# advimman/lama

Hardware: AMD Instinct MI355X
Metric: inpainted images/sec at 512x512 big-lama (higher is better)
Workload: dtype f32 (3-term f16 split on the 16-bit MFMA, fp32 accumulate, fp32 activations); 1 GPU; big-lama FFCResNetGenerator 512x512 batch=8/GPU fp32 (BASELINE configs[1]), mask-compose + generator + blend + u8, random-init weights; global_batch=8, resolution=512, parallelism=dp1, hip_graph=True, precision=f16x3, split_batch=1, full=False

## Files before the change

### include/lama_hip.h

```cpp
#ifndef LAMA_HIP_H
#define LAMA_HIP_H
#include <stddef.h>
#include <stdint.h>

#ifdef __cplusplus
extern "C" {
#endif

#define LAMA_HIP_VERSION 112

#define LAMA_OK 0
#define LAMA_ERR_BAD_ARG (-1)
#define LAMA_ERR_UNSUPPORTED (-2)
#define LAMA_ERR_WORKSPACE (-3)

#define LAMA_ACT_NONE 0
#define LAMA_ACT_RELU 1
#define LAMA_ACT_SIGMOID 2
#define LAMA_ACT_TANH 3

#define LAMA_PAD_ZERO 0
#define LAMA_PAD_REFLECT 1

#define LAMA_PREC_F32 0
#define LAMA_PREC_BF16X3 1
#define LAMA_PREC_F16X3 2
#define LAMA_PREC_F16 3

#define LAMA_DT_F32 0
#define LAMA_DT_F16 1

typedef struct lama_tensor {
    void* ptr;
    int64_t batch_stride;
    int32_t C, H, W;
    int32_t dtype;
} lama_tensor;

typedef struct lama_conv2d_args {
    lama_tensor x;
    const void* w_packed;
    int32_t kh, kw, stride, pad, pad_mode, transposed;
    lama_tensor x2;
    const void* w2_packed;
    const float* bias;
    int32_t act;
    lama_tensor resid;
    lama_tensor y;
    int32_t batch;
    int32_t precision;
    uint32_t* range_flag;
    const void* fuse1_w;
    const float* fuse1_bias;
    lama_tensor fuse1_y;
    int32_t flags;
} lama_conv2d_args;
#define LAMA_CONV_COOPERATIVE 1
#define LAMA_CONV_SIBLINGS_SHIFT 8
#define LAMA_CONV_SIBLINGS_MASK (7 << LAMA_CONV_SIBLINGS_SHIFT)
#define LAMA_CONV_SIBLINGS_LOG2(flags) (((flags) & LAMA_CONV_SIBLINGS_MASK) >> LAMA_CONV_SIBLINGS_SHIFT)
#define LAMA_CONV_DEFER_OUT 2

void lama_fuse1_channel_order(int32_t* order);

int lama_version(void);
const char* lama_error_string(int code);

int64_t lama_conv2d_packed_weight_bytes(int32_t cout, int32_t cin, int32_t kh, int32_t kw, int32_t stride,
                                        int32_t transposed, int32_t precision);
int lama_conv2d_pack_weight(void* stream, const float* w, const float* scale, int32_t cout, int32_t cin, int32_t kh,
                            int32_t kw, int32_t stride, int32_t transposed, int32_t precision, void* dst);
int lama_conv2d_fwd(void* stream, const lama_conv2d_args* args);

int64_t lama_winograd_packed_weight_bytes(int32_t cout, int32_t cin, int32_t precision);
int32_t lama_winograd_supported(int32_t cout, int32_t cin, int32_t H, int32_t W, int32_t precision);
int32_t lama_winograd_preferred(int32_t batch, int32_t cout, int32_t cin, int32_t H, int32_t W, int32_t precision);
int lama_winograd_pack_weight(void* stream, const float* w, const float* scale, int32_t cout, int32_t cin, int32_t precision, void* dst);
size_t lama_winograd_workspace_bytes(int32_t batch, int32_t cout, int32_t H, int32_t W);
int lama_winograd_conv3x3_fwd(void* stream, const lama_conv2d_args* args, void* workspace, size_t workspace_bytes);
int lama_winograd_out_fwd(void* stream, const lama_conv2d_args* args, void* workspace, size_t workspace_bytes);
int lama_rfft2_winograd_out_fwd(void* stream, const lama_tensor* x, const lama_tensor* spec, int32_t batch, void* workspace, size_t workspace_bytes,
                                const lama_conv2d_args* wino_args, void* wino_workspace, size_t wino_workspace_bytes);
int lama_fourier_unit_winograd_out_fwd(void* stream, const lama_tensor* x, const void* w_packed, const float* bias, const lama_tensor* y,
                                       int32_t batch, int32_t add_input, int32_t precision, void* workspace, size_t workspace_bytes,
                                       uint32_t* range_flag, const lama_conv2d_args* wino_args, void* wino_workspace,
                                       size_t wino_workspace_bytes);

int lama_multidilated_conv3x3_fwd(void* stream, const lama_conv2d_args* args, int32_t groups, int32_t min_dilation);

int lama_rfft2_fwd(void* stream, const lama_tensor* x, const lama_tensor* spec, int32_t batch, void* workspace,
                   size_t workspace_bytes);
int lama_irfft2_fwd(void* stream, const lama_tensor* spec, const lama_tensor* resid, const lama_tensor* y,
                    int32_t batch, void* workspace, size_t workspace_bytes);
int lama_rfft2_masked_fwd(void* stream, const lama_tensor* x, const lama_tensor* spec, const lama_tensor* mask_y, int32_t batch,
                          void* workspace, size_t workspace_bytes);
int lama_irfft2_masked_fwd(void* stream, const lama_tensor* spec, const lama_tensor* resid, const lama_tensor* mask_y, const lama_tensor* y,
                           int32_t batch, void* workspace, size_t workspace_bytes);
size_t lama_fft_workspace_bytes(int32_t batch, int32_t C, int32_t h, int32_t w);
#define LAMA_FFT_KIND_WINO64 0
#define LAMA_FFT_KIND_IP64 1
#define LAMA_FFT_KIND_IP128 2
#define LAMA_FFT_KIND_TRACE64 3
#define LAMA_FFT_KIND_SEQ 4
#define LAMA_FFT_KIND_SIZED 5
#define LAMA_FFT_KIND_GENERIC 6
int lama_fft_route_query(const lama_tensor* real, const lama_tensor* resid, const lama_tensor* spec, const lama_tensor* mask, int32_t batch,
                         int32_t inverse, const void* workspace, size_t workspace_bytes, int32_t* family, int32_t* kind);

size_t lama_fourier_unit_workspace_bytes(int32_t batch, int32_t C, int32_t h, int32_t w);
int lama_fourier_unit_fwd(void* stream, const lama_tensor* x, const void* w_packed, const float* bias,
                          const lama_tensor* y, int32_t batch, int32_t add_input, int32_t precision, void* workspace,
                          size_t workspace_bytes, uint32_t* range_flag);
int lama_fourier_unit_ex_fwd(void* stream, const lama_tensor* x, const void* w_packed, const float* bias, const lama_tensor* y,
// ... 111 lines not shown
```

### lama_amd/_lib.py

```python
from __future__ import annotations

import ctypes as C
import os
from typing import Optional

import torch

ACT_NONE, ACT_RELU, ACT_SIGMOID, ACT_TANH = 0, 1, 2, 3
PAD_ZERO, PAD_REFLECT = 0, 1
PREC_F32, PREC_BF16X3, PREC_F16X3, PREC_F16 = 0, 1, 2, 3
CONV_COOPERATIVE = 1
CONV_DEFER_OUT = 2
CONV_SIBLINGS_SHIFT = 8
DT_F32, DT_F16 = 0, 1
POOL_MAX, POOL_AVG_EXCLUDE_PAD = 0, 1
ABI_VERSION = 112
PREC_NAMES = {'f32': PREC_F32, 'bf16x3': PREC_BF16X3, 'f16x3': PREC_F16X3, 'f16': PREC_F16}

_DEFAULT = os.path.join(os.path.dirname(os.path.abspath(__file__)), 'lib', 'liblama_hip.so')


class LamaError(RuntimeError):

    def __init__(self, msg: str = '', code=None):
        super().__init__(msg)
        self.code = code


class LamaRangeError(LamaError):
    """A weight or an activation left the range of the fp16 split (|x| <= 65504): re-run with PREC_BF16X3 / PREC_F32."""

F16_MAX = 65504.0
ERR_BAD_ARG, ERR_UNSUPPORTED, ERR_WORKSPACE = -1, -2, -3
FFT_KIND_WINO64, FFT_KIND_IP64, FFT_KIND_IP128, FFT_KIND_TRACE64, FFT_KIND_SEQ, FFT_KIND_SIZED, FFT_KIND_GENERIC = range(7)


class Tensor4(C.Structure):
    _fields_ = [('ptr', C.c_void_p), ('batch_stride', C.c_int64), ('C', C.c_int32), ('H', C.c_int32), ('W', C.c_int32),
                ('dtype', C.c_int32)]


class Conv2dArgs(C.Structure):
    _fields_ = [('x', Tensor4), ('w_packed', C.c_void_p),
                ('kh', C.c_int32), ('kw', C.c_int32), ('stride', C.c_int32), ('pad', C.c_int32),
                ('pad_mode', C.c_int32), ('transposed', C.c_int32),
                ('x2', Tensor4), ('w2_packed', C.c_void_p), ('bias', C.c_void_p), ('act', C.c_int32),
                ('resid', Tensor4), ('y', Tensor4), ('batch', C.c_int32), ('precision', C.c_int32),
                ('range_flag', C.c_void_p), ('fuse1_w', C.c_void_p), ('fuse1_bias', C.c_void_p), ('fuse1_y', Tensor4),
                ('flags', C.c_int32)]


class Conv2dRectArgs(C.Structure):
    _fields_ = [('x', Tensor4), ('w_packed', C.c_void_p), ('bias', C.c_void_p), ('act', C.c_int32), ('y', Tensor4), ('batch', C.c_int32),
                ('kh', C.c_int32), ('kw', C.c_int32), ('stride', C.c_int32), ('pad_h', C.c_int32), ('pad_w', C.c_int32),
                ('precision', C.c_int32), ('range_flag', C.c_void_p)]


class TailLists(C.Structure):
    _fields_ = [('n_up', C.c_int32), ('head_rs', C.c_int32), ('up_mg', C.c_int32 * 4), ('head_list', C.c_void_p), ('head_count', C.c_void_p),
                ('up_list', C.c_void_p * 4), ('up_count', C.c_void_p * 4)]


def view(t: Optional[torch.Tensor], c0: int = 0, c: Optional[int] = None) -> Tensor4:
    if t is None:
        return Tensor4(None, 0, 0, 0, 0, 0)
    if t.dtype not in (torch.float32, torch.float16) or t.dim() != 4 or not t.is_contiguous():
        raise LamaError(f'expected a contiguous fp32 / fp16 NCHW tensor, got {t.dtype} {tuple(t.shape)}')
    B, Ct, H, W = t.shape
    c = Ct - c0 if c is None else c
    if c0 < 0 or c <= 0 or c0 + c > Ct:
        raise LamaError('channel slice out of range')
    return Tensor4(t.data_ptr() + t.element_size() * c0 * H * W, Ct * H * W, c, H, W, DT_F16 if t.dtype == torch.float16 else DT_F32)


class LamaLib:
    def __init__(self, path: Optional[str] = None, host_emulated: bool = False):
        self.host_emulated = host_emulated
        path = path or _DEFAULT
        if not os.path.exists(path):
            raise LamaError(f'{path} not found: build it with `python -m lama_amd.build` '
                            f'(hipcc --offload-arch=gfx950); lama_amd has no fallback path')
        self.path = path
        L = self._l = C.CDLL(path)
        i32, i64, vp, sz = C.c_int32, C.c_int64, C.c_void_p, C.c_size_t
        T = C.POINTER(Tensor4)
        L.lama_version.restype = C.c_int
        L.lama_error_string.restype = C.c_char_p
        L.lama_error_string.argtypes = [C.c_int]
        L.lama_conv2d_packed_weight_bytes.restype = i64
        L.lama_conv2d_packed_weight_bytes.argtypes = [i32] * 7
        L.lama_conv2d_pack_weight.restype = C.c_int
        L.lama_conv2d_pack_weight.argtypes = [vp, vp, vp, i32, i32, i32, i32, i32, i32, i32, vp]
        L.lama_conv2d_fwd.restype = C.c_int
        L.lama_conv2d_fwd.argtypes = [vp, C.POINTER(Conv2dArgs)]
        L.lama_conv2d_list_fwd.restype, L.lama_conv2d_list_fwd.argtypes = C.c_int, [vp, C.POINTER(Conv2dArgs), vp, vp, i32]
        L.lama_conv2d_list_supported.restype, L.lama_conv2d_list_supported.argtypes = i32, [C.POINTER(Conv2dArgs), i32]
        L.lama_tail_lists_workspace_bytes.restype, L.lama_tail_lists_workspace_bytes.argtypes = sz, [i32, i32, i32, C.POINTER(TailLists)]
        L.lama_tail_lists_build.restype, L.lama_tail_lists_build.argtypes = C.c_int, [vp, T, i32, C.POINTER(TailLists), vp, sz]
        L.lama_rfft2_fwd.restype = C.c_int
        L.lama_rfft2_fwd.argtypes = [vp, T, T, i32, vp, sz]
        L.lama_irfft2_fwd.restype = C.c_int
        L.lama_irfft2_fwd.argtypes = [vp, T, T, T, i32, vp, sz]
        L.lama_winograd_out_fwd.restype = C.c_int
        L.lama_winograd_out_fwd.argtypes = [vp, C.POINTER(Conv2dArgs), vp, sz]
        L.lama_rfft2_winograd_out_fwd.restype = C.c_int
        L.lama_rfft2_winograd_out_fwd.argtypes = [vp, T, T, i32, vp, sz, C.POINTER(Conv2dArgs), vp, sz]
        L.lama_rfft2_masked_fwd.restype = C.c_int
        L.lama_rfft2_masked_fwd.argtypes = [vp, T, T, T, i32, vp, sz]
        L.lama_irfft2_masked_fwd.restype = C.c_int
        L.lama_irfft2_masked_fwd.argtypes = [vp, T, T, T, T, i32, vp, sz]
        L.lama_fft_workspace_bytes.restype = sz
        L.lama_fft_workspace_bytes.argtypes = [i32] * 4
        L.lama_fft_route_query.restype = C.c_int
        L.lama_fft_route_query.argtypes = [T, T, T, T, i32, i32, vp, sz, C.POINTER(C.c_int32), C.POINTER(C.c_int32)]
        L.lama_fourier_unit_workspace_bytes.restype = sz
        L.lama_fourier_unit_workspace_bytes.argtypes = [i32] * 4
        L.lama_fourier_unit_fwd.restype = C.c_int
        L.lama_fourier_unit_fwd.argtypes = [vp, T, vp, vp, T, i32, i32, i32, vp, sz, vp]
        L.lama_fourier_unit_winograd_out_fwd.restype = C.c_int
        L.lama_fourier_unit_winograd_out_fwd.argtypes = [vp, T, vp, vp, T, i32, i32, i32, vp, sz, vp, C.POINTER(Conv2dArgs), vp, sz]
        L.lama_fourier_unit_ex_fwd.restype = C.c_int
        L.lama_fourier_unit_ex_fwd.argtypes = [vp, T, vp, vp, T, i32, i32, i32, vp, sz, vp, i32, C.POINTER(Conv2dArgs), vp, sz]
        L.lama_mask_compose_fwd.restype = C.c_int
        L.lama_mask_compose_fwd.argtypes = [vp, T, T, T, i32]
        L.lama_blend_fwd.restype = C.c_int
        L.lama_blend_fwd.argtypes = [vp, T, T, T, T, i32]
        L.lama_quantize_u8_hwc_fwd.restype = C.c_int
        L.lama_quantize_u8_hwc_fwd.argtypes = [vp, T, vp, i32, i32, i32]
        L.lama_mask_compose_u8_fwd.restype = C.c_int
        L.lama_mask_compose_u8_fwd.argtypes = [vp, vp, vp, vp, T, i32, i32]
        L.lama_blend_quantize_u8_fwd.restype = C.c_int
        L.lama_blend_quantize_u8_fwd.argtypes = [vp, vp, vp, vp, T, vp, i32, i32]
        L.lama_resize_u8_fwd.restype = C.c_int
        L.lama_resize_u8_fwd.argtypes = [vp, vp, vp, vp, vp, i32, i32, C.c_double, T, T, i32, i32]
        L.lama_eval_ingest_u8_fwd.restype = C.c_int
        L.lama_eval_ingest_u8_fwd.argtypes = [vp, vp, vp, vp, C.POINTER(i32), i32, i32, i32, i32, C.c_float, C.c_float, T, T, vp, i32]
        L.lama_affine_act_fwd.restype = C.c_int
        L.lama_affine_act_fwd.argtypes = [vp, T, vp, vp, i32, T, i32]
        L.lama_reflect_pad_fwd.restype = C.c_int
        L.lama_reflect_pad_fwd.argtypes = [vp, T, i32, T, i32]
        f32, dp = C.c_float, C.POINTER(C.c_double)
        for name, args in (('lama_act_bwd', [vp, T, T, i32, T, i32]), ('lama_add_fwd', [vp, T, T, T, i32]),
                           ('lama_reflect_pad_bwd', [vp, T, T, i32, T, i32]), ('lama_reflect_pad_bwd_fused', [vp, T, T, T, i32, T, i32, T, T, i32, vp]),
                           ('lama_dgrad_ring_fwd', [vp, T, vp, i32, vp, i32]),
                           ('lama_gauss5_fwd', [vp, T, T, i32]),
                           ('lama_gauss5_bwd', [vp, T, T, i32]), ('lama_bilinear_fwd', [vp, T, T, i32]),
                           ('lama_bilinear_bwd', [vp, T, T, i32]), ('lama_threshold_fwd', [vp, T, f32, T, i32]),
                           ('lama_erode_fwd', [vp, T, vp, i32, i32, f32, T, i32]),
                           ('lama_l1_masked_fwd', [vp, T, T, T, f32, i32, vp, i32]),
                           ('lama_l1_masked_bwd', [vp, T, T, T, f32, i32, f32, i32, T, i32]),
                           ('lama_l1_masked_per_image_fwd', [vp, T, T, T, f32, i32, vp, i32]),
                           ('lama_l1_masked_per_image_bwd', [vp, T, T, T, f32, i32, vp, i32, T, i32]),
                           ('lama_adam_step', [vp, vp, vp, vp, vp, i64, f32, f32, f32, f32, i32])):
            fn = getattr(L, name)
            fn.restype, fn.argtypes = C.c_int, args
# ... 531 lines not shown
```

### lama_amd/csrc/conv_mfma.hip

```cpp
#include "common.h"

typedef float f32x16 __attribute__((ext_vector_type(16)));

#define CONV_BN 128
#define CONV_MAX_TAPS 49

struct ConvSeg {
    const float* x;
    long long bstride;
    int C, H, W;
    const float* w;
    int stride, pad_mode;
    int dy0, dx0;
    int PH, PW;
    int tapoff[CONV_MAX_TAPS];
};

struct ConvParams {
    ConvSeg s1, s2;
    const float* bias;
    const float* resid;
    long long resid_bstride;
    float* y;
    long long y_bstride;
// ... 491 lines not shown
    const int m0 = blockIdx.y * 16, b = blockIdx.z;
    if (pix >= HW) return;
    const int gy = pix / p.W, gx = pix - gy * p.W;
    const float* xb = p.x + (long long)b * p.x_bstride;
    float acc[16];
#pragma unroll
    for (int j = 0; j < 16; ++j) acc[j] = 0.0f;
    for (int c = 0; c < p.C; ++c) {
        const int d = p.dmin << (c / p.gch);
        const float* xc = xb + (long long)c * HW;
        const float* wc = p.w + ((long long)(c >> 3) * 72 + (c & 7)) * p.Mpad + m0;
        for (int ky = 0; ky < 3; ++ky) {
            const int iy = conv_src_coord(gy + (ky - 1) * d, p.H, LAMA_PAD_REFLECT);
            for (int kx = 0; kx < 3; ++kx) {
                const int ix = conv_src_coord(gx + (kx - 1) * d, p.W, LAMA_PAD_REFLECT);
                const float v = xc[iy * p.W + ix];
                const float* wt = wc + (long long)((ky * 3 + kx) * 8) * p.Mpad;
#pragma unroll
                for (int j = 0; j < 16; ++j) acc[j] = fmaf(wt[j], v, acc[j]);
            }
        }
    }
#pragma unroll
    for (int j = 0; j < 16; ++j) {
        const int m = m0 + j;
        float v = acc[j];
        if (p.bias) v += p.bias[m];
        if (p.act == LAMA_ACT_RELU) v = fmaxf(v, 0.0f);
        else if (p.act == LAMA_ACT_SIGMOID) v = 1.0f / (1.0f + expf(-v));
        else if (p.act == LAMA_ACT_TANH) v = tanhf(v);
        const long long o = (long long)m * HW + pix;
        if (p.resid) v += p.resid[(long long)b * p.resid_bstride + o];
        p.y[(long long)b * p.y_bstride + o] = v;
    }
}

extern "C" int lama_multidilated_conv3x3_fwd(void* stream, const lama_conv2d_args* a, int32_t groups, int32_t min_dilation) {
    if (!a || !tensor_ok(a->x) || !tensor_ok(a->y) || !a->w_packed || a->batch <= 0) return LAMA_ERR_BAD_ARG;
    if ((groups != 1 && groups != 2 && groups != 4) || min_dilation < 1 || min_dilation > 8) return LAMA_ERR_UNSUPPORTED;
    if (a->kh != 3 || a->kw != 3 || a->stride != 1 || a->pad_mode != LAMA_PAD_REFLECT || a->transposed) return LAMA_ERR_UNSUPPORTED;
    if (a->x2.ptr || a->fuse1_w) return LAMA_ERR_UNSUPPORTED;
    if (a->x.dtype != LAMA_DT_F32 || a->y.dtype != LAMA_DT_F32 || (a->resid.ptr && a->resid.dtype != LAMA_DT_F32)) return LAMA_ERR_UNSUPPORTED;
    if (a->x.H != a->y.H || a->x.W != a->y.W) return LAMA_ERR_BAD_ARG;
    if (a->resid.ptr && (a->resid.C != a->y.C || a->resid.H != a->y.H || a->resid.W != a->y.W)) return LAMA_ERR_BAD_ARG;
    const int cout = a->y.C, cin = a->x.C, H = a->x.H, W = a->x.W;
    if (cin % (16 * groups) != 0 || cout % 32 != 0) return LAMA_ERR_UNSUPPORTED;
    const int dmax = min_dilation << (groups - 1);
    if (H <= dmax || W <= dmax) return LAMA_ERR_UNSUPPORTED;
    if (a->precision == LAMA_PREC_BF16X3) return lama_cb_mdconv_fwd_bf16x3((hipStream_t)stream, a, groups, min_dilation);
    if (a->precision == LAMA_PREC_F16X3) return lama_cb_mdconv_fwd_f16x3((hipStream_t)stream, a, groups, min_dilation);
    if (a->precision != LAMA_PREC_F32) return LAMA_ERR_UNSUPPORTED;
    if ((long long)cin * H * W >= (1ll << 31) || cout / 16 > 65535 || a->batch > 65535) return LAMA_ERR_UNSUPPORTED;
    MdF32Params p;
    memset(&p, 0, sizeof(p));
    p.x = (const float*)a->x.ptr;
    p.x_bstride = a->x.batch_stride;
    p.C = cin; p.H = H; p.W = W;
    p.w = (const float*)a->w_packed;
    p.Mpad = lama_round_up(cout, pick_bm(cout));
    p.bias = a->bias;
    p.resid = (const float*)a->resid.ptr;
    p.resid_bstride = a->resid.batch_stride;
    p.y = (float*)a->y.ptr;
    p.y_bstride = a->y.batch_stride;
    p.M = cout;
    p.gch = cin / groups;
    p.dmin = min_dilation;
    p.act = a->act;
    hipLaunchKernelGGL(mdconv_f32_kernel, dim3(lama_ceil_div(H * W, LAMA_NTHREADS), cout / 16, a->batch), dim3(LAMA_NTHREADS), 0, (hipStream_t)stream, p);
    LAMA_CHECK_LAUNCH();
    return LAMA_OK;
}

extern "C" void lama_fuse1_channel_order(int32_t* order) {
    for (int kq = 0; kq < 24; ++kq)
        for (int kh = 0; kh < 2; ++kh)
            for (int i = 0; i < 8; ++i) order[16 * kq + 8 * kh + i] = 32 * (kq / 2) + 16 * (kq & 1) + 8 * (i / 4) + 4 * kh + (i % 4);
}

static int conv2d_impl(void* stream, const lama_conv2d_args* a, const LamaTileList* tl) {
    if (!a || !tensor_ok(a->x) || !tensor_ok(a->y) || !a->w_packed || a->batch <= 0) return LAMA_ERR_BAD_ARG;
    if (a->precision != LAMA_PREC_F32 && a->precision != LAMA_PREC_BF16X3 && a->precision != LAMA_PREC_F16X3 && a->precision != LAMA_PREC_F16)
        return LAMA_ERR_UNSUPPORTED;
    {
        const bool xh = a->x.dtype == LAMA_DT_F16, yh = a->y.dtype == LAMA_DT_F16;
        if ((a->x.dtype != LAMA_DT_F32 && !xh) || (a->y.dtype != LAMA_DT_F32 && !yh)) return LAMA_ERR_BAD_ARG;
        if (a->x2.ptr && a->x2.dtype != LAMA_DT_F32 && a->x2.dtype != LAMA_DT_F16) return LAMA_ERR_BAD_ARG;
        if (a->x2.ptr && a->x2.dtype == LAMA_DT_F16 && a->precision != LAMA_PREC_F16) return LAMA_ERR_UNSUPPORTED;
        if (a->resid.ptr && a->resid.dtype != a->y.dtype) return LAMA_ERR_BAD_ARG;
        if ((xh || yh) != (a->precision == LAMA_PREC_F16)) return LAMA_ERR_UNSUPPORTED;
    }
    const int cout = a->y.C, cin = a->x.C;
    ConvPlan pl;
    if (!make_plan(cout, cin, a->kh, a->kw, a->stride, a->pad, a->transposed, &pl)) return LAMA_ERR_UNSUPPORTED;
    int Ho, Wo;
    if (a->transposed) {
        Ho = a->x.H * 2; Wo = a->x.W * 2;
    } else {
        Ho = (a->x.H + 2 * a->pad - a->kh) / a->stride + 1;
        Wo = (a->x.W + 2 * a->pad - a->kw) / a->stride + 1;
    }
    if (Ho != a->y.H || Wo != a->y.W) return LAMA_ERR_BAD_ARG;
    if (a->pad_mode == LAMA_PAD_REFLECT && (a->pad >= a->x.H || a->pad >= a->x.W)) return LAMA_ERR_BAD_ARG;
    const bool has2 = a->x2.ptr != nullptr;
    if (has2 && (a->transposed || !a->w2_packed || a->x2.H != Ho || a->x2.W != Wo || !tensor_ok(a->x2))) return LAMA_ERR_BAD_ARG;
    if (a->resid.ptr && (a->resid.C != cout || a->resid.H != Ho || a->resid.W != Wo)) return LAMA_ERR_BAD_ARG;
    if (a->fuse1_w) {
        if (!tensor_ok(a->fuse1_y) || a->fuse1_y.dtype != LAMA_DT_F32 || a->fuse1_y.C != 192 || a->fuse1_y.H != Ho || a->fuse1_y.W != Wo) return LAMA_ERR_BAD_ARG;
        if (cout != 384 || !has2 || a->kh != 3 || a->stride != 1 || a->y.dtype != LAMA_DT_F32 ||
            (a->precision != LAMA_PREC_BF16X3 && a->precision != LAMA_PREC_F16X3))
            return LAMA_ERR_UNSUPPORTED;
    }
    if (a->precision == LAMA_PREC_BF16X3) return lama_cb_conv2d_fwd_bf16x3((hipStream_t)stream, a, Ho, Wo, tl);
    if (a->precision == LAMA_PREC_F16X3) return lama_cb_conv2d_fwd_f16x3((hipStream_t)stream, a, Ho, Wo, tl);
    if (a->precision == LAMA_PREC_F16) return lama_cb_conv2d_fwd_f16((hipStream_t)stream, a, Ho, Wo, tl);
    if (tl) return LAMA_ERR_UNSUPPORTED;

    ConvPlan pl2;
    if (has2 && !make_plan(cout, a->x2.C, 1, 1, 1, 0, 0, &pl2)) return LAMA_ERR_UNSUPPORTED;
    if (has2 && pl2.BM != pl.BM) return LAMA_ERR_UNSUPPORTED;

    for (int cls = 0; cls < pl.nseg; ++cls) {
        ConvParams p;
        memset(&p, 0, sizeof(p));
        const bool flat = (pl.T[cls] == 1 && !a->transposed && a->stride == 1 && a->pad == 0 && !has2);
        p.bias = a->bias;
        p.resid = (const float*)a->resid.ptr;
        p.resid_bstride = a->resid.batch_stride;
        p.y = (float*)a->y.ptr;
        p.y_bstride = a->y.batch_stride;
        p.M = cout;
        p.Mpad = pl.Mpad;
        p.MT = pl.MT;
        p.B = a->batch;
        p.act = a->act;
        if (flat) {
            p.Ho = 1; p.Wo = Ho * Wo; p.GH = 1; p.GW = Ho * Wo; p.ostep = 1;
        } else if (a->transposed) {
            p.Ho = Ho; p.Wo = Wo; p.GH = a->x.H; p.GW = a->x.W; p.ostep = 2;
            p.oy0 = pl.oy0[cls]; p.ox0 = pl.ox0[cls];
        } else {
            p.Ho = Ho; p.Wo = Wo; p.GH = Ho; p.GW = Wo; p.ostep = 1;
        }
        const int stride = a->transposed ? 1 : a->stride;
        const int pad_mode = a->transposed ? LAMA_PAD_ZERO : a->pad_mode;
        const int maxp1 = pl.T[cls] == 1 ? pl.BKC[cls] * CONV_BN / LAMA_NTHREADS : 10;
        int twlog = flat ? 7 : 5;
        while (twlog > 3 && (1 << (twlog - 1)) >= p.GW) --twlog;
        bool ok = false;
        for (; twlog >= 3; --twlog) {
            ok = fill_seg(&p.s1, a->x, (const float*)a->w_packed + pl.woff[cls], pl, cls, stride, pad_mode, twlog, maxp1, flat);
            if (ok) break;
        }
        if (!ok) return LAMA_ERR_UNSUPPORTED;
        p.TWlog = twlog;
        p.tiles_x = lama_ceil_div(p.GW, 1 << twlog);
        p.tiles_y = lama_ceil_div(p.GH, CONV_BN >> twlog);
        int T2 = 0, BKC2 = 0;
        if (has2) {
            T2 = 1; BKC2 = pl2.BKC[0];
            if (!fill_seg(&p.s2, a->x2, (const float*)a->w2_packed, pl2, 0, 1, LAMA_PAD_ZERO, twlog, BKC2 * CONV_BN / LAMA_NTHREADS, false))
                return LAMA_ERR_UNSUPPORTED;
        }
        int rc = launch_conv((hipStream_t)stream, p, pl.T[cls], pl.BKC[cls], T2, BKC2, pl.BM);
        if (rc != LAMA_OK) return rc;
    }
    return LAMA_OK;
// ... 14 lines not shown
```

### lama_amd/csrc/conv_split3.inc

```
#include "common.h"
#include <stdlib.h>

typedef float f32x16 __attribute__((ext_vector_type(16)));
typedef float f32x2 __attribute__((ext_vector_type(2)));
#ifndef CB_HALF
#define CB_HALF 0
#endif
#ifndef CB_HF_W2
#define CB_HF_W2 1
#endif
#if CB_F16
typedef _Float16 cb_half_t;
#define CB_MFMA __builtin_amdgcn_mfma_f32_32x32x16_f16
#if CB_HALF
#define CB_NAME(x) x##_f16
#else
#define CB_NAME(x) x##_f16x3
#endif
#else
typedef __bf16 cb_half_t;
#define CB_MFMA __builtin_amdgcn_mfma_f32_32x32x16_bf16
#define CB_NAME(x) x##_bf16x3
#endif
typedef cb_half_t bf16x2 __attribute__((ext_vector_type(2)));
typedef cb_half_t bf16x8 __attribute__((ext_vector_type(8)));
typedef unsigned u32x4 __attribute__((ext_vector_type(4)));

namespace CB_NAME(cbns) {

#define CB_THREADS 512
#define CB_MAX_TAPS 49

enum { CB_IO_F32 = 0, CB_IO_F16_F32 = 1, CB_IO_F32_F16 = 2, CB_IO_F16 = 3, CB_IO_X2H = 4 };

struct CbSeg {
    const float* x;
    long long bstride;
    int C, H, W;
    const char* w;
    int mft;
    int nchunk, NG;
    int stride, pad_mode;
    int dy0, dx0;
    int PH, PW;
    int PWs, PWh;
    int npix;
    int tapoff[CB_MAX_TAPS];
    int vpad;
};

struct CbParams {
    CbSeg s1, s2;
    const float* bias;
    const float* resid;
    long long resid_bstride;
    float* y;
    long long y_bstride;
    int M, MT;
    int Ho, Wo;
    int GH, GW, oy0, ox0, ostep;
    long long* trace;
    const char* f1_w;
    const float* f1_bias;
    float* f1_y;
    long long f1_y_bstride;
    int TWlog, tiles_x, tiles_y, B;
    int act;
    int wbytes, pbytes;
    int nwbuf;
    unsigned* range_flag;
};

template <int BM, int NACC = 1, int MODE = 0>
struct CbGeom {
    static constexpr int WAVES_M = (BM >= 128 || ((NACC == 4 || MODE == 1) && BM == 64)) ? 2 : 1;
    static constexpr int WAVES_N = 8 / WAVES_M;
    static constexpr int BN = WAVES_N * 32;
    static constexpr int TM = BM / WAVES_M / 32;
    static constexpr int MF = BM / 32;
};

__device__ __forceinline__ int cb_src_coord(int i, int n, int pad_mode) {
    if (pad_mode == LAMA_PAD_REFLECT) {
        if (i < 0) i = -i;
        if (i >= n) i = 2 * (n - 1) - i;
        if (i < 0) i = 0;
        if (i >= n) i = n - 1;
        return i;
    }
    return (i < 0 || i >= n) ? -1 : i;
}

__device__ __forceinline__ void cb_split2(float a, float b, unsigned& hi, unsigned& lo) {
    f32x2 v = {a, b};
    bf16x2 h = __builtin_convertvector(v, bf16x2);
    f32x2 r = v - __builtin_convertvector(h, f32x2);
    bf16x2 l = __builtin_convertvector(r, bf16x2);
    hi = __builtin_bit_cast(unsigned, h);
    lo = __builtin_bit_cast(unsigned, l);
}

__device__ __forceinline__ void cb_split2_mix(float a, float b, unsigned& hi, unsigned& lo) {
#if CB_F16
    f32x2 v = {a, b};
    hi = __builtin_bit_cast(unsigned, __builtin_convertvector(v, bf16x2));
    LAMA_F16_SPLIT_LO(lo, hi, a, b);
#else
    cb_split2(a, b, hi, lo);
#endif
}

typedef unsigned short cb_u16x2 __attribute__((ext_vector_type(2)));
__device__ __forceinline__ void cb_split2(float a, float b, unsigned& hi, unsigned& lo, unsigned& rw) {
    cb_split2(a, b, hi, lo);
#if CB_F16
    rw = __builtin_bit_cast(unsigned, __builtin_elementwise_max(__builtin_bit_cast(cb_u16x2, rw), __builtin_bit_cast(cb_u16x2, hi & 0x7fff7fffu)));
// ... 752 lines not shown
        return LAMA_ERR_UNSUPPORTED;
    }
#if defined(LAMA_PROFILING) && !CB_HALF
    if (!CB_F16 && T1 == 9 && T2 == 0 && BM == 128 && maxu <= 1) {
        static const int abl = lama_env_int("LAMA_CB_ABLATE", 0);
#define CB_ABL(v) \
    if (abl == v) { hipLaunchKernelGGL((CB_NAME(conv_kernel)<9, 3, 1, 0, 0, 0, 128, 1, v>), dim3(grid), dim3(CB_THREADS), shmem, st, p); LAMA_CHECK_LAUNCH(); return LAMA_OK; }
        CB_ABL(1) CB_ABL(2) CB_ABL(4) CB_ABL(6) CB_ABL(8) CB_ABL(14) CB_ABL(15) CB_ABL(16) CB_ABL(32)
#undef CB_ABL
    }
#endif
#define CB_CASE(t1, g1, k1, t2, g2, k2) \
    if (T1 == t1 && T2 == t2) return cb_launch_bm<t1, g1, k1, t2, g2, k2>(st, p, BM, maxu, grid, shmem, io);
    CB_CASE(9, 3, 1, 0, 0, 0)
    CB_CASE(9, 3, 1, 1, 1, 2)
    CB_CASE(1, 1, 2, 0, 0, 0)
    CB_CASE(49, 7, 1, 0, 0, 0)
    CB_CASE(2, 2, 1, 0, 0, 0)
    CB_CASE(4, 4, 1, 0, 0, 0)
#undef CB_CASE
    return LAMA_ERR_UNSUPPORTED;
}

#include "conv_wreg_host.inc"

}

}
using namespace CB_NAME(cbns);

int64_t CB_NAME(lama_cb_packed_weight_bytes)(int cout, int cin, int kh, int kw, int stride, int transposed) {
    CbPlan pl;
    if (!cb_make_plan(cout, cin, kh, kw, stride, transposed ? 1 : kh / 2, transposed, &pl)) return LAMA_ERR_UNSUPPORTED;
    return pl.total_bytes;
}

int CB_NAME(lama_cb_pack_weight)(hipStream_t stream, const float* w, const float* scale, int cout, int cin, int kh, int kw, int stride,
                        int transposed, void* dst) {
    CbPlan pl;
    if (!cb_make_plan(cout, cin, kh, kw, stride, transposed ? 1 : kh / 2, transposed, &pl)) return LAMA_ERR_UNSUPPORTED;
    for (int cls = 0; cls < pl.nseg; ++cls) {
        CbPackParams pp;
        memset(&pp, 0, sizeof(pp));
        pp.w = w;
        pp.scale = scale;
        pp.dst = (char*)dst + pl.woff[cls];
        pp.M = cout;
        pp.C = cin;
        pp.MFT = pl.mft;
        pp.mode = pl.mode;
        pp.TG = pl.TG[cls];
        pp.KS = pl.KS[cls];
        pp.NG = pl.T[cls] / pl.TG[cls];
        pp.nchunk = pl.nchunk[cls];
        pp.kh = kh;
        pp.kw = kw;
        pp.transposed = transposed;
        for (int t = 0; t < pl.T[cls]; ++t) { pp.tap_ky[t] = pl.ky[cls][t]; pp.tap_kx[t] = pl.kx[cls][t]; }
        long long total = pl.cls_bytes[cls] / 32;
        int grid = (int)((total + 255) / 256);
        if (grid > 4096) grid = 4096;
        hipLaunchKernelGGL(CB_NAME(conv_pack_kernel), dim3(grid), dim3(256), 0, stream, pp);
        LAMA_CHECK_LAUNCH();
    }
    return LAMA_OK;
}

int CB_NAME(lama_cb_conv2d_fwd)(hipStream_t stream, const lama_conv2d_args* a, int Ho, int Wo, const LamaTileList* tl) {
    const int cout = a->y.C, cin = a->x.C;
    CbPlan pl;
    if (!cb_make_plan(cout, cin, a->kh, a->kw, a->stride, a->pad, a->transposed, &pl)) return LAMA_ERR_UNSUPPORTED;
    const bool has2 = a->x2.ptr != nullptr;
    if (tl) {
        if (has2 || a->fuse1_w) return LAMA_ERR_UNSUPPORTED;
        const int io_l = (a->x.dtype == LAMA_DT_F16 ? 1 : 0) | (a->y.dtype == LAMA_DT_F16 ? 2 : 0);
        if ((io_l != CB_IO_F32) != (CB_HALF != 0)) return LAMA_ERR_UNSUPPORTED;
        return a->transposed ? ct_try_launch(stream, a, pl, Ho, Wo, io_l, tl) : head_try_launch(stream, a, pl, Ho, Wo, io_l, tl);
    }
    CbPlan pl2;
    if (has2 && !cb_make_plan(cout, a->x2.C, 1, 1, 1, 0, 0, &pl2)) return LAMA_ERR_UNSUPPORTED;
    if (has2 && pl.mode) return LAMA_ERR_UNSUPPORTED;
    const int io = (a->x.dtype == LAMA_DT_F16 ? 1 : 0) | (a->y.dtype == LAMA_DT_F16 ? 2 : 0) | ((has2 && a->x2.dtype == LAMA_DT_F16) ? CB_IO_X2H : 0);
    if ((io != CB_IO_F32) != (CB_HALF != 0)) return LAMA_ERR_UNSUPPORTED;
    {
        int rc = cw_try_launch(stream, a, pl, has2 ? &pl2 : nullptr, Ho, Wo, io);
        if (rc != LAMA_ERR_UNSUPPORTED) return rc;
        if (!has2) {
            rc = ct_try_launch(stream, a, pl, Ho, Wo, io);
            if (rc != LAMA_ERR_UNSUPPORTED) return rc;
        }
    }
    if (a->fuse1_w) return LAMA_ERR_UNSUPPORTED;

    if (!has2) {
        int rc = stem_try_launch(stream, a, pl, Ho, Wo, io);
        if (rc != LAMA_ERR_UNSUPPORTED) return rc;
        rc = head_try_launch(stream, a, pl, Ho, Wo, io);
        if (rc != LAMA_ERR_UNSUPPORTED) return rc;
    }
    int BM = cb_pick_bm(pl.rows, pl.mode ? 49 : pl.T[0], a->transposed ? 1 : a->stride, a->batch, a->transposed ? a->x.H : Ho,
                        a->transposed ? a->x.W : Wo);
    { static const int bm_env = lama_env_int("LAMA_CB_BM", 0); if (bm_env && a->transposed) BM = bm_env; }
    if (BM < 128 && !a->transposed && a->stride == 2) BM = 128;
    if (pl.mode == 1) BM = cout > 64 ? 128 : 64;
    const int BN = (BM >= 128 || ((a->transposed || pl.mode == 1) && BM == 64)) ? 128 : 256;
    if ((long long)a->x.C * a->x.H * a->x.W >= (1ll << 31) || (has2 && (long long)a->x2.C * a->x2.H * a->x2.W >= (1ll << 31)))
        return LAMA_ERR_UNSUPPORTED;

    for (int cls = 0; cls < (a->transposed ? 1 : pl.nseg); ++cls) {
        CbParams p;
        memset(&p, 0, sizeof(p));
        const bool flat = (pl.T[cls] == 1 && !a->transposed && a->stride == 1 && a->pad == 0 && !has2);
        p.bias = a->bias;
        p.resid = (const float*)a->resid.ptr;
        p.resid_bstride = a->resid.batch_stride;
        p.y = (float*)a->y.ptr;
        p.y_bstride = a->y.batch_stride;
        p.M = pl.rows;
        p.MT = lama_ceil_div(pl.rows, BM);
        p.B = a->batch;
        p.act = a->act;
        p.range_flag = a->range_flag;
        if (flat) {
            p.Ho = 1; p.Wo = Ho * Wo; p.GH = 1; p.GW = Ho * Wo; p.ostep = 1;
        } else if (a->transposed) {
            p.Ho = Ho; p.Wo = Wo; p.GH = a->x.H; p.GW = a->x.W; p.ostep = 2;
            p.oy0 = pl.oy0[cls]; p.ox0 = pl.ox0[cls];
        } else {
            p.Ho = Ho; p.Wo = Wo; p.GH = Ho; p.GW = Wo; p.ostep = 1;
        }
        const int stride = a->transposed ? 1 : a->stride;
        const int pad_mode = a->transposed ? LAMA_PAD_ZERO : a->pad_mode;
        int twlog = flat ? lama_ilog2(BN) : 5;
        while (pl.mode != 2 && twlog > 3 && (1 << (twlog - 1)) >= p.GW) --twlog;
        const int TW = 1 << twlog, TH = BN >> twlog;
        p.TWlog = twlog;
        p.tiles_x = pl.mode == 2 ? lama_ceil_div(p.GW, 26) : lama_ceil_div(p.GW, TW);
        p.tiles_y = lama_ceil_div(p.GH, TH);
        int units = cb_fill_seg(&p.s1, a->x, (const char*)a->w_packed + pl.woff[cls], pl, cls, stride, pad_mode, TH, TW, flat);
        p.s1.vpad = a->pad;
        long long wbytes = (long long)pl.TG[cls] * pl.KS[cls] * (BM / 32) * 2048;
        long long pbytes = (long long)2 * 2 * pl.KS[cls] * p.s1.npix * 16;
        int TG2 = 0, KS2 = 0;
        if (has2) {
            TG2 = pl2.TG[0]; KS2 = pl2.KS[0];
            int u2 = cb_fill_seg(&p.s2, a->x2, (const char*)a->w2_packed, pl2, 0, 1, LAMA_PAD_ZERO, TH, TW, false);
            units = u2 > units ? u2 : units;
            long long w2 = (long long)TG2 * KS2 * (BM / 32) * 2048, p2 = (long long)2 * 2 * KS2 * p.s2.npix * 16;
            wbytes = w2 > wbytes ? w2 : wbytes;
            pbytes = p2 > pbytes ? p2 : pbytes;
        }
        p.wbytes = (int)wbytes;
        p.pbytes = (int)pbytes;
        {
            int smax = p.s1.nchunk * p.s1.NG;
            if (has2 && p.s2.nchunk * p.s2.NG > smax) smax = p.s2.nchunk * p.s2.NG;
            p.nwbuf = smax < 3 ? smax : 3;
        }
        int rc = cb_launch(stream, p, pl.T[cls], has2 ? 1 : 0, BM, lama_ceil_div(units, CB_THREADS), a->transposed != 0, pl.mode, io);
        if (rc != LAMA_OK) return rc;
    }
    return LAMA_OK;
}

#if !CB_HALF
int CB_NAME(lama_cb_mdconv_fwd)(hipStream_t stream, const lama_conv2d_args* a, int groups, int min_dilation) {
// ... 238 lines not shown
```

### lama_amd/csrc/conv_stem_dev.inc

```

struct StemParams {
    const float* x;
    long long x_bstride;
    int C, H, W;
    const char* w;
    int mft;
    const float* bias;
    float* y;
    long long y_bstride;
    int M, B, act;
    int tx;
    int ns, rs;
    int nseg;
    unsigned* range_flag;
};

#define STEM_WIN 40
#define STEM_SLOT (4 * STEM_WIN)
#define STEM_WAVE_LDS (8 * STEM_SLOT + 64)
#define STEM_LDS_BYTES (4 * STEM_WAVE_LDS * 4)

__device__ __forceinline__ void stem_pack2(float a, float b, unsigned& pa, unsigned& pb, unsigned& rw) {
    unsigned hi, lo;
    cb_split2(a, b, hi, lo, rw);
    pa = __builtin_amdgcn_perm(lo, hi, 0x05040100u);
    pb = __builtin_amdgcn_perm(lo, hi, 0x07060302u);
}

template <bool HO = false>
__global__ __launch_bounds__(256, 2) void CB_NAME(stem7_ws_kernel)(StemParams p) {
    constexpr int ESO = HO ? 2 : 4;
    const int tid = threadIdx.x, lane = tid & 63, wave = LAMA_WAVE_UNIFORM(tid >> 6);
    const int F = wave & 1, half = wave >> 1;
    const int khalf = lane >> 5, l31 = lane & 31;
    const int H = p.H, W = p.W, HW = H * W;
    const int strip = blockIdx.x * 2 + half, nstrips = gridDim.x * 2;
    unsigned* const win = reinterpret_cast<unsigned*>(lama_smem) + wave * STEM_WAVE_LDS;
    unsigned rw = 0;

    for (int i = lane; i < STEM_WAVE_LDS; i += 64) win[i] = 0u;

    constexpr bool ALO = !HO || CB_HF_W2;
    u32x4 ah[14], al[ALO ? 14 : 1];
    {
        const lama_buf_t wres = LAMA_BUF_RSRC(p.w, (long long)14 * p.mft * 2048);
        const int Fc = F < p.mft ? F : p.mft - 1;
#pragma unroll
        for (int s = 0; s < 14; ++s) {
            ah[s] = __builtin_bit_cast(u32x4, LAMA_BUF_LOAD_B128(wres, lane * 16, (s * p.mft + Fc) * 2048));
            if constexpr (ALO) al[s] = __builtin_bit_cast(u32x4, LAMA_BUF_LOAD_B128(wres, lane * 16 + 1024, (s * p.mft + Fc) * 2048));
        }
    }
    float bv[16];
    {
        const lama_buf_t bres = LAMA_BUF_RSRC(p.bias, p.bias ? (long long)p.M * 4 : 0ll);
#pragma unroll
        for (int r = 0; r < 16; ++r) bv[r] = __builtin_bit_cast(float, LAMA_BUF_LOAD_B32(bres, (F * 32 + (r & 3) + 8 * (r >> 2) + 4 * khalf) * 4, 0));
    }
    int widx[2][8];
#pragma unroll
    for (int ks = 0; ks < 2; ++ks)
#pragma unroll
        for (int e = 0; e < 8; ++e) {
            const int c = 16 * ks + 8 * khalf + e;
            const int cc = c / 7, kx = c - cc * 7;
            widx[ks][e] = c < 28 ? cc * STEM_WIN + l31 + kx : l31;
        }
    int lcc[3], lj[3], lw[3];
#pragma unroll
    for (int i = 0; i < 3; ++i) {
        const int id = lane + 64 * i;
        lcc[i] = id / 38;
        lj[i] = id - lcc[i] * 38;
        lw[i] = id < 152 ? lcc[i] * STEM_WIN + lj[i] : -1;
    }
    LAMA_WAVE_SYNC();

#pragma unroll 1
    for (int g = strip; g < p.nseg; g += nstrips) {
        const int col = g / p.ns, part = g - col * p.ns;
        const int b = col / p.tx, px0 = (col - b * p.tx) * 32;
        const int y0 = part * p.rs, y1 = (y0 + p.rs < H) ? y0 + p.rs : H;
        const lama_buf_t xres = LAMA_BUF_RSRC(p.x + (long long)b * p.x_bstride, (long long)p.C * HW * 4);
        const lama_buf_t yres = LAMA_BUF_RSRC(reinterpret_cast<char*>(p.y) + (long long)b * p.y_bstride * ESO, (long long)p.M * HW * ESO);
        int coloff[3];
#pragma unroll
        for (int i = 0; i < 3; ++i) {
            int ix = px0 - 3 + lj[i];
            ix = ix < 0 ? -ix : ix;
            ix = ix >= W ? 2 * (W - 1) - ix : ix;
            ix = ix < 0 ? 0 : (ix >= W ? W - 1 : ix);
            coloff[i] = (lw[i] >= 0 && lcc[i] < p.C) ? (lcc[i] * HW + ix) * 4 : 0x7ffffff0;
        }
        auto row_off = [&](int u) {
            int iy = u < 0 ? -u : u;
            iy = iy >= H ? 2 * (H - 1) - iy : iy;
            iy = iy < 0 ? 0 : (iy >= H ? H - 1 : iy);
            return iy * W * 4;
        };
        float nr[3];
        auto request_row = [&](int u) {
            const int ro = row_off(u);
#pragma unroll
            for (int i = 0; i < 3; ++i) nr[i] = __builtin_bit_cast(float, LAMA_BUF_LOAD_B32(xres, coloff[i], ro));
        };
        auto deposit_row = [&](int u) {
            unsigned pk[4];
            stem_pack2(nr[0], nr[1], pk[0], pk[1], rw);
            stem_pack2(nr[2], 0.0f, pk[2], pk[3], rw);
            unsigned* slot = win + ((u + 8) & 7) * STEM_SLOT;
#pragma unroll
            for (int i = 0; i < 3; ++i) {
                if (lw[i] >= 0) slot[lw[i]] = pk[i];
                else win[8 * STEM_SLOT + lane] = pk[i];
            }
        };
        for (int u = y0 - 3; u <= y0 + 3; ++u) {
            request_row(u);
            deposit_row(u);
        }
        LAMA_WAVE_SYNC();

#pragma unroll 1
        for (int y = y0; y < y1; ++y) {
            request_row(y + 4);
            f32x16 acc;
#pragma unroll
            for (int r = 0; r < 16; ++r) acc[r] = 0.0f;
            unsigned d[2][8];
            auto read_k = [&](auto s_tag) {
                constexpr int s = decltype(s_tag)::value;
                const unsigned* slot = win + ((y + (s >> 1) + 5) & 7) * STEM_SLOT;
#pragma unroll
                for (int e = 0; e < 8; ++e) d[s & 1][e] = slot[widx[s & 1][e]];
            };
            auto mma_k = [&](auto s_tag) {
                constexpr int s = decltype(s_tag)::value;
                if constexpr (s + 1 < 14) read_k(CbTag<(s + 1 < 14 ? s + 1 : 0)>{});
                unsigned hh[4], ll[4];
#pragma unroll
                for (int e = 0; e < 4; ++e) {
                    hh[e] = __builtin_amdgcn_perm(d[s & 1][2 * e + 1], d[s & 1][2 * e], 0x05040100u);
                    ll[e] = __builtin_amdgcn_perm(d[s & 1][2 * e + 1], d[s & 1][2 * e], 0x07060302u);
                }
                const bf16x8 bh = __builtin_bit_cast(bf16x8, u32x4{hh[0], hh[1], hh[2], hh[3]});
                const bf16x8 bl = __builtin_bit_cast(bf16x8, u32x4{ll[0], ll[1], ll[2], ll[3]});
                __builtin_amdgcn_sched_barrier(0);
                acc = CB_MFMA(__builtin_bit_cast(bf16x8, ah[s]), bh, acc, 0, 0, 0);
                if constexpr (!HO) acc = CB_MFMA(__builtin_bit_cast(bf16x8, ah[s]), bl, acc, 0, 0, 0);
                if constexpr (ALO) acc = CB_MFMA(__builtin_bit_cast(bf16x8, al[s]), bh, acc, 0, 0, 0);
            };
            read_k(CbTag<0>{});
            mma_k(CbTag<0>{}); mma_k(CbTag<1>{}); mma_k(CbTag<2>{}); mma_k(CbTag<3>{}); mma_k(CbTag<4>{}); mma_k(CbTag<5>{}); mma_k(CbTag<6>{});
            mma_k(CbTag<7>{}); mma_k(CbTag<8>{}); mma_k(CbTag<9>{}); mma_k(CbTag<10>{}); mma_k(CbTag<11>{}); mma_k(CbTag<12>{}); mma_k(CbTag<13>{});
            LAMA_WAVE_SYNC();
            deposit_row(y + 4);
            LAMA_WAVE_SYNC();
            const int px = px0 + l31;
            const int eoff = (px < W && F < p.mft) ? ((F * 32 + 4 * khalf) * HW + y * W + px) * ESO : 0x7ffffff0;
            float ov[16];
#pragma unroll
            for (int r = 0; r < 16; ++r) ov[r] = acc[r] + bv[r];
            if (p.act == LAMA_ACT_RELU) {
#pragma unroll
                for (int r = 0; r < 16; ++r) ov[r] = fmaxf(ov[r], 0.0f);
            } else if (p.act == LAMA_ACT_SIGMOID) {
#pragma unroll
                for (int r = 0; r < 16; ++r) ov[r] = 1.0f / (1.0f + expf(-ov[r]));
            } else if (p.act == LAMA_ACT_TANH) {
#pragma unroll
                for (int r = 0; r < 16; ++r) ov[r] = tanhf(ov[r]);
            }
#pragma unroll
            for (int r = 0; r < 16; ++r) {
                if constexpr (HO) LAMA_BUF_STORE_B16(yres, __builtin_bit_cast(unsigned short, (_Float16)ov[r]), eoff, ((r & 3) + 8 * (r >> 2)) * HW * ESO);
                else LAMA_BUF_STORE_B32(yres, __builtin_bit_cast(unsigned, ov[r]), eoff, ((r & 3) + 8 * (r >> 2)) * HW * ESO);
            }
        }
        LAMA_WAVE_SYNC();
    }
    cb_range_report(rw, p.range_flag);
}
```

### lama_amd/csrc/conv_wreg_dev.inc

```

template <int T, int KSC, int WMV, int KG>
struct CwShape {
    static_assert((T == 9 && (KSC == 2 || (KSC == 1 && KG == 1))) || (T == 1 && KSC == 4),
                  "3x3 over 32-channel chunks (16-channel chunks in the 4 x 1 geometry) or 1x1 over 64-channel chunks");
    static_assert(KG == 1 || KG == 2, "K-groups");
    static constexpr int THREADS = 64 * WMV * KG;
    static constexpr int NKG = T * KSC / KG;
    static constexpr int WPS = WMV * KG / 4;
    static constexpr int PFD = (T == 1 && KG == 2) ? 2 : 1;
#ifndef LAMA_CW_RING9
#define LAMA_CW_RING9 0
#endif
    static constexpr int RING = (T == 9) ? ((LAMA_CW_RING9 && KG == 2 && WPS <= 2) ? 9 : ((KSC == 2 && WMV == 4 && KG == 1) ? 6 : 3)) : ((WPS >= 3) ? 2 : 4);
    static constexpr bool BDB = WPS <= 2;
    static constexpr int NOCT = 2 * KSC;
    static_assert((PFD * NKG) % RING == 0, "ring slot must be a compile-time function of the unrolled position");
};

struct CwFrag {
    bf16x8 bh[4], bl[4];
};

template <int T, int KSC, int WMV, int KG, int ABL = 0, int SCH = 2, bool HF = false, bool HI = HF, bool ROLL = false, int NU = 2>
__device__ __forceinline__ void cw_segment(const CbSeg& s, int F, int b, int gy0, int gx0, int TWlog, char* pbuf0, int pbytes,
                                           f32x16 (&acc)[4], unsigned& rw, long long* trace = nullptr) {
    using S = CwShape<T, KSC, WMV, KG>;
    constexpr int NKG = S::NKG, PFD = S::PFD, RING = S::RING, NOCT = S::NOCT, D = RING - 1, THREADS = S::THREADS;
    constexpr bool BDB = S::BDB;
    constexpr int BKC = 16 * KSC;
    constexpr int ES = HI ? 2 : 4;
    const int tid = threadIdx.x, lane = tid & 63, wave = LAMA_WAVE_UNIFORM(tid >> 6);
    const int kg = KG == 1 ? 0 : wave / WMV;
    const int khalf = lane >> 5, l31 = lane & 31;
    const int TW = 1 << TWlog;
    const int HW = s.H * s.W;
    const int NPR = s.PH * s.PW;
    const int nunits = NPR * NOCT;
    const int pdump = NOCT * s.npix * 16;
    const int plo = pdump + 16;
    const int nchunk = s.C / BKC;

    int ubase[NU], lds_off[NU], uvalid[NU];
#pragma unroll
    for (int i = 0; i < NU; ++i) {
        const int u = i * THREADS + tid;
        int so = 0, lo = pdump, ok = 0, q = 0;
        if (u < nunits) {
            q = u / NPR;
            const int pp = u - q * NPR;
            const int py = pp / s.PW, px = pp - py * s.PW;
            const int iy = cb_src_coord(gy0 * s.stride + s.dy0 + py, s.H, s.pad_mode);
            const int ix = cb_src_coord(gx0 * s.stride + s.dx0 + px, s.W, s.pad_mode);
            if (iy >= 0 && ix >= 0) { so = iy * s.W + ix; ok = 1; }
            lo = (q * s.npix + py * s.PWs + (s.PWh ? (px & 1) * s.PWh + (px >> 1) : px)) * 16;
        }
        ubase[i] = (q * 8 * HW + so) * ES;
        lds_off[i] = lo;
        uvalid[i] = ok;
    }
    const lama_buf_t xres = LAMA_BUF_RSRC(reinterpret_cast<const char*>(s.x) + (long long)b * s.bstride * ES, (long long)s.C * HW * ES);
    float preg[PFD][NU][8];
    auto load_units = [&](int ch, auto slot_tag) {
        constexpr int SL = decltype(slot_tag)::value;
#pragma unroll
        for (int e = 0; e < 8; ++e) {
            const int so = (ch * BKC + e) * HW * ES;
#pragma unroll
            for (int i = 0; i < NU; ++i) {
                if constexpr (HI) preg[SL][i][e] = __builtin_bit_cast(float, (unsigned)LAMA_BUF_LOAD_B16(xres, ubase[i], so));
                else preg[SL][i][e] = __builtin_bit_cast(float, LAMA_BUF_LOAD_B32(xres, ubase[i], so));
            }
        }
    };
    auto write_units = [&](char* pb, auto slot_tag) {
        constexpr int SL = decltype(slot_tag)::value;
#pragma unroll
        for (int i = 0; i < NU; ++i) {
            unsigned hh[4], ll[4];
#pragma unroll
            for (int e = 0; e < 4; ++e) {
                if constexpr (HI) {
                    hh[e] = __builtin_bit_cast(unsigned, preg[SL][i][2 * e]) | (__builtin_bit_cast(unsigned, preg[SL][i][2 * e + 1]) << 16);
                    cb_range_watch(hh[e], rw);
                    ll[e] = 0u;
                } else if constexpr (HF) {
                    f32x2 v2 = {preg[SL][i][2 * e], preg[SL][i][2 * e + 1]};
                    hh[e] = __builtin_bit_cast(unsigned, __builtin_convertvector(v2, bf16x2));
                    cb_range_watch(hh[e], rw);
                    ll[e] = 0u;
                } else cb_split2(preg[SL][i][2 * e], preg[SL][i][2 * e + 1], hh[e], ll[e], rw);
            }
            u32x4 h = {hh[0], hh[1], hh[2], hh[3]}, l = {ll[0], ll[1], ll[2], ll[3]};
            if (!uvalid[i]) { h = u32x4{0, 0, 0, 0}; l = h; }
            *reinterpret_cast<u32x4*>(pb + lds_off[i]) = h;
            if constexpr (!HF) *reinterpret_cast<u32x4*>(pb + plo + lds_off[i]) = l;
        }
    };

    auto c16_of = [&](int kk) { return T == 9 ? (KG == 2 ? kg : kk / 9) : (KG == 2 ? 2 * kg + kk : kk); };
    int boff[4];
#pragma unroll
    for (int j = 0; j < 4; ++j) {
        const int n = j * 32 + l31;
        const int ty = n >> TWlog, tx = n & (TW - 1);
        boff[j] = (((KG == 2 ? (T == 9 ? 2 * kg : 4 * kg) : 0) + khalf) * s.npix + ty * s.stride * s.PWs + tx) * 16;
    }
    int tgoff[T];
#pragma unroll
    for (int t = 0; t < T; ++t) tgoff[t] = s.tapoff[t] * 16;
    auto read_bj = [&](CwFrag& f, const char* pb, int kk, int j, bool hi, bool lo) {
        const int koct = T == 9 ? (KG == 2 ? 0 : kk / 9) : kk;
        const char* bp = pb + tgoff[T == 1 ? 0 : kk % T] + koct * 2 * s.npix * 16 + boff[j];
        if (hi) f.bh[j] = *reinterpret_cast<const bf16x8*>(bp);
        if constexpr (!HF) { if (lo) f.bl[j] = *reinterpret_cast<const bf16x8*>(bp + plo); }
    };
    auto read_b = [&](CwFrag& f, const char* pb, int kk) {
#pragma unroll
        for (int j = 0; j < 4; ++j) read_bj(f, pb, kk, j, true, true);
    };

    const int kbytes = s.mft * 2048;
    const lama_buf_t wres = LAMA_BUF_RSRC(s.w, (long long)(s.C / 16) * T * kbytes);
    const int aoff = F * 2048 + lane * 16;
    constexpr bool ALO = !HF || CB_HF_W2;
    u32x4 ah[RING], al[ALO ? RING : 1];
    auto tap_of = [&](int sx) { return ROLL ? (sx % 3) * 3 + sx / 3 : sx; };
    auto kstep_q = [&](int c, int kk) { return (T == 9) ? (KSC * c + c16_of(kk)) * 9 + tap_of(kk % 9) : 4 * c + c16_of(kk); };
    auto load_a = [&](int R, int q) {
        ah[R] = __builtin_bit_cast(u32x4, LAMA_BUF_LOAD_B128(wres, aoff, q * kbytes));
        if constexpr (ALO) al[R] = __builtin_bit_cast(u32x4, LAMA_BUF_LOAD_B128(wres, aoff + 1024, q * kbytes));
    };

    load_units(0, CbTag<0>{});
#pragma unroll
    for (int i = 0; i < D; ++i) load_a(i, kstep_q(i / NKG, i % NKG));
    write_units(pbuf0, CbTag<0>{});
    if constexpr (PFD == 2) load_units(1, CbTag<1>{});
    __syncthreads();
    if constexpr (ABL & 64) { if (threadIdx.x == 0) trace[1] = LAMA_CLOCK(); }

    auto chunk = [&](int c, auto slot_tag) {
        constexpr int SLOT = decltype(slot_tag)::value;
        const char* pb = pbuf0 + (c & 1) * pbytes;
        char* pbn = pbuf0 + ((c + 1) & 1) * pbytes;
        CwFrag fr[BDB ? 2 : 1];
        read_b(fr[0], pb, 0);
        auto kstep = [&](auto kk_tag) {
            constexpr int kk = decltype(kk_tag)::value;
            constexpr int RS = (SLOT * NKG + kk) % RING;
            constexpr int CUR = BDB ? (kk & 1) : 0, NXT = BDB ? ((kk + 1) & 1) : 0;
            if constexpr (SCH == 2) __builtin_amdgcn_sched_barrier(0);
            constexpr bool LDU = !(ABL & 4) && !(ABL & 32) && kk == 0;
            constexpr bool WRU = !(ABL & 4) && !(ABL & 16) && kk == NKG - 1;
            constexpr bool RDB = (kk + 1 < NKG) && !(ABL & 2);
            if constexpr (LDU) load_units(c + PFD, CbTag<SLOT>{});
            if constexpr (!(ABL & 1)) {
                constexpr int n2 = kk + D;
                load_a((RS + D) % RING, kstep_q(c + n2 / NKG, n2 % NKG));
            }
            if constexpr (BDB && kk + 1 < NKG) {
                if constexpr (ABL & 2) fr[NXT] = fr[CUR];
                else read_b(fr[NXT], pb, kk + 1);
            }
            if constexpr ((ABL & 16) && kk == NKG - 1) {
#pragma unroll
                for (int e = 0; e < 8; ++e)
#pragma unroll
                    for (int i = 0; i < NU; ++i) LAMA_KEEP_LIVE(preg[0][i][e]);
            }
            if constexpr (WRU) write_units(pbn, CbTag<(SLOT + 1) % PFD>{});
            if constexpr (SCH == 1) __builtin_amdgcn_sched_barrier(0);
            const bf16x8 a_hi = __builtin_bit_cast(bf16x8, ah[RS]), a_lo = __builtin_bit_cast(bf16x8, al[ALO ? RS : 0]);
            CwFrag& f = fr[CUR];
            if constexpr (HF) {
                if constexpr (CB_HF_W2) {
#pragma unroll
                    for (int j = 0; j < 4; ++j) acc[j] = CB_MFMA(a_hi, f.bh[j], acc[j], 0, 0, 0);
                }
#pragma unroll
                for (int j = 0; j < 4; ++j) {
                    acc[j] = CB_MFMA(CB_HF_W2 ? a_lo : a_hi, f.bh[j], acc[j], 0, 0, 0);
                    if constexpr (!BDB && RDB) read_bj(f, pb, kk + 1, j, true, false);
                }
            } else if constexpr (ABL & 8) {
                LAMA_KEEP_LIVE(a_hi); LAMA_KEEP_LIVE(a_lo);
#pragma unroll
                for (int j = 0; j < 4; ++j) { LAMA_KEEP_LIVE(f.bh[j]); LAMA_KEEP_LIVE(f.bl[j]); }
            } else if constexpr (BDB) {
#pragma unroll
                for (int j = 0; j < 4; ++j) acc[j] = CB_MFMA(a_hi, f.bh[j], acc[j], 0, 0, 0);
#pragma unroll
                for (int j = 0; j < 4; ++j) acc[j] = CB_MFMA(a_hi, f.bl[j], acc[j], 0, 0, 0);
#pragma unroll
                for (int j = 0; j < 4; ++j) acc[j] = CB_MFMA(a_lo, f.bh[j], acc[j], 0, 0, 0);
            } else {
#pragma unroll
                for (int j = 0; j < 4; ++j) acc[j] = CB_MFMA(a_hi, f.bh[j], acc[j], 0, 0, 0);
#pragma unroll
                for (int j = 0; j < 4; ++j) {
                    acc[j] = CB_MFMA(a_hi, f.bl[j], acc[j], 0, 0, 0);
                    if constexpr (RDB) read_bj(f, pb, kk + 1, j, false, true);
                }
#pragma unroll
                for (int j = 0; j < 4; ++j) {
                    acc[j] = CB_MFMA(a_lo, f.bh[j], acc[j], 0, 0, 0);
                    if constexpr (RDB) read_bj(f, pb, kk + 1, j, true, false);
                }
            }
            if constexpr (SCH == 1) __builtin_amdgcn_sched_barrier(0);
            if constexpr (SCH == 2 && !(ABL & 8) && !HF) {
                constexpr int NVM = ((ABL & 1) ? 0 : 2) + (LDU ? 8 * NU : 0);
                auto grp = [&](auto i_tag) {
                    constexpr int i = decltype(i_tag)::value;
                    __builtin_amdgcn_sched_group_barrier(0x008, 1, 0);
                    if constexpr (BDB) {
                        if constexpr (RDB && i < 8) __builtin_amdgcn_sched_group_barrier(0x100, 1, 0);
                        constexpr int nv = (i >= 8) ? (NVM + 11 - i) / 4 : 0;
                        if constexpr (nv > 0) __builtin_amdgcn_sched_group_barrier(0x020, nv, 0);
                        if constexpr (WRU && i >= 8) __builtin_amdgcn_sched_group_barrier(0x200, (2 * NU + 11 - i) / 4, 0);
                    } else {
                        constexpr int nv = (i < 4) ? (NVM + 3 - i) / 4 : 0;
                        if constexpr (nv > 0) __builtin_amdgcn_sched_group_barrier(0x020, nv, 0);
                        if constexpr (WRU && i < 4) __builtin_amdgcn_sched_group_barrier(0x200, (2 * NU + 3 - i) / 4, 0);
                        if constexpr (RDB && i >= 4) __builtin_amdgcn_sched_group_barrier(0x100, 1, 0);
                    }
                };
                grp(CbTag<0>{}); grp(CbTag<1>{}); grp(CbTag<2>{}); grp(CbTag<3>{}); grp(CbTag<4>{}); grp(CbTag<5>{});
                grp(CbTag<6>{}); grp(CbTag<7>{}); grp(CbTag<8>{}); grp(CbTag<9>{}); grp(CbTag<10>{}); grp(CbTag<11>{});
                __builtin_amdgcn_sched_barrier(0);
            }
        };
        static_assert(NKG == 2 || NKG == 4 || NKG == 9 || NKG == 18, "k-steps per chunk");
        kstep(CbTag<0>{});
        kstep(CbTag<1>{});
        if constexpr (NKG > 2) { kstep(CbTag<2>{}); kstep(CbTag<3>{}); }
        if constexpr (NKG > 4) {
            kstep(CbTag<4>{}); kstep(CbTag<5>{}); kstep(CbTag<6>{}); kstep(CbTag<7>{}); kstep(CbTag<8>{});
        }
        if constexpr (NKG > 9) {
            kstep(CbTag<9>{}); kstep(CbTag<10>{}); kstep(CbTag<11>{}); kstep(CbTag<12>{}); kstep(CbTag<13>{}); kstep(CbTag<14>{});
            kstep(CbTag<15>{}); kstep(CbTag<16>{}); kstep(CbTag<17>{});
        }
        __syncthreads();
        if constexpr (ABL & 64) { if (threadIdx.x == 0 && c < 28) trace[2 + c] = LAMA_CLOCK(); }
    };
    struct CwRow { bf16x8 h, l; };
    [[maybe_unused]] int rowoff[6];
    if constexpr (ROLL) {
#pragma unroll
        for (int r = 0; r < 6; ++r) rowoff[r] = (((KG == 2 ? 2 * kg : 0) + khalf) * s.npix + r * s.PWs + l31) * 16;
    }
    [[maybe_unused]] auto read_row = [&](CwRow& d, const char* pb, int g, int kx, int r) {
        const char* bp = pb + (g * 2 * s.npix + kx) * 16 + rowoff[r];
        d.h = *reinterpret_cast<const bf16x8*>(bp);
        if constexpr (!HF) d.l = *reinterpret_cast<const bf16x8*>(bp + plo);
    };
    [[maybe_unused]] auto chunk_roll = [&](int c, auto) {
        static_assert(!ROLL || (T == 9 && PFD == 1 && NKG % 9 == 0), "ROLL: 3x3 only");
        const char* pb = pbuf0 + (c & 1) * pbytes;
        char* pbn = pbuf0 + ((c + 1) & 1) * pbytes;
        constexpr int NSET = NKG / 3;
        CwRow rows[8];
        [[maybe_unused]] long long tks[NKG + 1];
#pragma unroll
        for (int r = 0; r < 4; ++r) read_row(rows[r], pb, 0, 0, r);
        auto kstep = [&](auto kk_tag) {
            constexpr int kk = decltype(kk_tag)::value;
            constexpr int g = kk / 9, kx = (kk % 9) / 3, ky = kk % 3, si = kk / 3, par = si & 1;
            constexpr int RS = kk % RING;
            constexpr bool more = si + 1 < NSET;
            constexpr int gn = (3 * (si + 1)) / 9, kxn = ((3 * (si + 1)) % 9) / 3;
            constexpr int S2 = par ? 6 : 2, S3 = par ? 7 : 3, S2n = par ? 2 : 6, S3n = par ? 3 : 7;
            __builtin_amdgcn_sched_barrier(0);
            if constexpr (ABL & 64) { if (c == 8 && wave == 0) tks[kk] = LAMA_CYCLES(); }
            constexpr bool LDU = !(ABL & 4) && !(ABL & 32) && kk == 0;
            constexpr bool WRU = !(ABL & 4) && !(ABL & 16) && kk == NKG - 1;
            constexpr int NDS = (ABL & 2) ? 0 : ((ky == 0 || more) ? (HF ? 2 : 4) : 0);
            if constexpr (LDU) load_units(c + PFD, CbTag<0>{});
            if constexpr (!(ABL & 1)) {
                constexpr int n2 = kk + D;
                load_a((RS + D) % RING, kstep_q(c + n2 / NKG, n2 % NKG));
            }
            if constexpr (NDS > 0) {
                if constexpr (ky == 0) { read_row(rows[4], pb, g, kx, 4); read_row(rows[5], pb, g, kx, 5); }
                else if constexpr (ky == 1) { read_row(rows[0], pb, gn, kxn, 0); read_row(rows[S2n], pb, gn, kxn, 2); }
                else { read_row(rows[1], pb, gn, kxn, 1); read_row(rows[S3n], pb, gn, kxn, 3); }
            }
            if constexpr ((ABL & 16) && kk == NKG - 1) {
#pragma unroll
                for (int e = 0; e < 8; ++e)
#pragma unroll
                    for (int i = 0; i < NU; ++i) LAMA_KEEP_LIVE(preg[0][i][e]);
            }
            if constexpr (WRU) write_units(pbn, CbTag<0>{});
            const bf16x8 a_hi = __builtin_bit_cast(bf16x8, ah[RS]), a_lo = __builtin_bit_cast(bf16x8, al[ALO ? RS : 0]);
            auto slot = [&](int r) { return r == 2 ? S2 : (r == 3 ? S3 : r); };
            if constexpr (ABL & 8) {
                LAMA_KEEP_LIVE(a_hi); LAMA_KEEP_LIVE(a_lo);
#pragma unroll
                for (int j = 0; j < 4; ++j) { LAMA_KEEP_LIVE(rows[slot(ky + j)].h); LAMA_KEEP_LIVE(rows[slot(ky + j)].l); }
            } else {
#pragma unroll
            for (int j = 0; j < 4; ++j) acc[j] = CB_MFMA(a_hi, rows[slot(ky + j)].h, acc[j], 0, 0, 0);
            }
            if constexpr (!HF && !(ABL & 8)) {
#pragma unroll
                for (int j = 0; j < 4; ++j) acc[j] = CB_MFMA(a_hi, rows[slot(ky + j)].l, acc[j], 0, 0, 0);
#pragma unroll
                for (int j = 0; j < 4; ++j) acc[j] = CB_MFMA(a_lo, rows[slot(ky + j)].h, acc[j], 0, 0, 0);
            } else if constexpr (HF && CB_HF_W2 && !(ABL & 8)) {
#pragma unroll
                for (int j = 0; j < 4; ++j) acc[j] = CB_MFMA(a_lo, rows[slot(ky + j)].h, acc[j], 0, 0, 0);
            }
            if constexpr (SCH == 2 && !HF && !(ABL & 8)) {
                constexpr int NVM = ((ABL & 1) ? 0 : 2) + (LDU ? 8 * NU : 0);
                auto grp = [&](auto i_tag) {
                    constexpr int i = decltype(i_tag)::value;
                    __builtin_amdgcn_sched_group_barrier(0x008, 1, 0);
                    if constexpr (i < NDS) __builtin_amdgcn_sched_group_barrier(0x100, 1, 0);
                    constexpr int nv = (i >= 8) ? (NVM + 11 - i) / 4 : 0;
                    if constexpr (nv > 0) __builtin_amdgcn_sched_group_barrier(0x020, nv, 0);
                    if constexpr (WRU && i >= 8) __builtin_amdgcn_sched_group_barrier(0x200, (2 * NU + 11 - i) / 4, 0);
                };
                grp(CbTag<0>{}); grp(CbTag<1>{}); grp(CbTag<2>{}); grp(CbTag<3>{}); grp(CbTag<4>{}); grp(CbTag<5>{});
                grp(CbTag<6>{}); grp(CbTag<7>{}); grp(CbTag<8>{}); grp(CbTag<9>{}); grp(CbTag<10>{}); grp(CbTag<11>{});
                __builtin_amdgcn_sched_barrier(0);
            }
        };
        kstep(CbTag<0>{}); kstep(CbTag<1>{}); kstep(CbTag<2>{}); kstep(CbTag<3>{}); kstep(CbTag<4>{});
        kstep(CbTag<5>{}); kstep(CbTag<6>{}); kstep(CbTag<7>{}); kstep(CbTag<8>{});
        if constexpr (NKG > 9) {
            kstep(CbTag<9>{}); kstep(CbTag<10>{}); kstep(CbTag<11>{}); kstep(CbTag<12>{}); kstep(CbTag<13>{}); kstep(CbTag<14>{});
            kstep(CbTag<15>{}); kstep(CbTag<16>{}); kstep(CbTag<17>{});
        }
        if constexpr (ABL & 64) { if (c == 8 && wave == 0) tks[NKG] = LAMA_CYCLES(); }
        if constexpr (!(ABL & 128)) __syncthreads();
        if constexpr (ABL & 64) {
            if (threadIdx.x == 0 && c < 16) trace[2 + c] = LAMA_CLOCK();
            if (threadIdx.x == 0 && c == 8 && NKG == 9) {
#pragma unroll
                for (int i = 0; i <= NKG; ++i) trace[18 + i] = tks[i];
                trace[28] = LAMA_CYCLES();
            }
        }
    };
    if constexpr (ROLL) {
        for (int c = 0; c < nchunk; ++c) chunk_roll(c, CbTag<0>{});
    } else if constexpr (PFD == 1) {
        for (int c = 0; c < nchunk; ++c) chunk(c, CbTag<0>{});
    } else {
        for (int c = 0; c < nchunk; c += 2) {
            chunk(c, CbTag<0>{});
            if (c + 1 < nchunk) chunk(c + 1, CbTag<1>{});
        }
    }
}

template <int T1, int KSC1, int T2, int KSC2, int WMV = 4, int KG = 2, int ABL = 0, int SCH = 2, bool HF = false, bool HI1 = HF, bool HI2 = HF,
          bool HO = HF, bool ROLL = false, int NU = 2, bool FUSE1 = false>
__global__ __launch_bounds__(64 * WMV * KG, (WMV * KG == 4) ? 2 : 1) void CB_NAME(conv_wr_kernel)(CbParams p) {
    using AT = typename LamaAct<HO>::T;
    const int L = lama_xcd_remap(blockIdx.x, gridDim.x);
    const int mt = L % p.MT;
    int tile = L / p.MT;
    const int tix = tile % p.tiles_x;
    tile /= p.tiles_x;
    const int tiy = tile % p.tiles_y;
    const int b = tile / p.tiles_y;
    const int TW = 1 << p.TWlog, TH = 128 >> p.TWlog;
    const int gy0 = tiy * TH, gx0 = tix * TW;
    const int tid = threadIdx.x, lane = tid & 63, wave = LAMA_WAVE_UNIFORM(tid >> 6);
    const int kg = wave / WMV, wm = wave % WMV;
    const int F = mt * WMV + wm;
    const int Fc = F < p.s1.mft ? F : p.s1.mft - 1;

    long long* trace = nullptr;
    if constexpr (ABL & 64) {
        trace = p.trace + (long long)blockIdx.x * 32;
        if (threadIdx.x == 0) trace[0] = LAMA_CLOCK();
    }
    f32x16 acc[4];
#pragma unroll
    for (int j = 0; j < 4; ++j)
#pragma unroll
        for (int r = 0; r < 16; ++r) acc[j][r] = 0.0f;

    unsigned rw = 0;
    const int Fw = (ABL & 256) ? Fc % 6 : Fc;
    cw_segment<T1, KSC1, WMV, KG, (ABL & 255), SCH, HF, HI1, ROLL && T1 == 9, NU>(p.s1, Fw, b, gy0, gx0, p.TWlog, lama_smem, p.pbytes, acc, rw, trace);
    if constexpr (T2 > 0) cw_segment<T2, KSC2, WMV, KG, (ABL & 65), SCH, HF, HI2>(p.s2, Fw, b, gy0, gx0, p.TWlog, lama_smem, p.pbytes, acc, rw, (ABL & 64) ? trace + 7 : nullptr);
    cb_range_report(rw, p.range_flag);

    const long long plane = (long long)p.Ho * p.Wo;
    const int khalf4 = 4 * (lane >> 5);
    const int kplane = khalf4 * (int)plane;
    auto row_u = [&](int r) { return F * 32 + (r & 3) + 8 * (r >> 2); };
    float bv[16];
#pragma unroll
    for (int r = 0; r < 16; ++r) bv[r] = p.bias ? p.bias[row_u(r) + khalf4 < p.M ? row_u(r) + khalf4 : p.M - 1] : 0.0f;
    constexpr int NRV = (WMV * KG / 4 >= 3) ? 1 : 2;
    float rv[NRV][16];
    auto frag_off = [&](int j, bool& pv) {
        const int n = j * 32 + (lane & 31);
        const int gy = gy0 + (n >> p.TWlog), gx = gx0 + (n & (TW - 1));
        pv = gy < p.GH && gx < p.GW;
        return (gy < p.GH ? gy : p.GH - 1) * p.Wo + (gx < p.GW ? gx : p.GW - 1);
    };
    auto load_resid = [&](int j, int slot) {
        bool pv;
        const int po = frag_off(j, pv);
#pragma unroll
        for (int r = 0; r < 16; ++r) {
            const int mu = row_u(r), muc = mu < p.M ? mu : p.M - 1;
            rv[slot][r] = p.resid ? (float)(reinterpret_cast<const AT*>(p.resid) + (long long)b * p.resid_bstride + (long long)muc * plane)[(unsigned)(po + (mu + khalf4 < p.M ? kplane : 0))] : 0.0f;
        }
    };
    auto store_frag = [&](int j, const f32x16& v16, int slot) {
        bool pv;
        const unsigned lo = (unsigned)(frag_off(j, pv) + kplane);
#pragma unroll
        for (int r = 0; r < 16; ++r) {
            const int mu = row_u(r);
            float v = v16[r] + bv[r];
            if (p.act == LAMA_ACT_RELU) v = fmaxf(v, 0.0f);
            else if (p.act == LAMA_ACT_SIGMOID) v = 1.0f / (1.0f + expf(-v));
            else if (p.act == LAMA_ACT_TANH) v = tanhf(v);
            v += rv[slot][r];
            if (pv && mu + khalf4 < p.M) (reinterpret_cast<AT*>(p.y) + (long long)b * p.y_bstride + (long long)mu * plane)[lo] = (AT)v;
        }
    };
    if constexpr (FUSE1) {
        static_assert(WMV == 12 && KG == 1 && !HF, "fused conv1: the 12 x 1 geometry of the 3-term split only");
        const int F1 = wave % 6, g1 = wave / 6;
        const lama_buf_t w1res = LAMA_BUF_RSRC(p.f1_w, (long long)24 * 6 * 2048);
        char* const lb = lama_smem;
        constexpr int R1 = 6;
        u32x4 wh[R1], wl[R1];
        auto load_w1 = [&](int slot, int kk) {
            const int so = ((12 * g1 + kk) * 6 + F1) * 2048;
            wh[slot] = __builtin_bit_cast(u32x4, LAMA_BUF_LOAD_B128(w1res, lane * 16, so));
            wl[slot] = __builtin_bit_cast(u32x4, LAMA_BUF_LOAD_B128(w1res, lane * 16 + 1024, so));
        };
        u32x4 bq[4][2][2];
#pragma unroll
        for (int j = 0; j < 4; ++j) {
            load_resid(j, 0);
            bool pv;
            const unsigned lo = (unsigned)(frag_off(j, pv) + kplane);
            float vv[16];
#pragma unroll
            for (int r = 0; r < 16; ++r) {
                const int mu = row_u(r);
                float v = acc[j][r] + bv[r];
                if (p.act == LAMA_ACT_RELU) v = fmaxf(v, 0.0f);
                else if (p.act == LAMA_ACT_SIGMOID) v = 1.0f / (1.0f + expf(-v));
                else if (p.act == LAMA_ACT_TANH) v = tanhf(v);
                v += rv[0][r];
                vv[r] = v;
                if (pv && mu + khalf4 < p.M) (reinterpret_cast<AT*>(p.y) + (long long)b * p.y_bstride + (long long)mu * plane)[lo] = (AT)v;
            }
#pragma unroll
            for (int ks = 0; ks < 2; ++ks) {
                unsigned hh[4], ll[4];
#pragma unroll
                for (int e = 0; e < 4; ++e) cb_split2(vv[8 * ks + 2 * e], vv[8 * ks + 2 * e + 1], hh[e], ll[e], rw);
                bq[j][ks][0] = u32x4{hh[0], hh[1], hh[2], hh[3]};
                bq[j][ks][1] = u32x4{ll[0], ll[1], ll[2], ll[3]};
            }
        }
#pragma unroll
        for (int pass = 0; pass < 2; ++pass) {
#pragma unroll
            for (int i = 0; i < R1; ++i) load_w1(i, i);
#pragma unroll
            for (int jj = 0; jj < 2; ++jj)
#pragma unroll
                for (int ks = 0; ks < 2; ++ks) {
                    char* dst = lb + ((((2 * F + ks) * 2 + jj) * 2) * 64 + lane) * 16;
                    *reinterpret_cast<u32x4*>(dst) = bq[2 * pass + jj][ks][0];
                    *reinterpret_cast<u32x4*>(dst + 1024) = bq[2 * pass + jj][ks][1];
                }
            __syncthreads();
            f32x16 a2[2];
#pragma unroll
            for (int jj = 0; jj < 2; ++jj)
#pragma unroll
                for (int r = 0; r < 16; ++r) a2[jj][r] = 0.0f;
            bf16x8 xh[2][2], xl[2][2];
            auto read_x = [&](int buf, int kk) {
#pragma unroll
                for (int jj = 0; jj < 2; ++jj) {
                    const char* src = lb + ((((12 * g1 + kk) * 2 + jj) * 2) * 64 + lane) * 16;
                    xh[buf][jj] = *reinterpret_cast<const bf16x8*>(src);
                    xl[buf][jj] = *reinterpret_cast<const bf16x8*>(src + 1024);
                }
            };
            read_x(0, 0);
#pragma unroll
            for (int kk = 0; kk < 12; ++kk) {
                const bf16x8 w_hi = __builtin_bit_cast(bf16x8, wh[kk % R1]), w_lo = __builtin_bit_cast(bf16x8, wl[kk % R1]);
                if (kk + 1 < 12) read_x((kk + 1) & 1, kk + 1);
#pragma unroll
                for (int jj = 0; jj < 2; ++jj) {
                    a2[jj] = CB_MFMA(w_hi, xh[kk & 1][jj], a2[jj], 0, 0, 0);
                    a2[jj] = CB_MFMA(w_hi, xl[kk & 1][jj], a2[jj], 0, 0, 0);
                    a2[jj] = CB_MFMA(w_lo, xh[kk & 1][jj], a2[jj], 0, 0, 0);
                }
                if (kk + R1 < 12) load_w1(kk % R1, kk + R1);
            }
            {
                typedef float f32x4 __attribute__((ext_vector_type(4)));
                f32x4* xw = reinterpret_cast<f32x4*>(lama_smem + 96 * 1024) + wave * 256;
#pragma unroll
                for (int r4 = 0; r4 < 4; ++r4) {
                    const f32x16& o = g1 == 0 ? a2[1] : a2[0];
                    xw[r4 * 64 + lane] = f32x4{o[4 * r4], o[4 * r4 + 1], o[4 * r4 + 2], o[4 * r4 + 3]};
                }
                __syncthreads();
                const f32x4* xr = reinterpret_cast<const f32x4*>(lama_smem + 96 * 1024) + (F1 + 6 * (1 - g1)) * 256;
                f32x16 sum = g1 == 0 ? a2[0] : a2[1];
#pragma unroll
                for (int r4 = 0; r4 < 4; ++r4) {
                    const f32x4 o = xr[r4 * 64 + lane];
#pragma unroll
                    for (int e = 0; e < 4; ++e) sum[4 * r4 + e] += o[e];
                }
                bool pv;
                const unsigned lo1 = (unsigned)(frag_off(2 * pass + g1, pv) + kplane);
#pragma unroll
                for (int r = 0; r < 16; ++r) {
                    const int mu1 = F1 * 32 + (r & 3) + 8 * (r >> 2);
                    const float v = fmaxf(sum[r] + (p.f1_bias ? p.f1_bias[mu1 + khalf4] : 0.0f), 0.0f);
                    if (pv) (p.f1_y + (long long)b * p.f1_y_bstride + (long long)mu1 * plane)[lo1] = v;
                }
            }
        }
        cb_range_report(rw, p.range_flag);
    } else if constexpr (KG == 1) {
        if (NRV == 2) load_resid(0, 0);
#pragma unroll
        for (int j = 0; j < 4; ++j) {
            if (NRV == 1) load_resid(j, 0);
            else if (j + 1 < 4) load_resid(j + 1, (j + 1) & 1);
            store_frag(j, acc[j], NRV == 1 ? 0 : (j & 1));
        }
    } else {
        if (kg == 1) {
#pragma unroll
            for (int r = 0; r < 16; ++r) {
                float t0 = acc[0][r], t1 = acc[1][r];
                acc[0][r] = acc[2][r]; acc[1][r] = acc[3][r];
                acc[2][r] = t0; acc[3][r] = t1;
            }
        }
        typedef float f32x4 __attribute__((ext_vector_type(4)));
        f32x4* xw = reinterpret_cast<f32x4*>(lama_smem) + wave * 512;
#pragma unroll
        for (int jj = 0; jj < 2; ++jj)
#pragma unroll
            for (int r4 = 0; r4 < 4; ++r4)
                xw[(jj * 4 + r4) * 64 + lane] = f32x4{acc[2 + jj][4 * r4], acc[2 + jj][4 * r4 + 1], acc[2 + jj][4 * r4 + 2], acc[2 + jj][4 * r4 + 3]};
        __syncthreads();
        const f32x4* xr = reinterpret_cast<const f32x4*>(lama_smem) + ((1 - kg) * WMV + wm) * 512;
        if constexpr (NRV == 2) {
            load_resid(2 * kg, 0);
            load_resid(2 * kg + 1, 1);
        }
#pragma unroll
        for (int jj = 0; jj < 2; ++jj) {
            if constexpr (NRV == 1) load_resid(2 * kg + jj, 0);
            f32x16 sum = acc[jj];
#pragma unroll
            for (int r4 = 0; r4 < 4; ++r4) {
                const f32x4 o = xr[(jj * 4 + r4) * 64 + lane];
#pragma unroll
                for (int e = 0; e < 4; ++e) sum[4 * r4 + e] += o[e];
            }
            store_frag(2 * kg + jj, sum, NRV == 1 ? 0 : jj);
        }
    }
    if constexpr (ABL & 64) { if (threadIdx.x == 0) { trace[30] = LAMA_CLOCK(); trace[31] = L; } }
}
```

### lama_amd/csrc/conv_wreg_host.inc

```

template <int T1, int KSC1, int T2, int KSC2, int WMV, int KG>
int cw_launch_t(hipStream_t st, const CbParams& p, int grid, size_t shmem, int io = CB_IO_F32) {
#if CB_HALF
    constexpr bool CAN_ROLL = (T1 == 9 && WMV * KG <= 8);
    const bool roll = CAN_ROLL && p.TWlog == 5;
#define CW_H(hi1, hi2, ho)                                                                                                                       \
    do {                                                                                                                                         \
        if (roll) hipLaunchKernelGGL((CB_NAME(conv_wr_kernel)<T1, KSC1, T2, KSC2, WMV, KG, 0, 0, true, hi1, hi2, ho, CAN_ROLL>), dim3(grid),    \
                                     dim3(64 * WMV * KG), shmem, st, p);                                                                        \
        else hipLaunchKernelGGL((CB_NAME(conv_wr_kernel)<T1, KSC1, T2, KSC2, WMV, KG, 0, 0, true, hi1, hi2, ho>), dim3(grid),                   \
                                dim3(64 * WMV * KG), shmem, st, p);                                                                             \
    } while (0)
    const int io3 = io & 3;
    const bool x2h = (io & CB_IO_X2H) != 0;
    if (io != CB_IO_F32) {
        if (T2 > 0 && !x2h) return LAMA_ERR_UNSUPPORTED;
        if (io3 == CB_IO_F16) CW_H(true, true, true);
        else if constexpr ((T1 == 9 && T2 == 0 && WMV == 4 && KG == 2) || (T1 == 9 && T2 == 1 && WMV == 12 && KG == 1)) {
            if (io3 == CB_IO_F32_F16) CW_H(false, true, true);
            else if (io3 == CB_IO_F16_F32) CW_H(true, true, false);
            else return LAMA_ERR_UNSUPPORTED;
        } else return LAMA_ERR_UNSUPPORTED;
        LAMA_CHECK_LAUNCH();
        return LAMA_OK;
// ... 163 lines not shown
    memset(&p, 0, sizeof(p));
    p.x = (const float*)a->x.ptr;
    p.x_bstride = a->x.batch_stride;
    p.HW = (int)HW;
    p.C = C;
    p.w = (const char*)a->w_packed + pl.woff[0];
    p.mft = pl.mft;
    p.bias = a->bias;
    p.resid = (const float*)a->resid.ptr;
    p.resid_bstride = a->resid.batch_stride;
    p.y = (float*)a->y.ptr;
    p.y_bstride = a->y.batch_stride;
    p.M = pl.rows;
    p.B = a->batch;
    p.act = a->act;
    p.range_flag = a->range_flag;
    static const int NH_env = lama_env_int("LAMA_GEMM_WS_NH", 1) == 2 ? 2 : 1;
    const int NH = io != CB_IO_F32 ? 1 : NH_env;
    p.tiles_per_img = (int)lama_ceil_div64(HW, GW_TILE(NH));
    p.ntiles = p.B * p.tiles_per_img;
    p.ntypes = pl.mft / 3;
    const int wgs = 256 * (3 - NH);
    if (p.ntypes > wgs) return LAMA_ERR_UNSUPPORTED;
    if (mode != 2 && (long long)p.ntiles * p.ntypes < 64) return LAMA_ERR_UNSUPPORTED;
    p.nslots = wgs / p.ntypes;
    if (p.nslots > p.ntiles) p.nslots = p.ntiles;
    const int grid = p.nslots * p.ntypes;
    if (grid <= 0) return LAMA_OK;
    { static const int abl = lama_env_int("LAMA_GW_ABLATE", 0); p.abl = abl; }
    { static const int prio = lama_env_int("LAMA_SIDE_PRIO", 1); p.prio = prio; }
    const dim3 blk(GW_THREADS(NH));
    const size_t lds = GW_LDS_BYTES(NH);
#if defined(LAMA_PROFILING) && !CB_HALF
    if (CB_F16 && C == 384) {
        static const unsigned long long tr = lama_env_u64("LAMA_GW_TRACE");
        if (tr) {
            p.trace = reinterpret_cast<long long*>(tr);
            if (NH == 2) hipLaunchKernelGGL((CB_NAME(gemm1x1_ws_kernel)<6, true, 2, true>), dim3(grid), blk, lds, stream, p);
            else hipLaunchKernelGGL((CB_NAME(gemm1x1_ws_kernel)<6, true, 1, true>), dim3(grid), blk, lds, stream, p);
            LAMA_CHECK_LAUNCH();
            return LAMA_OK;
        }
    }
#endif
    const bool rs = p.resid != nullptr;
#if CB_HALF
    if (io == CB_IO_F16) {
#define GW_CASE_H(nch, rs_) hipLaunchKernelGGL((CB_NAME(gemm1x1_ws_kernel)<nch, rs_, 1, false, true>), dim3(grid), blk, lds, stream, p)
        if (C == 384) { if (rs) GW_CASE_H(6, true); else GW_CASE_H(6, false); }
        else { if (rs) GW_CASE_H(3, true); else GW_CASE_H(3, false); }
#undef GW_CASE_H
        LAMA_CHECK_LAUNCH();
        return LAMA_OK;
    }
    if (io == CB_IO_F32_F16) {
        if (C != 384 || rs) return LAMA_ERR_UNSUPPORTED;
        hipLaunchKernelGGL((CB_NAME(gemm1x1_ws_kernel)<6, false, 1, false, true, false, true>), dim3(grid), blk, lds, stream, p);
        LAMA_CHECK_LAUNCH();
        return LAMA_OK;
    }
    return LAMA_ERR_UNSUPPORTED;
#else
    if (io != CB_IO_F32) return LAMA_ERR_UNSUPPORTED;
#define GW_CASE(nch, rs, nh) hipLaunchKernelGGL((CB_NAME(gemm1x1_ws_kernel)<nch, rs, nh>), dim3(grid), blk, lds, stream, p)
    if (NH == 2) {
        if (C == 384) { if (rs) GW_CASE(6, true, 2); else GW_CASE(6, false, 2); }
        else { if (rs) GW_CASE(3, true, 2); else GW_CASE(3, false, 2); }
    } else {
        if (C == 384) { if (rs) GW_CASE(6, true, 1); else GW_CASE(6, false, 1); }
        else { if (rs) GW_CASE(3, true, 1); else GW_CASE(3, false, 1); }
    }
#undef GW_CASE
    LAMA_CHECK_LAUNCH();
    return LAMA_OK;
#endif
}

int cw_launch_s2(hipStream_t st, const CbParams& p, int grid, size_t shmem, int io) {
#if CB_HALF
    if (io != CB_IO_F16 && io != CB_IO_F16_F32) return LAMA_ERR_UNSUPPORTED;
    if (io == CB_IO_F16) hipLaunchKernelGGL((CB_NAME(conv_wr_kernel)<9, 1, 0, 0, 4, 1, 0, 0, true, true, true, true, false, 5>), dim3(grid), dim3(256), shmem, st, p);
    else hipLaunchKernelGGL((CB_NAME(conv_wr_kernel)<9, 1, 0, 0, 4, 1, 0, 0, true, true, true, false, false, 5>), dim3(grid), dim3(256), shmem, st, p);
#else
    if (io != CB_IO_F32) return LAMA_ERR_UNSUPPORTED;
    static const int geo = lama_env_int("LAMA_CW_S2", 1);
    if (geo == 2) hipLaunchKernelGGL((CB_NAME(conv_wr_kernel)<9, 2, 0, 0, 4, 2, 0, 2, false, false, false, false, false, 5>), dim3(grid), dim3(512), shmem, st, p);
    else hipLaunchKernelGGL((CB_NAME(conv_wr_kernel)<9, 1, 0, 0, 4, 1, 0, 2, false, false, false, false, false, 5>), dim3(grid), dim3(256), shmem, st, p);
#endif
    LAMA_CHECK_LAUNCH();
    return LAMA_OK;
}

static long long cw_pick_tile(int GW, int GH, int batch, unsigned flags, int* twlog_out) {
    int twlog = 5;
    while (twlog > 3 && (1 << (twlog - 1)) >= GW) --twlog;
    if (twlog == 5) {
        long long best_rounds = 0;
        for (int tl = 5; tl >= 3; --tl) {
            const long long nt = ((long long)batch * lama_ceil_div(GW, 1 << tl) * lama_ceil_div(GH, 128 >> tl)) << LAMA_CONV_SIBLINGS_LOG2(flags);
            const long long rounds = (nt + 255) / 256;
            if (tl == 5 || rounds < best_rounds) { best_rounds = rounds; twlog = tl; }
        }
        static const int force = lama_env_int("LAMA_CW_TWLOG", 0);
        if (force >= 3 && force <= 5) twlog = force;
    }
    *twlog_out = twlog;
    return (long long)lama_ceil_div(GW, 1 << twlog) * lama_ceil_div(GH, 128 >> twlog);
}

int cw_try_launch(hipStream_t stream, const lama_conv2d_args* a, const CbPlan& pl, const CbPlan* pl2, int Ho, int Wo, int io) {
    if (!pl2) {
        int rc = gk_try_launch(stream, a, pl, Ho, Wo, io);
        if (rc != LAMA_ERR_UNSUPPORTED) return rc;
        rc = g4_try_launch(stream, a, pl, Ho, Wo, io);
        if (rc != LAMA_ERR_UNSUPPORTED) return rc;
        rc = gw_try_launch(stream, a, pl, Ho, Wo, io);
        if (rc != LAMA_ERR_UNSUPPORTED) return rc;
    }
    if (!cw_enabled() || a->transposed || (a->stride != 1 && a->stride != 2) || pl.mode != 0 || pl.nseg != 1) return LAMA_ERR_UNSUPPORTED;
    const bool s2 = a->stride == 2;
    if (s2 && (pl.T[0] != 9 || pl2 || a->pad != 1)) return LAMA_ERR_UNSUPPORTED;
    const int T1 = pl.T[0];
    int twlog3 = 5;
    const long long tiles_img = (T1 == 9 && !s2) ? cw_pick_tile(Wo, Ho, a->batch, a->flags, &twlog3) : lama_ceil_div64((long long)Ho * Wo, 128);
    if (!((T1 == 9 && a->x.C % 32 == 0) || (T1 == 1 && a->x.C % 64 == 0))) return LAMA_ERR_UNSUPPORTED;
    if (pl2 && a->x2.C % 64 != 0) return LAMA_ERR_UNSUPPORTED;
    if (pl.rows < 96) return LAMA_ERR_UNSUPPORTED;
    int WMV = 4, KG = 2;
#if CB_HALF
    const int s2geo = 1;
#else
    static const int s2geo = lama_env_int("LAMA_CW_S2", 1);
#endif
    if (s2 && s2geo != 2) KG = 1;
    const int g41 = lama_env_int("LAMA_CW_41", 0);
    bool geo41 = false, coop41 = false;
    if (pl.T[0] == 9 && !pl2 && !s2 && pl.mft % 4 == 0) {
        const long long wgs = (long long)a->batch * tiles_img * (pl.mft / 4);
        const bool f32io = (io == CB_IO_F32) && !CB_HALF;
        if (g41 == 2 || ((g41 == 0 || g41 == 1) && wgs >= 512 && f32io)) { geo41 = true; KG = 1; }
        const bool flagged = (a->flags & LAMA_CONV_COOPERATIVE) && g41 != -1 && wgs >= 224;
        if ((flagged || g41 == 3) && f32io && wgs <= 320) { geo41 = true; coop41 = true; KG = 1; }
    }
    static const int g12 = lama_env_int("LAMA_CW_G12", 1);
    static const int g12_min = lama_env_int("LAMA_CW_G12_MIN", 160);
    const long long tiles_g = ((long long)a->batch * tiles_img) << LAMA_CONV_SIBLINGS_LOG2(a->flags);
    if (T1 == 9 && pl2 && pl.mft == 12 && (g12 == 2 || (g12 == 1 && tiles_g >= g12_min))) { WMV = 12; KG = 1; }
    if (T1 == 1 && !pl2) {
        static const int full_m = lama_env_int("LAMA_CW_1X1", 1);
        const long long tiles128 = (long long)a->batch * lama_ceil_div64((long long)Ho * Wo, 128);
        const bool want = full_m >= 2 || (full_m == 1 && tiles128 >= 96);
        if (full_m == 3 && pl.mft == 12) { WMV = 6; KG = 2; }
        else if (want && pl.mft == 12) { WMV = 12; KG = 1; }
        else if (want && pl.mft == 6) { WMV = 6; KG = 2; }
        else if (pl.mft % 4 != 0) return LAMA_ERR_UNSUPPORTED;
    }
    const int threads = 64 * WMV * KG;
    if ((long long)a->x.C * a->x.H * a->x.W >= (1ll << 31) || (pl2 && (long long)a->x2.C * a->x2.H * a->x2.W >= (1ll << 31)))
        return LAMA_ERR_UNSUPPORTED;
    CbParams p;
    memset(&p, 0, sizeof(p));
    const bool flat = (T1 == 1 && a->pad == 0 && !pl2);
    p.bias = a->bias;
    p.resid = (const float*)a->resid.ptr;
    p.resid_bstride = a->resid.batch_stride;
    p.y = (float*)a->y.ptr;
    p.y_bstride = a->y.batch_stride;
    p.M = pl.rows;
    p.MT = lama_ceil_div(pl.mft, WMV);
    p.B = a->batch;
    p.act = a->act;
    p.range_flag = a->range_flag;
    p.ostep = 1;
    if (flat) { p.Ho = 1; p.Wo = Ho * Wo; p.GH = 1; p.GW = Ho * Wo; }
    else { p.Ho = Ho; p.Wo = Wo; p.GH = Ho; p.GW = Wo; }
    int twlog = flat ? 7 : 5;
    while (twlog > 3 && (1 << (twlog - 1)) >= p.GW) --twlog;
    if (T1 == 9 && !s2) twlog = twlog3;
    const int TW = 1 << twlog, TH = 128 >> twlog;
    p.TWlog = twlog;
    p.tiles_x = lama_ceil_div(p.GW, TW);
    p.tiles_y = lama_ceil_div(p.GH, TH);
    const int KSC1 = T1 == 9 ? (KG == 1 && WMV == 4 && !coop41 ? 1 : 2) : 4;
    cb_fill_seg(&p.s1, a->x, (const char*)a->w_packed + pl.woff[0], pl, 0, a->stride, a->pad_mode, TH, TW, flat);
    p.s1.vpad = a->pad;
    int units = p.s1.PH * p.s1.PW * 2 * KSC1;
    long long pbytes = (long long)2 * (2 * KSC1 * p.s1.npix * 16 + 16);
    if (pl2) {
        cb_fill_seg(&p.s2, a->x2, (const char*)a->w2_packed, *pl2, 0, 1, LAMA_PAD_ZERO, TH, TW, false);
        const int u2 = p.s2.PH * p.s2.PW * 8;
        const long long p2 = (long long)2 * (8 * p.s2.npix * 16 + 16);
        units = u2 > units ? u2 : units;
        pbytes = p2 > pbytes ? p2 : pbytes;
    }
    if (units > (s2 ? 5 : (coop41 ? 4 : 2)) * threads) return LAMA_ERR_UNSUPPORTED;
    p.pbytes = (int)pbytes;
    size_t shmem = 2 * (size_t)pbytes;
    if (KG == 2 && shmem < (size_t)(threads / 64) * 8192) shmem = (size_t)(threads / 64) * 8192;
    if (shmem > 160 * 1024) return LAMA_ERR_UNSUPPORTED;
    const int grid = p.B * p.tiles_x * p.tiles_y * p.MT;
    if (grid <= 0) return LAMA_OK;
#if defined(LAMA_PROFILING) && !CB_HALF
    if (CB_F16 && T1 == 9 && !pl2 && WMV == 4 && !s2) {
        static const int abl = lama_env_int("LAMA_CW_ABLATE", 0);
#define CW_ABL(v) \
    if (abl == v && p.TWlog == 5) { hipLaunchKernelGGL((CB_NAME(conv_wr_kernel)<9, 2, 0, 0, 4, 2, v, 2, false, false, false, false, true>), dim3(grid), dim3(512), shmem, stream, p); LAMA_CHECK_LAUNCH(); return LAMA_OK; }
        CW_ABL(1) CW_ABL(2) CW_ABL(4) CW_ABL(3) CW_ABL(7) CW_ABL(8) CW_ABL(16) CW_ABL(32) CW_ABL(128) CW_ABL(132) CW_ABL(135)
#undef CW_ABL
        static const int sch = lama_env_int("LAMA_CW_SCHED", 2);
        if (sch == 0) { hipLaunchKernelGGL((CB_NAME(conv_wr_kernel)<9, 2, 0, 0, 4, 2, 0, 0>), dim3(grid), dim3(512), shmem, stream, p); LAMA_CHECK_LAUNCH(); return LAMA_OK; }
        if (sch == 1) { hipLaunchKernelGGL((CB_NAME(conv_wr_kernel)<9, 2, 0, 0, 4, 2, 0, 1>), dim3(grid), dim3(512), shmem, stream, p); LAMA_CHECK_LAUNCH(); return LAMA_OK; }
    }
    if (CB_F16 && pl2 && WMV == 12 && T1 == 9 && io == CB_IO_F32) {
        static const int ablg = lama_env_int("LAMA_CW_ABLATE", 0);
        if (ablg == 1 || ablg == 256) {
            if (a->fuse1_w && pl.rows == 384) {
                p.f1_w = (const char*)a->fuse1_w; p.f1_bias = a->fuse1_bias; p.f1_y = (float*)a->fuse1_y.ptr; p.f1_y_bstride = a->fuse1_y.batch_stride;
// ... 35 lines not shown
        if (p.TWlog == 5) hipLaunchKernelGGL((CB_NAME(conv_wr_kernel)<9, 2, 0, 0, 4, 1, 0, 2, false, false, false, false, true, 4>), dim3(grid), dim3(256), shmem, stream, p);
        else hipLaunchKernelGGL((CB_NAME(conv_wr_kernel)<9, 2, 0, 0, 4, 1, 0, 2, false, false, false, false, false, 4>), dim3(grid), dim3(256), shmem, stream, p);
        LAMA_CHECK_LAUNCH();
        return LAMA_OK;
    }
#endif
    if (geo41) return cw_launch_t<9, 1, 0, 0, 4, 1>(stream, p, grid, shmem, io);
    if (T1 == 9 && !pl2) return cw_launch_t<9, 2, 0, 0, 4, 2>(stream, p, grid, shmem, io);
    if (a->fuse1_w && !(T1 == 9 && pl2 && WMV == 12 && io == CB_IO_F32 && pl.rows == 384)) return LAMA_ERR_UNSUPPORTED;
#if !CB_HALF
    if (a->fuse1_w) {
        p.f1_w = (const char*)a->fuse1_w;
        p.f1_bias = a->fuse1_bias;
        p.f1_y = (float*)a->fuse1_y.ptr;
        p.f1_y_bstride = a->fuse1_y.batch_stride;
        if (shmem < 144 * 1024) shmem = 144 * 1024;
        hipLaunchKernelGGL((CB_NAME(conv_wr_kernel)<9, 2, 1, 4, 12, 1, 0, 2, false, false, false, false, false, 2, true>), dim3(grid), dim3(768), shmem, stream, p);
        LAMA_CHECK_LAUNCH();
        return LAMA_OK;
    }
#endif
    if (T1 == 9 && pl2 && WMV == 12) return cw_launch_t<9, 2, 1, 4, 12, 1>(stream, p, grid, shmem, io);
    if (T1 == 9 && pl2) return cw_launch_t<9, 2, 1, 4, 4, 2>(stream, p, grid, shmem, io);
    if (T1 == 1 && !pl2 && WMV == 12) return cw_launch_t<1, 4, 0, 0, 12, 1>(stream, p, grid, shmem, io);
    if (T1 == 1 && !pl2 && WMV == 6) return cw_launch_t<1, 4, 0, 0, 6, 2>(stream, p, grid, shmem, io);
    if (T1 == 1 && !pl2) return cw_launch_t<1, 4, 0, 0, 4, 2>(stream, p, grid, shmem, io);
    return LAMA_ERR_UNSUPPORTED;
}

int ct_try_launch(hipStream_t stream, const lama_conv2d_args* a, const CbPlan& pl, int Ho, int Wo, int io, const LamaTileList* tl = nullptr) {
#if CB_HALF
    (void)stream; (void)a; (void)pl; (void)Ho; (void)Wo; (void)io; (void)tl;
    return LAMA_ERR_UNSUPPORTED;
#else
    const int mode = lama_env_int("LAMA_CT", 1);
    if (mode == 0 || !a->transposed || pl.nseg != 5 || pl.mode != 0 || io != CB_IO_F32 || a->resid.ptr || a->fuse1_w) return LAMA_ERR_UNSUPPORTED;
    const int C = a->x.C, H = a->x.H, W = a->x.W, M = pl.rows;
    if (C % 32 != 0 || M % 64 != 0 || H < 1 || W < 1 || Ho != 2 * H || Wo != 2 * W) return LAMA_ERR_UNSUPPORTED;
    if ((long long)C * H * W * 4 >= (1ll << 31)) return LAMA_ERR_UNSUPPORTED;
    CtParams p;
    memset(&p, 0, sizeof(p));
    p.x = (const float*)a->x.ptr;
    p.x_bstride = a->x.batch_stride;
    p.C = C; p.H = H; p.W = W;
    for (int c = 0; c < 4; ++c) {
        const int cls = c + 1;
        p.w[c] = (const char*)a->w_packed + pl.woff[cls];
        p.T[c] = pl.T[cls];
        p.py[c] = pl.oy0[cls]; p.px[c] = pl.ox0[cls];
        if (pl.T[cls] != (1 + p.py[c]) * (1 + p.px[c])) return LAMA_ERR_UNSUPPORTED;
        for (int t = 0; t < pl.T[cls]; ++t) p.off[c][t] = pl.dy[cls][t] * CT_PWS + pl.dx[cls][t];
    }
    if (p.T[0] != 4 || p.T[3] != 1 || p.T[1] != 2 || p.T[2] != 2) return LAMA_ERR_UNSUPPORTED;
    bool table_ok = true;
    for (int q = 0; q < 9; ++q) table_ok = table_ok && p.off[c2_cls(q)][c2_tap(q)] == c2_dy(q) * CT_PWS + c2_dx(q);
    for (int c = 0; c < 4; ++c) table_ok = table_ok && p.py[c] == (c < 2 ? 1 : 0) && p.px[c] == ((c == 0 || c == 2) ? 1 : 0);
    if (!table_ok || (a->act != LAMA_ACT_NONE && a->act != LAMA_ACT_RELU)) return LAMA_ERR_UNSUPPORTED;
    p.mft = pl.mft;
    p.bias = a->bias;
    p.y = (float*)a->y.ptr;
    p.y_bstride = a->y.batch_stride;
    p.M = M; p.B = a->batch; p.act = a->act;
    p.tiles_x = lama_ceil_div(W, 32); p.tiles_y = lama_ceil_div(H, 4); p.MG = M / 64;
    p.range_flag = a->range_flag;
    if ((a->y.batch_stride % 4) != 0 || ((uintptr_t)a->y.ptr & 15) != 0) return LAMA_ERR_UNSUPPORTED;
    const long long tiles = (long long)a->batch * p.tiles_x * p.tiles_y * p.MG;
    if (tiles <= 0) return LAMA_OK;
    if (tiles >= (1ll << 30)) return LAMA_ERR_UNSUPPORTED;
    if (tl && tl->dry) return LAMA_OK;
    { static const int abl = lama_env_int("LAMA_CT_ABLATE", 0); p.abl = abl; }
    long long grid = tiles < 512 ? tiles : 512;
    { const int cap = lama_env_int("LAMA_CT_GRID", 0); if (cap > 0 && grid > cap) grid = cap; }
    if (tl) {
        p.list = tl->list; p.count = tl->count;
        hipLaunchKernelGGL(CB_NAME(convt2_kernel)<true>, dim3((int)grid), dim3(C2_THREADS), C2_LDS_BYTES, stream, p);
    } else
        hipLaunchKernelGGL(CB_NAME(convt2_kernel)<false>, dim3((int)grid), dim3(C2_THREADS), C2_LDS_BYTES, stream, p);
    LAMA_CHECK_LAUNCH();
    return LAMA_OK;
#endif
}

int stem_try_launch(hipStream_t stream, const lama_conv2d_args* a, const CbPlan& pl, int Ho, int Wo, int io) {
    if (io != CB_IO_F32 && io != CB_IO_F32_F16) return LAMA_ERR_UNSUPPORTED;
    static const int mode = lama_env_int("LAMA_STEM_WS", 1);
    if (mode == 0 || pl.mode != 1 || pl.mft != 2 || a->transposed || a->stride != 1 || a->pad != 3 || a->pad_mode != LAMA_PAD_REFLECT ||
        a->resid.ptr || a->x.H < 4 || a->x.W < 4)
        return LAMA_ERR_UNSUPPORTED;
    const long long HW = (long long)Ho * Wo;
    if ((long long)a->x.C * HW >= (1ll << 29) || 64 * HW >= (1ll << 29)) return LAMA_ERR_UNSUPPORTED;
    StemParams p;
    memset(&p, 0, sizeof(p));
    p.x = (const float*)a->x.ptr;
    p.x_bstride = a->x.batch_stride;
    p.C = a->x.C; p.H = Ho; p.W = Wo;
    p.w = (const char*)a->w_packed + pl.woff[0];
    p.mft = pl.mft;
    p.bias = a->bias;
    p.y = (float*)a->y.ptr;
    p.y_bstride = a->y.batch_stride;
    p.M = pl.rows;
    p.B = a->batch;
    p.act = a->act;
    p.range_flag = a->range_flag;
    p.tx = lama_ceil_div(Wo, 32);
    const long long ntiles = (long long)a->batch * Ho * p.tx;
    if (mode != 2 && ntiles < 4096) return LAMA_ERR_UNSUPPORTED;
    const long long cols = (long long)a->batch * p.tx;
    long long ns = cols >= 1024 ? 1 : lama_ceil_div64(1024, cols);
    if (ns > Ho) ns = Ho;
    p.rs = (int)lama_ceil_div64(Ho, ns);
    p.ns = lama_ceil_div(Ho, p.rs);
    if (cols * p.ns >= (1ll << 31)) return LAMA_ERR_UNSUPPORTED;
    p.nseg = (int)(cols * p.ns);
    int grid = 512;
    if ((long long)grid * 2 > p.nseg) grid = (p.nseg + 1) / 2;
#if CB_HALF
    if (io != CB_IO_F32_F16) return LAMA_ERR_UNSUPPORTED;
    hipLaunchKernelGGL(CB_NAME(stem7_ws_kernel)<true>, dim3(grid), dim3(256), STEM_LDS_BYTES, stream, p);
#else
    if (io != CB_IO_F32) return LAMA_ERR_UNSUPPORTED;
    hipLaunchKernelGGL(CB_NAME(stem7_ws_kernel)<false>, dim3(grid), dim3(256), STEM_LDS_BYTES, stream, p);
#endif
    LAMA_CHECK_LAUNCH();
    return LAMA_OK;
}

int head_try_launch(hipStream_t stream, const lama_conv2d_args* a, const CbPlan& pl, int Ho, int Wo, int io, const LamaTileList* tl = nullptr) {
    if (io != CB_IO_F32 && io != CB_IO_F16_F32) return LAMA_ERR_UNSUPPORTED;
    if (tl && (io != CB_IO_F32 || tl->head_rs < HEAD_R || tl->head_rs % HEAD_R != 0)) return LAMA_ERR_UNSUPPORTED;
    static const int mode = lama_env_int("LAMA_HEAD_WS", 1);
    if (mode == 0 || pl.mode != 2 || pl.mft != 1 || a->x.C != 64 || a->y.C > 4 || a->transposed || a->stride != 1 || a->pad != 3 ||
        a->pad_mode != LAMA_PAD_REFLECT || a->resid.ptr || a->x.H < 4 || a->x.W < 4)
        return LAMA_ERR_UNSUPPORTED;
    const long long HW = (long long)Ho * Wo;
    if (64 * HW >= (1ll << 29)) return LAMA_ERR_UNSUPPORTED;
    HeadParams p;
    memset(&p, 0, sizeof(p));
    p.x = (const float*)a->x.ptr;
    p.x_bstride = a->x.batch_stride;
    p.C = 64; p.H = Ho; p.W = Wo;
    p.w = (const char*)a->w_packed + pl.woff[0];
    p.bias = a->bias;
    p.y = (float*)a->y.ptr;
    p.y_bstride = a->y.batch_stride;
    p.M = a->y.C;
    p.B = a->batch;
    p.act = a->act;
    p.range_flag = a->range_flag;
    p.tx = lama_ceil_div(Wo, 26);
    const long long cols = (long long)a->batch * p.tx;
    if (mode != 2 && cols * Ho < 8192) return LAMA_ERR_UNSUPPORTED;
    const int wgs = 768;
    int best_rs = HEAD_R;
    double best = -1.0;
    for (int rs = HEAD_R; rs <= HEAD_R * lama_ceil_div(Ho, HEAD_R); rs += HEAD_R) {
        const long long nseg = cols * lama_ceil_div(Ho, rs);
        const double per = (double)nseg / wgs;
        const double rounds = per <= 1.0 ? 1.0 : (double)lama_ceil_div64(nseg, wgs);
        const double eff = (per <= 1.0 ? per : per / rounds) * rs / (rs + 6.0 + HEAD_D);
        if (eff > best) { best = eff; best_rs = rs; }
    }
    p.rs = tl ? tl->head_rs : best_rs;
    p.ns = lama_ceil_div(Ho, p.rs);
    if (cols * p.ns >= (1ll << 31)) return LAMA_ERR_UNSUPPORTED;
    p.nseg = (int)(cols * p.ns);
    const int grid = p.nseg < wgs ? p.nseg : wgs;
    if (tl && tl->dry) return LAMA_OK;
#if !CB_HALF
    if (tl) {
        p.list = tl->list; p.count = tl->count;
        hipLaunchKernelGGL((CB_NAME(head7_ws_kernel)<false, true>), dim3(grid), dim3(256), HEAD_LDS_BYTES, stream, p);
        LAMA_CHECK_LAUNCH();
        return LAMA_OK;
    }
#endif
#if CB_HALF
    if (io != CB_IO_F16_F32) return LAMA_ERR_UNSUPPORTED;
    hipLaunchKernelGGL(CB_NAME(head7_ws_kernel)<true>, dim3(grid), dim3(256), HEAD_LDS_BYTES, stream, p);
#else
    if (io != CB_IO_F32) return LAMA_ERR_UNSUPPORTED;
    hipLaunchKernelGGL(CB_NAME(head7_ws_kernel)<false>, dim3(grid), dim3(256), HEAD_LDS_BYTES, stream, p);
#endif
    LAMA_CHECK_LAUNCH();
    return LAMA_OK;
}
```

### lama_amd/ffc.py

```python
from __future__ import annotations

from typing import List, Optional, Tuple

import collections
import contextlib
import warnings

import torch
import torch.nn as nn

from . import _lib as L
from ._lib import LamaError, LamaRangeError

_ACT = {'relu': L.ACT_RELU, 'sigmoid': L.ACT_SIGMOID, 'tanh': L.ACT_TANH, None: L.ACT_NONE}



def _bn_fold(bn: nn.BatchNorm2d) -> Tuple[torch.Tensor, torch.Tensor]:
    scale = bn.weight.detach().float() / torch.sqrt(bn.running_var.detach().float() + bn.eps)
    shift = bn.bias.detach().float() - bn.running_mean.detach().float() * scale
    return scale, shift


def _act_code(layer) -> int:
    if layer is None or isinstance(layer, nn.Identity) or layer is nn.Identity:
        return L.ACT_NONE
    if isinstance(layer, nn.ReLU) or layer is nn.ReLU:
        return L.ACT_RELU
    if isinstance(layer, nn.Sigmoid) or layer is nn.Sigmoid:
        return L.ACT_SIGMOID
    if isinstance(layer, nn.Tanh) or layer is nn.Tanh:
        return L.ACT_TANH
    raise NotImplementedError(f'activation {layer} is not supported by the HIP epilogues')


def _adjacent(a: torch.Tensor, b: torch.Tensor) -> Optional[torch.Tensor]:
    if a.dim() != 4 or b.dim() != 4 or a.shape[0] != b.shape[0] or a.shape[2:] != b.shape[2:]:
        return None
    B, ca, H, W = a.shape
    cb = b.shape[1]
    bs = (ca + cb) * H * W
    want = (bs, H * W, W, 1)
    if tuple(a.stride()) != want or tuple(b.stride()) != want:
        return None
    if a.untyped_storage().data_ptr() != b.untyped_storage().data_ptr():
        return None
    if b.storage_offset() != a.storage_offset() + ca * H * W:
        return None
    return torch.as_strided(a, (B, ca + cb, H, W), want, a.storage_offset())


def _pair_buffer(x_l: torch.Tensor, x_g) -> Tuple[torch.Tensor, int, int]:
    if not torch.is_tensor(x_g):
        return x_l.contiguous(), x_l.shape[1], 0
    buf = _adjacent(x_l, x_g)
    if buf is None:
        buf = torch.cat([x_l, x_g], dim=1)
    return buf, x_l.shape[1], x_g.shape[1]


def _check_input(x: torch.Tensor):
    if not x.is_cuda:
        raise LamaError('lama_amd runs on an MI355X only: input tensor is on ' + str(x.device) +
                        ' (there is no CPU fallback; the CPU oracle lives in oracle/ for tests)')
    if x.dtype not in (torch.float32, torch.float16):
        raise LamaError(f'fp32 (or, with precision f16, fp16) activations expected, got {x.dtype}')


class SidePipe:

    def __init__(self, stream: 'torch.cuda.Stream'):
        self.stream = stream
        self.prev_local = None

    def join(self):
        if self.prev_local is not None:
            torch.cuda.current_stream(self.stream.device).wait_stream(self.stream)
            self.prev_local = None


class _Exec:

    def __init__(self, lib: Optional[L.LamaLib] = None):
        self._lib = lib
        self.injected = lib is not None
        self._flags = {}
        self._deferred_since_read = {}
        self._sticky = {}
        self._depth = 0
        self.no_fuse1 = set()
        self._cur_flag = None
        self.fuse1_min_tiles = 192
        self.siblings_log2 = 0
        self.winograd = True
        self.local_first = True
        self.cooperative_serial = False

    @property
    def lib(self) -> L.LamaLib:
        if self._lib is None:
            self._lib = L.get_lib()
        return self._lib

    def stream(self, t: torch.Tensor) -> int:
        return torch.cuda.current_stream(t.device).cuda_stream if t.is_cuda else 0

    def check(self, x: torch.Tensor):
        if not self.injected:
            _check_input(x)

    @contextlib.contextmanager
    def range_scope(self, t: torch.Tensor, precision: int, deferred: bool = False):
        outer = self._depth == 0
        if outer and precision in (L.PREC_F16X3, L.PREC_F16):
            key = self._dev_key(t.device)
            if key not in self._flags:
                self._flags[key] = torch.zeros(1, dtype=torch.int32, device=t.device)
            elif not deferred and self._deferred_since_read.get(key):
                if int(self._flags[key].item()) != 0:
                    self._sticky[key] = True
                self._flags[key].zero_()
            self._deferred_since_read[key] = bool(deferred)
            self._cur_flag = self._flags[key]
        self._depth += 1
        try:
            yield
        except BaseException:
            self._depth -= 1
            if outer:
                self._cur_flag = None
            raise
        self._depth -= 1
        if outer:
            flag, self._cur_flag = self._cur_flag, None
            if flag is not None and not deferred and int(flag.item()) != 0:
                flag.zero_()
                raise LamaRangeError(_RANGE_MSG)

    def range_flag_raised(self, device=None) -> bool:
        bad = False
        want = None if device is None else self._dev_key(device)
        for key, flag in self._flags.items():
            if want is not None and key != want:
                continue
            self._deferred_since_read[key] = False
            if int(flag.item()) != 0:
                flag.zero_()
                bad = True
            if self._sticky.pop(key, False):
                bad = True
        return bad

    @contextlib.contextmanager
    def scratch_range_scope(self, t: torch.Tensor, precision: int):
        key = self._dev_key(t.device)
        flag = self._flags.get(key)
        pending = bool(self._deferred_since_read.get(key))
        was = flag is not None and pending and int(flag.item()) != 0
        try:
            with self.range_scope(t, precision, deferred=True):
                yield
        finally:
            flag = self._flags.get(key)
            if flag is not None:
                flag.fill_(1 if was else 0)
            self._deferred_since_read[key] = pending

    @staticmethod
    def _dev_key(device) -> str:
        d = torch.device(device)
        if d.type == 'cuda' and d.index is None:
            d = torch.device('cuda', torch.cuda.current_device())
        return str(d)

    def conv2d(self, *a, **kw):
        flag = self._cur_flag if kw.get('precision') in (L.PREC_F16X3, L.PREC_F16) else None
        if self.siblings_log2:
            kw['siblings_log2'] = self.siblings_log2
        return self.lib.conv2d(*a, range_flag=flag, **kw)
# ... 45 lines not shown
        return super().load_state_dict(*a, **kw)

    def set_exec(self, ex: _Exec):
        for m in self.modules():
            if isinstance(m, _HipModule):
                m._exec = ex
                m._packed = None
        return self

    def set_precision(self, precision: int):
        for m in self.modules():
            if isinstance(m, _HipModule):
                m.precision = precision
        self._precision_hook(precision)
        self._invalidate()
        return self

    def _precision_hook(self, precision: int):
        """Per-layer exceptions to a uniform precision (FFCResNetGenerator: the fp32 tail of LAMA_PREC_F16)."""

    def train(self, mode: bool = True):
        if mode:
            raise NotImplementedError('lama_amd modules are inference-only (eval-mode BatchNorm is folded into the kernels)')
        return super().train(False)


class _PlanGenerator(_HipModule):

    def __init__(self):
        super().__init__()
        self.use_graph = False
        self.auto_fallback = True
        self.defer_range_check = False
        self.clone_output = True
        self.max_plans = 4
        self.sparse_tail = False
        self._assume_graph = False
        self.split_decisions = {}
        self._plans = collections.OrderedDict()

    def _invalidate(self):
        super()._invalidate()
        self._plans = collections.OrderedDict()

    @staticmethod
    def _plan_key(shape, device):
        return (tuple(int(v) for v in shape), _Exec._dev_key(device))

    has_sparse_tail = False

    def _sparse(self) -> bool:
        return bool(self.sparse_tail and self.has_sparse_tail)

    def _cache_key(self, shape, device):
        key = self._plan_key(shape, device)
        return key + ('sparse_tail',) if self._sparse() else key

    def _split_parts(self, shape, device) -> int:
        return 1

    def _new_plan(self, shape, device, n: int) -> dict:
        return self._build_plan(shape, device)

    def _make_room(self):
        while len(self._plans) >= max(1, self.max_plans):
            self._plans.popitem(last=False)

    def _plan_for(self, shape, device) -> dict:
        key = self._cache_key(shape, device)
        n = self._split_parts(shape, device)
        plan = self._plans.get(key)
        if plan is not None and plan.get('nsplit', 1) != n:
            plan = None
            del self._plans[key]
        if plan is None:
            self._make_room()
            plan = self._plans[key] = self._new_plan(shape, device, n)
        else:
            self._plans.move_to_end(key)
        return plan

    def drop_plan(self, shape, device) -> None:
        key = self._plan_key(shape, device)
        self._plans.pop(key, None)
        self._plans.pop(key + ('sparse_tail',), None)

    def input_buffer(self, shape, device) -> torch.Tensor:
        device = torch.device(device)
        plan = self._plan_for(shape, device)
        if plan['static_in'] is None:
            plan['static_in'] = torch.empty(tuple(shape), device=device, dtype=torch.float32)
        return plan['static_in']

    def _capture(self, plan, device):
        side = torch.cuda.Stream(device=device)
        side.wait_stream(torch.cuda.current_stream(device))
        with torch.cuda.stream(side):
            self._run_plan(plan, plan['static_in'])
        torch.cuda.current_stream(device).wait_stream(side)
        g = torch.cuda.CUDAGraph()
        with torch.cuda.graph(g):
            plan['static_out'] = self._run_plan(plan, plan['static_in'])
        plan['graph'] = g

    def _forward(self, x: torch.Tensor) -> torch.Tensor:
        plan = self._plan_for(x.shape, x.device)
        fin = (lambda t: t.clone()) if self.clone_output else (lambda t: t)
        if not (self.use_graph and x.is_cuda):
            return fin(self._run_plan(plan, x))
        own = plan['static_in'] is not None and x.data_ptr() == plan['static_in'].data_ptr()
        if plan['graph'] is None:
            if not own:
                plan['static_in'] = torch.empty_like(x)
                plan['static_in'].copy_(x)
            self._capture(plan, x.device)
        if not own:
            plan['static_in'].copy_(x)
        plan['graph'].replay()
        return fin(plan['static_out'])

    def _can_fall_back(self) -> bool:
        return self.auto_fallback and self.precision in (L.PREC_F16X3, L.PREC_F16)

    def _check_input(self, x: torch.Tensor):
        self._exec.check(x)

    def forward(self, input: torch.Tensor) -> torch.Tensor:
        self._check_input(input)
        x = input.contiguous()
        try:
            with self._exec.range_scope(x, self.precision, deferred=self.defer_range_check):
                return self._forward(x)
        except LamaRangeError as e:
            if not self._can_fall_back():
                raise
            warnings.warn(f'lama_amd: {e}; switching this generator to the 3-term bf16 split (PREC_BF16X3)')
            self.set_precision(L.PREC_BF16X3)
            return self.forward(input)

    def check_range(self, device=None, reduce=None) -> bool:
        bad = self._exec.range_flag_raised(device)
        if reduce is not None:
            bad = bool(reduce(bad))
        if not bad:
            return True
        if not self._can_fall_back():
            raise LamaRangeError(_RANGE_MSG)
        warnings.warn(f'lama_amd: {_RANGE_MSG}; switching this generator to the 3-term bf16 split (PREC_BF16X3): re-run the inputs since the last check')
        self.set_precision(L.PREC_BF16X3)
        return False


def _plan_up(layers, i, src, dst, src_shape, bufs, steps, device):
    lay, n = layers[i], len(layers)
    bn = layers[i + 1] if i + 1 < n and isinstance(layers[i + 1], BatchNorm2dEval) else None
    act = layers[i + 2] if bn is not None and i + 2 < n and isinstance(layers[i + 2], Activation) else None
    B, _, H, W = src_shape
    shp = (B, lay.out_channels, 2 * H, 2 * W)
    bufs[dst] = torch.empty(shp, device=device, dtype=_act_dtype(lay.precision))
    steps.append(('up', lay, src, dst, bn, _ACT[act.kind] if act else L.ACT_NONE))
    return shp, 1 + (bn is not None) + (act is not None)


def _plan_out(layers, i, src, dst, src_shape, pad, bufs, steps, device):
    lay = layers[i]
    act = layers[i + 1] if i + 1 < len(layers) and isinstance(layers[i + 1], Activation) else None
    B, _, H, W = src_shape
    kk, p = lay.kernel_size[0], lay.padding[0] + pad
# ... 106 lines not shown
                self._pack(None)
            x1 = torch.empty(b, half, h, w, device=x.device, dtype=x.dtype)
            t = torch.empty_like(x1)
            st = self._exec.stream(x)
            self.run_front(L.view(x), x1, t, self.fu.workspace(x1), b, st)
            y = torch.empty(b, self.conv2.out_channels, h, w, device=x.device, dtype=x.dtype)
            self._exec.conv2d(L.view(t), self._packed['w2'], L.view(y), b, 1, precision=self.precision, stream=st)
        return y



class FFC(_HipModule):

    def __init__(self, in_channels, out_channels, kernel_size, ratio_gin, ratio_gout, stride=1, padding=0, dilation=1,
                 groups=1, bias=False, enable_lfu=True, padding_type='reflect', gated=False, **spectral_kwargs):
        super().__init__()
        assert stride == 1 or stride == 2, "Stride should be 1 or 2."
        if dilation != 1 or groups != 1 or bias or gated:
            raise NotImplementedError('FFC: dilation/groups/bias/gated variants are not used by the shipped LaMa configs')
        if padding_type != 'reflect' and padding != 0:
            raise NotImplementedError('FFC: only reflect padding is implemented')
        self.stride, self.kernel_size, self.padding = stride, kernel_size, padding
        in_cg = int(in_channels * ratio_gin)
        in_cl = in_channels - in_cg
        out_cg = int(out_channels * ratio_gout)
        out_cl = out_channels - out_cg
        self.in_cl, self.in_cg, self.out_cl, self.out_cg = in_cl, in_cg, out_cl, out_cg
        self.ratio_gin, self.ratio_gout = ratio_gin, ratio_gout
        self.global_in_num = in_cg

        def conv(ci, co):
            return nn.Conv2d(ci, co, kernel_size, stride, padding, dilation, groups, bias, padding_mode=padding_type)

        self.convl2l = nn.Identity() if in_cl == 0 or out_cl == 0 else conv(in_cl, out_cl)
        self.convl2g = nn.Identity() if in_cl == 0 or out_cg == 0 else conv(in_cl, out_cg)
        self.convg2l = nn.Identity() if in_cg == 0 or out_cl == 0 else conv(in_cg, out_cl)
        self.convg2g = nn.Identity() if in_cg == 0 or out_cg == 0 else SpectralTransform(in_cg, out_cg, stride, 1, enable_lfu,
                                                                                         **spectral_kwargs)
        self.gated = gated
        self.gate = nn.Identity()
        if in_cl == 0:
            raise NotImplementedError('FFC with ratio_gin == 1 (no local input) is not implemented')
        if in_cg > 0 and (out_cl == 0 or out_cg == 0):
            raise NotImplementedError('FFC with a global input needs both local and global outputs (ratio_gout in (0,1))')
        if in_cg > 0 and (stride != 1 or kernel_size != 3):
            raise NotImplementedError('FFC with a global input is implemented for 3x3 stride-1 layers (the resnet blocks)')

    def pack(self, sl=None, bl=None, sg=None, bg=None):
        f, lib, prec = self, self._exec.lib, self.precision
        pk = {}

        def cat_opt(ts, n):
            return None if any(t is None for t in ts) else torch.cat(ts, 0).contiguous()

        if f.in_cg == 0:
            ws, ss, bs = [], [], []
            if f.out_cl:
                ws.append(f.convl2l.weight.detach()); ss.append(sl); bs.append(bl)
            if f.out_cg:
                ws.append(f.convl2g.weight.detach()); ss.append(sg); bs.append(bg)
            pk['w_all'] = lib.pack_conv_weight(torch.cat(ws, 0), cat_opt(ss, 0), stride=f.stride, precision=prec)
            pk['b_all'] = cat_opt(bs, 0)
        else:
            w_lout = torch.cat([f.convl2l.weight.detach(), f.convg2l.weight.detach()], dim=1)
            pk['w_lout'] = lib.pack_conv_weight(w_lout, sl, precision=prec)
            if (f.kernel_size == 3 and f.stride == 1 and f.padding == 1 and prec in (L.PREC_F16X3, L.PREC_BF16X3)
                    and w_lout.shape[0] % 128 == 0 and w_lout.shape[1] % 32 == 0):
                try:
                    pk['w_lout_wino'] = lib.pack_winograd_weight(w_lout, sl, prec)
                except LamaRangeError:
                    pass
            pk['b_l'] = None if bl is None else bl.contiguous()
            pk['w_l2g'] = lib.pack_conv_weight(f.convl2g.weight.detach(), sg, precision=prec)
            pk['b_g'] = None if bg is None else bg.contiguous()
            st = f.convg2g
            st._packed = None
            st._pack(sg)
            st._packed['fused_scale'] = id(sg) if sg is not None else 'none'
            st.fu._pack()
        return pk

    def launch(self, pk: dict, act: int, src: torch.Tensor, dst: torch.Tensor, scratch: Optional[dict],
               resid: Optional[torch.Tensor] = None, extra_pad: int = 0, side: Optional['torch.cuda.Stream'] = None,
               x1_ready: bool = False, fuse_next: Optional['SpectralTransform'] = None) -> bool:
        f, ex, prec = self, self._exec, self.precision
        B = src.shape[0]
        st = ex.stream(src)
        pad = f.padding + extra_pad
        if f.in_cg == 0:
            ex.conv2d(L.view(src), pk['w_all'], L.view(dst), B, f.kernel_size, f.stride, pad, L.PAD_REFLECT, False, pk['b_all'],
                      act, None if resid is None else L.view(resid), precision=prec, stream=st)
            return False
        cl, cg, ocl, ocg = f.in_cl, f.in_cg, f.out_cl, f.out_cg
        spec = f.convg2g
        wino = (ex.winograd and pad == 1 and 'w_lout_wino' in pk and scratch is not None and scratch.get('wino') is not None
                and src.dtype == torch.float32 and dst.dtype == torch.float32 and not isinstance(side, SidePipe))

        def local_conv(stream, cooperative):
            rl = None if resid is None else L.view(resid, 0, ocl)
            if wino:
                try:
                    defer = bool(scratch.get('defer_out')) and side is None
                    pend = ex.winograd_conv3x3(L.view(src), pk['w_lout_wino'], L.view(dst, 0, ocl), B, scratch['wino'], pk['b_l'], act, rl,
                                               precision=prec, stream=stream, defer_out=defer)
                    if defer:
                        scratch['pending_out'] = (pend, scratch['wino'])
                    return
                except LamaError as e:
                    if e.code != L.ERR_UNSUPPORTED:
                        raise
                    scratch['wino'] = None
            ex.conv2d(L.view(src), pk['w_lout'], L.view(dst, 0, ocl), B, 3, 1, pad, L.PAD_REFLECT, False, pk['b_l'], act, rl, precision=prec,
                      stream=stream, cooperative=cooperative)

        if isinstance(side, SidePipe) and src.is_cuda:
            main = torch.cuda.current_stream(src.device)
            side.stream.wait_stream(main)
            local_conv(side.stream.cuda_stream, True)
            done = torch.cuda.Event()
            done.record(side.stream)
            spec.run_front(L.view(src, cl, cg), scratch['x1'], scratch['t'], scratch['ws'], B, st, x1_ready)
            if side.prev_local is not None:
                main.wait_event(side.prev_local)
            side.prev_local = done
        elif side is not None and src.is_cuda:
            main = torch.cuda.current_stream(src.device)
            side.wait_stream(main)
            if not ex.local_first:
                spec.run_front(L.view(src, cl, cg), scratch['x1'], scratch['t'], scratch['ws'], B, side.cuda_stream, x1_ready)
            local_conv(st, True)
            if ex.local_first:
                spec.run_front(L.view(src, cl, cg), scratch['x1'], scratch['t'], scratch['ws'], B, side.cuda_stream, x1_ready)
            main.wait_stream(side)
        else:
            spec.run_front(L.view(src, cl, cg), scratch['x1'], scratch['t'], scratch['ws'], B, st, x1_ready, wino_out=scratch.pop('pending_out', None))
            local_conv(st, ex.cooperative_serial)
        fuse1 = None
        shape_key = (tuple(src.shape), prec)
        tiles = (B * ((dst.shape[2] * dst.shape[3] + 127) // 128)) << ex.siblings_log2
        if (fuse_next is not None and f.kernel_size == 3 and f.stride == 1 and ocg == 384 and shape_key not in ex.no_fuse1
                and (tiles >= ex.fuse1_min_tiles or ex.injected)):
            fuse1 = fuse_next.fuse1_operands(scratch['x1'])
        gargs = (L.view(src, 0, cl), pk['w_l2g'], L.view(dst, ocl, ocg), B, 3, 1, pad, L.PAD_REFLECT, False, pk['b_g'], act,
                 None if resid is None else L.view(resid, ocl, ocg))
        gkw = dict(x2=L.view(scratch['t']), w2_packed=spec._packed['w2'], precision=prec, stream=st)
        if fuse1 is not None:
            try:
                ex.conv2d(*gargs, fuse1=fuse1, **gkw)
                return True
            except LamaError as e:
                if e.code != L.ERR_UNSUPPORTED:
                    raise
                ex.no_fuse1.add(shape_key)
        ex.conv2d(*gargs, **gkw)
        return False

    def out_shape(self, src_shape, extra_pad: int = 0):
        B, _, H, W = src_shape
        pad = self.padding + extra_pad
        Ho = (H + 2 * pad - self.kernel_size) // self.stride + 1
        Wo = (W + 2 * pad - self.kernel_size) // self.stride + 1
        return (B, self.out_cl + self.out_cg, Ho, Wo)

    def make_scratch(self, src_shape, device, alias_t: bool = False) -> Optional[dict]:
        if self.in_cg == 0:
            return None
        B, _, H, W = src_shape
        half = self.convg2g.conv2.in_channels
        x1 = torch.empty(B, half, H, W, device=device, dtype=_act_dtype(self.precision))
        sc = dict(x1=x1, t=x1 if alias_t else torch.empty_like(x1), ws=self.convg2g.fu.workspace(x1))
        lib = self._exec.lib
        if (self._exec.winograd and self.kernel_size == 3 and self.stride == 1 and self.padding == 1 and self.out_cl
                and lib.winograd_preferred(B, self.out_cl, self.in_cl + self.in_cg, H, W, self.precision)):
            sc['wino'] = torch.empty(lib.winograd_workspace_bytes(B, self.out_cl, H, W) // 4, device=device, dtype=torch.float32)
        return sc

    def forward(self, x):
        x_l, x_g = x if type(x) is tuple else (x, 0)
        self._exec.check(x_l)
        src, cl, cg = _pair_buffer(x_l, x_g)
        if cl != self.in_cl or cg != self.in_cg:
            raise LamaError(f'FFC expected ({self.in_cl},{self.in_cg}) local/global channels, got ({cl},{cg})')
        with self._exec.range_scope(src, self.precision):
            if self._packed is None or (self.in_cg and (self.convg2g._packed or {}).get('fused_scale') != 'none'):
                self._packed = self.pack()
            dst = torch.empty(self.out_shape(src.shape), device=src.device, dtype=_act_dtype(self.precision))
            self.launch(self._packed, L.ACT_NONE, src, dst, self.make_scratch(src.shape, src.device))
        return (dst[:, :self.out_cl] if self.out_cl else 0), (dst[:, self.out_cl:] if self.out_cg else 0)


class FFC_BN_ACT(_HipModule):

    def __init__(self, in_channels, out_channels, kernel_size, ratio_gin, ratio_gout, stride=1, padding=0, dilation=1,
                 groups=1, bias=False, norm_layer=nn.BatchNorm2d, activation_layer=nn.Identity, padding_type='reflect',
                 enable_lfu=True, **kwargs):
        super().__init__()
        if norm_layer is not nn.BatchNorm2d:
            raise NotImplementedError('only BatchNorm2d (eval) is folded into the kernels')
        self.ffc = FFC(in_channels, out_channels, kernel_size, ratio_gin, ratio_gout, stride, padding, dilation, groups, bias,
                       enable_lfu, padding_type=padding_type, **kwargs)
        global_channels = int(out_channels * ratio_gout)
        self.bn_l = nn.Identity() if ratio_gout == 1 else nn.BatchNorm2d(out_channels - global_channels)
        self.bn_g = nn.Identity() if ratio_gout == 0 else nn.BatchNorm2d(global_channels)
        self.act_l = nn.Identity() if ratio_gout == 1 else activation_layer(inplace=True)
        self.act_g = nn.Identity() if ratio_gout == 0 else activation_layer(inplace=True)
        self._act = _act_code(activation_layer)

    def _pack(self):
        if self._packed is not None:
            return self._packed
        f = self.ffc
        sl, bl = _bn_fold(self.bn_l) if f.out_cl else (None, None)
        sg, bg = _bn_fold(self.bn_g) if f.out_cg else (None, None)
        self._packed = f.pack(sl, bl, sg, bg)
        self._packed['_sg'] = sg
        f._packed = None
        return self._packed

    def run(self, src: torch.Tensor, dst: torch.Tensor, scratch: Optional[dict], resid: Optional[torch.Tensor] = None,
            extra_pad: int = 0, side: Optional['torch.cuda.Stream'] = None, x1_ready: bool = False,
            fuse_next: Optional['FFC_BN_ACT'] = None) -> bool:
        f = self.ffc
        if f.in_cg and self._packed is not None and (f.convg2g._packed or {}).get('fused_scale') != id(self._packed.get('_sg')):
            self._packed = None
        nxt = None
        if fuse_next is not None and fuse_next.ffc.in_cg:
            fuse_next._pack()
            nxt = fuse_next.ffc.convg2g
        return f.launch(self._pack(), self._act, src, dst, scratch, resid, extra_pad, side, x1_ready, nxt)

    def out_shape(self, src_shape, extra_pad: int = 0):
        return self.ffc.out_shape(src_shape, extra_pad)

    def make_scratch(self, src_shape, device, alias_t: bool = False) -> Optional[dict]:
        return self.ffc.make_scratch(src_shape, device, alias_t)

    def forward(self, x, extra_pad: int = 0):
        x_l, x_g = x if type(x) is tuple else (x, 0)
        self._exec.check(x_l)
        src, cl, cg = _pair_buffer(x_l, x_g)
        if cl != self.ffc.in_cl or cg != self.ffc.in_cg:
            raise LamaError(f'FFC_BN_ACT expected ({self.ffc.in_cl},{self.ffc.in_cg}) local/global channels, got ({cl},{cg})')
        dst = torch.empty(self.out_shape(src.shape, extra_pad), device=src.device,
                          dtype=torch.float32 if self.ffc.out_cg else _act_dtype(self.precision))
        with self._exec.range_scope(src, self.precision):
            self.run(src, dst, self.make_scratch(src.shape, src.device), None, extra_pad)
        ocl, ocg = self.ffc.out_cl, self.ffc.out_cg
        return (dst[:, :ocl] if ocl else 0), (dst[:, ocl:] if ocg else 0)


class FFCResnetBlock(_HipModule):

    def __init__(self, dim, padding_type, norm_layer, activation_layer=nn.ReLU, dilation=1, spatial_transform_kwargs=None,
                 inline=False, **conv_kwargs):
        super().__init__()
        if spatial_transform_kwargs is not None or inline or dilation != 1:
            raise NotImplementedError('FFCResnetBlock: spatial transforms / inline / dilation are not used by big-lama')
        self.conv1 = FFC_BN_ACT(dim, dim, kernel_size=3, padding=dilation, dilation=dilation, norm_layer=norm_layer,
                                activation_layer=activation_layer, padding_type=padding_type, **conv_kwargs)
        self.conv2 = FFC_BN_ACT(dim, dim, kernel_size=3, padding=dilation, dilation=dilation, norm_layer=norm_layer,
                                activation_layer=activation_layer, padding_type=padding_type, **conv_kwargs)
        self.inline = inline

    def run(self, src: torch.Tensor, tmp: torch.Tensor, dst: torch.Tensor, scratch: Optional[dict], side=None, x1_ready: bool = False,
            next_block: Optional['FFCResnetBlock'] = None, fuse: bool = False) -> bool:
        mid_ready = self.conv1.run(src, tmp, scratch, side=side, x1_ready=x1_ready, fuse_next=self.conv2 if fuse else None)
        return self.conv2.run(tmp, dst, scratch, resid=src, side=side, x1_ready=mid_ready,
                              fuse_next=None if next_block is None else next_block.conv1)

    def forward(self, x):
        x_l, x_g = x if type(x) is tuple else (x, 0)
        self._exec.check(x_l)
        src, cl, cg = _pair_buffer(x_l, x_g)
        tmp, dst = torch.empty_like(src, dtype=_act_dtype(self.precision)), torch.empty_like(src)
        with self._exec.range_scope(src, self.precision):
            self.run(src, tmp, dst, self.conv1.make_scratch(src.shape, src.device))
        return (dst[:, :cl], dst[:, cl:]) if cg else (dst, 0)


class ConcatTupleLayer(nn.Module):

    def forward(self, x):
        assert isinstance(x, tuple)
        x_l, x_g = x
        assert torch.is_tensor(x_l) or torch.is_tensor(x_g)
        if not torch.is_tensor(x_g):
            return x_l
        buf = _adjacent(x_l, x_g)
        return buf if buf is not None else torch.cat(x, dim=1)



class ReflectionPad2d(_HipModule):
    def __init__(self, padding: int):
        super().__init__()
        self.padding = int(padding)

    def forward(self, x):
        self._exec.check(x)
        x = x.contiguous()
        B, Cn, H, W = x.shape
        y = torch.empty(B, Cn, H + 2 * self.padding, W + 2 * self.padding, device=x.device, dtype=torch.float32)
        self._exec.lib.reflect_pad(L.view(x), self.padding, L.view(y), B, self._exec.stream(x))
        return y


class _Affine(_HipModule):
    def _launch(self, x, scale, shift, act):
        self._exec.check(x)
        x = x.contiguous()
        y = torch.empty_like(x)
        self._exec.lib.affine_act(L.view(x), scale, shift, act, L.view(y), x.shape[0], self._exec.stream(x))
# ... 93 lines not shown
        layers = list(self)
        i, n = 0, len(layers)
        while i < n:
            cur = layers[i]
            nxt = layers[i + 1] if i + 1 < n else None
            if isinstance(cur, ReflectionPad2d) and isinstance(nxt, FFC_BN_ACT) and torch.is_tensor(x):
                x = nxt(x, extra_pad=cur.padding); i += 2
            elif isinstance(cur, ReflectionPad2d) and isinstance(nxt, Conv2dOut):
                act = layers[i + 2] if i + 2 < n and isinstance(layers[i + 2], Activation) else None
                x = nxt(x, extra_pad=cur.padding, act=_ACT[act.kind] if act else L.ACT_NONE)
                i += 3 if act else 2
            elif isinstance(cur, ConvTranspose2dUp) and isinstance(nxt, BatchNorm2dEval) and i + 2 < n and \
                    isinstance(layers[i + 2], Activation):
                x = cur(x, bn=nxt, act=_ACT[layers[i + 2].kind]); i += 3
            else:
                x = cur(x); i += 1
        return x



class FFCResNetGenerator(_PlanGenerator):

    def __init__(self, input_nc, output_nc, ngf=64, n_downsampling=3, n_blocks=9, norm_layer=nn.BatchNorm2d,
                 padding_type='reflect', activation_layer=nn.ReLU, up_norm_layer=nn.BatchNorm2d, up_activation=nn.ReLU(True),
                 init_conv_kwargs={}, downsample_conv_kwargs={}, resnet_conv_kwargs={}, spatial_transform_layers=None,
                 spatial_transform_kwargs={}, add_out_act=True, max_features=1024, out_ffc=False, out_ffc_kwargs={}):
        assert (n_blocks >= 0)
        super().__init__()
        if spatial_transform_layers is not None or out_ffc:
            raise NotImplementedError('spatial_transform_layers / out_ffc are not used by big-lama and not implemented')
        if norm_layer is not nn.BatchNorm2d or up_norm_layer is not nn.BatchNorm2d or padding_type != 'reflect':
            raise NotImplementedError('only BatchNorm2d + reflect padding (the big-lama configuration) are implemented')
        up_act = 'relu' if isinstance(up_activation, nn.ReLU) else None
        if up_act is None:
            raise NotImplementedError('up_activation must be ReLU')

        model: List[nn.Module] = [ReflectionPad2d(3),
                                  FFC_BN_ACT(input_nc, ngf, kernel_size=7, padding=0, norm_layer=norm_layer,
                                             activation_layer=activation_layer, **init_conv_kwargs)]
        for i in range(n_downsampling):
            mult = 2 ** i
            if i == n_downsampling - 1:
                cur_conv_kwargs = dict(downsample_conv_kwargs)
                cur_conv_kwargs['ratio_gout'] = resnet_conv_kwargs.get('ratio_gin', 0)
            else:
                cur_conv_kwargs = downsample_conv_kwargs
            model += [FFC_BN_ACT(min(max_features, ngf * mult), min(max_features, ngf * mult * 2), kernel_size=3, stride=2,
                                 padding=1, norm_layer=norm_layer, activation_layer=activation_layer, **cur_conv_kwargs)]
        mult = 2 ** n_downsampling
        feats_num_bottleneck = min(max_features, ngf * mult)
        for i in range(n_blocks):
            model += [FFCResnetBlock(feats_num_bottleneck, padding_type=padding_type, activation_layer=activation_layer,
                                     norm_layer=norm_layer, **resnet_conv_kwargs)]
        model += [ConcatTupleLayer()]
        for i in range(n_downsampling):
            mult = 2 ** (n_downsampling - i)
            model += [ConvTranspose2dUp(min(max_features, ngf * mult), min(max_features, int(ngf * mult / 2))),
                      BatchNorm2dEval(min(max_features, int(ngf * mult / 2))), Activation(up_act)]
        model += [ReflectionPad2d(3), Conv2dOut(ngf, output_nc, kernel_size=7, padding=0)]
        if add_out_act:
            kind = 'tanh' if add_out_act is True else add_out_act
            if kind not in ('tanh', 'sigmoid'):
                raise ValueError(f'Unknown activation kind {kind}')
            model.append(Activation(kind))
        self.model = LayerSequence(*model)
        self.overlap_streams = True
        self.fuse_conv1 = None
        self.serial_with_winograd = True
        self.serial_when_full = True
        self.fuse_conv1_serial = True
        self.pipeline_local = False
        self.f16_fp32_tail = True
        self.inplace_residual = True
        self.alias_t = True
        self.alias_wino = True
        self.defer_wino_out = True
        self.split_batch = None
        self.n_downsampling = n_downsampling
        self.verify_split = True
        self._split_ok = {}
        self.split_margin = 0.02
        self.split_replays = 9
        self.tail_head_rs = 16
        super().train(False)

    def _precision_hook(self, precision: int):
        if precision != L.PREC_F16 or not getattr(self, 'f16_fp32_tail', False):
            return
        tail = False
        for lay in self.model:
            tail = tail or isinstance(lay, ConcatTupleLayer)
            if tail and isinstance(lay, _HipModule):
                lay.precision = L.PREC_F16X3

    def _invalidate(self):
        super()._invalidate()
        self._split_ok = {}

    def _build_plan(self, shape, device, one_stream: bool = False):
        layers = list(self.model)
        steps = []
        bufs = {}
        cur_shape = tuple(shape)
        cur = 'in'
        i, n = 0, len(layers)
        pad_pending = 0

        adt = _act_dtype(self.precision)

        def new(name, shp, dtype=None):
            bufs[name] = torch.empty(shp, device=device, dtype=dtype or adt)
            return name

        scratch = None
        k = 0
        while i < n:
            lay = layers[i]
            if isinstance(lay, ReflectionPad2d):
                pad_pending = lay.padding; i += 1; continue
            if isinstance(lay, FFC_BN_ACT):
                shp = lay.out_shape(cur_shape, pad_pending)
                feeds_blocks = lay.ffc.out_cg > 0
                dst = new(f'a{k}', shp, torch.float32 if feeds_blocks else None); k += 1
                steps.append(('ffc', lay, cur, dst, pad_pending))
                cur, cur_shape, pad_pending = dst, shp, 0
            elif isinstance(lay, FFCResnetBlock):
                if 'rt' not in bufs:
                    scratch = lay.conv1.make_scratch(cur_shape, device, alias_t=self.alias_t)
                    new('rt', cur_shape)
                if self.inplace_residual and cur != 'in' and bufs[cur].dtype == torch.float32:
                    dst = cur
                else:
                    dst = 'rA' if cur != 'rA' else 'rB'
                    if dst not in bufs:
                        new(dst, cur_shape, torch.float32)
                steps.append(('res', lay, cur, 'rt', dst))
                cur = dst
            elif isinstance(lay, ConcatTupleLayer):
                pass
            elif isinstance(lay, ConvTranspose2dUp):
                dst = f'a{k}'; k += 1
                cur_shape, took = _plan_up(layers, i, cur, dst, cur_shape, bufs, steps, device)
                cur = dst; i += took - 1
            elif isinstance(lay, Conv2dOut):
                cur_shape, took = _plan_out(layers, i, cur, 'out', cur_shape, pad_pending, bufs, steps, device)
                cur, pad_pending = 'out', 0; i += took - 1
            else:
                raise LamaError(f'no fused plan for layer {type(lay).__name__}; run generator.model layer by layer')
            i += 1
        res_layers = [l for st_ in steps if st_[0] == 'res' for l in (st_[1].conv1, st_[1].conv2)]
        wino = bool(scratch and scratch.get('wino') is not None and self._exec.winograd and res_layers
                    and all('w_lout_wino' in l._pack() for l in res_layers))
        if scratch and scratch.get('wino') is not None and not wino:
            scratch['wino'] = None
        serial = wino and self.serial_with_winograd
        if not wino and not serial and self.serial_when_full and res_layers and scratch and scratch.get('x1') is not None:
            B_, _, H_, W_ = scratch['x1'].shape
            serial = B_ * ((H_ * W_ + 127) // 128) >= 200
        if wino and serial and self.defer_wino_out:
            B_, C1, H_, W_ = scratch['x1'].shape
            spec_elems = (((B_ * 2 * C1 * H_ * (W_ // 2 + 1) * 4) + 255) & ~255) // 4
            wn = scratch['wino']
            ws = torch.empty(max(scratch['ws'].numel(), spec_elems + wn.numel()), device=device, dtype=torch.float32)
            scratch['ws'], scratch['wino'] = ws, ws[spec_elems:spec_elems + wn.numel()]
            scratch['defer_out'] = True
        elif wino and serial and self.alias_wino:
            ws, wn = scratch['ws'], scratch['wino']
            if wn.numel() <= ws.numel():
                scratch['wino'] = ws[:wn.numel()]
            else:
                scratch['ws'] = wn[:ws.numel()]
        side = torch.cuda.Stream(device=device) if (self.overlap_streams and not serial and not one_stream and torch.device(device).type == 'cuda') else None
        return dict(steps=steps, bufs=bufs, scratch=scratch, out=cur, graph=None, static_in=None, side=side,
                    tail=self._plan_tail(steps, bufs, tuple(shape), device) if self._sparse() else None,
                    fuse=self.fuse_conv1 or (serial and self.fuse_conv1 is not False and self.fuse_conv1_serial))

    has_sparse_tail = True

    def _plan_tail(self, steps, bufs, shape, device) -> Optional[dict]:
        _, C, H, W = shape
        if C != 4 or not steps or steps[-1][0] != 'out' or tuple(bufs[steps[-1][3]].shape[2:]) != (H, W):
            return None
        ups, i = [], len(steps) - 2
        while (i >= 0 and steps[i][0] == 'up' and len(ups) < 4 and steps[i][1].out_channels % 64 == 0
               and H % (2 << len(ups)) == 0 and W % (2 << len(ups)) == 0):
            ups.append(i)
            i -= 1
        lists = self._exec.lib.tail_lists_alloc(shape[0], H, W, self.tail_head_rs, [steps[j][1].out_channels // 64 for j in ups], device)
        return dict(lists=lists, out=len(steps) - 1, ups=ups, taken=None)

    def _tail_taken(self, plan, B) -> dict:
        tail, steps = plan['tail'], plan['steps']
        ls, rs = tail['lists'], tail['lists']['head_rs']
        taken = {}
        if _run_step(steps[tail['out']], B, tile_list=ls['head'] + (rs,), query=True):
            taken[tail['out']] = ls['head'] + (rs,)
            for lv, j in enumerate(tail['ups']):
                if not _run_step(steps[j], B, tile_list=ls['up'][lv] + (rs,), query=True):
                    break
                taken[j] = ls['up'][lv] + (rs,)
        return taken

    def _run_plan(self, plan, x):
        if 'parts' in plan:
            return self._run_split(plan, x)
        bufs = plan['bufs']

        def B(name):
            return x if name == 'in' else bufs[name]

        steps = plan['steps']
        sparse = {}
        if plan.get('tail') is not None:
            if plan['tail']['taken'] is None:
                plan['tail']['taken'] = self._tail_taken(plan, B)
            sparse = plan['tail']['taken']
            if sparse:
                self._exec.lib.tail_lists_build(L.view(x, 3, 1), plan['tail']['lists'], self._exec.stream(x))
        x1_ready = False
        if plan['scratch']:
            plan['scratch'].pop('pending_out', None)
        pipe = SidePipe(plan['side']) if (plan['side'] is not None and self.pipeline_local and x.is_cuda) else None
        for i, st in enumerate(steps):
            kind = st[0]
            if kind == 'ffc':
                _, lay, s, d, pad = st
                lay.run(B(s), B(d), plan['scratch'] if lay.ffc.in_cg else None, None, pad, side=plan['side'])
                x1_ready = False
            elif kind == 'res':
                _, lay, s, t, d = st
                fuse = plan.get('fuse', self.fuse_conv1)
                nxt = steps[i + 1][1] if fuse and i + 1 < len(steps) and steps[i + 1][0] == 'res' else None
                x1_ready = lay.run(B(s), B(t), B(d), plan['scratch'], side=pipe or plan['side'], x1_ready=x1_ready, next_block=nxt,
                                   fuse=fuse)
                if i + 1 == len(steps) or steps[i + 1][0] != 'res':
                    pend = plan['scratch'].pop('pending_out', None) if plan['scratch'] else None
                    if pend is not None:
                        self._exec.lib.winograd_out(pend[0], pend[1], self._exec.stream(x))
                    if pipe is not None:
                        pipe.join()
            elif i in sparse:
                _run_step(st, B, tile_list=sparse[i])
            else:
                _run_step(st, B)
        return bufs[plan['out']]

    def _split_parts(self, shape, device) -> int:
        B = int(shape[0])
        n = self.split_batch
        if n is None:
            if torch.device(device).type != 'cuda' or self.precision not in (L.PREC_F16X3, L.PREC_BF16X3, L.PREC_F16):
                return 1
            if not (self.use_graph or self._assume_graph):
                return 1
            h, w = int(shape[2]) >> self.n_downsampling, int(shape[3]) >> self.n_downsampling
            tiles = B * ((h * w + 127) // 128)
            n = 4 if tiles >= 256 else 1
            while n > 1 and B % n:
                n //= 2
            if n > 1 and self._split_ok.get(self._plan_key(shape, device)) is False:
                return 1
            return n
        n = int(n)
        if n < 1 or n & (n - 1) or n > 4 or B % n:
            raise LamaError(f'split_batch={n}: 1, 2 or 4 parts that divide the batch ({B})')
        return n

    def _build_split_plan(self, shape, device, n: int) -> dict:
        B = int(shape[0])
        h = B // n
        parts = [self._build_plan((h,) + tuple(shape[1:]), device, one_stream=True) for _ in range(n)]
        out_shape = (B,) + tuple(parts[0]['bufs'][parts[0]['out']].shape[1:])
        out_full = torch.empty(out_shape, device=device, dtype=parts[0]['bufs'][parts[0]['out']].dtype)
        for i, pl in enumerate(parts):
            pl['bufs'][pl['out']] = out_full[i * h:(i + 1) * h]
        streams = [torch.cuda.Stream(device=device) for _ in range(n - 1)] if torch.device(device).type == 'cuda' else []
        return dict(parts=parts, part_batch=h, streams=streams, out_full=out_full, nsplit=n, graph=None, static_in=None, scratch=None, side=None)

    def _run_split(self, plan, x):
        ex, parts, h = self._exec, plan['parts'], plan['part_batch']
        main = torch.cuda.current_stream(x.device) if x.is_cuda else None
        keep = ex.siblings_log2
        ex.siblings_log2 = len(parts).bit_length() - 1
        try:
            for i in range(1, len(parts)):
                xi = x[i * h:(i + 1) * h]
                if main is not None:
                    s = plan['streams'][i - 1]
                    s.wait_stream(main)
                    with torch.cuda.stream(s):
                        self._run_plan(parts[i], xi)
                else:
                    self._run_plan(parts[i], xi)
            self._run_plan(parts[0], x[:h])
            if main is not None:
                for s in plan['streams']:
                    main.wait_stream(s)
        finally:
            ex.siblings_log2 = keep
        return plan['out_full']

    def _new_plan(self, shape, device, n: int) -> dict:
        return self._build_split_plan(shape, device, n) if n > 1 else self._build_plan(shape, device)

    def tune_split(self, shape, device) -> int:
        device = torch.device(device)
        key = self._plan_key(shape, device)
        n = self._split_parts(shape, device)
        if (n <= 1 or self.split_batch is not None or not self.verify_split or key in self._split_ok or device.type != 'cuda'
                or torch.cuda.is_current_stream_capturing()):
# ... 40 lines not shown
```

Baseline: 859.9 images/s.

## Store stem and downsampling activations pre-split into fp16 hi/lo pairs

Adds a SPLIT16 tensor layout where an activation is kept as interleaved fp16 hi/lo halves in groups of eight channels. The stem 7x7 conv and the stride-2 downsampling convs now write this layout directly, and the next stride-2 conv reads it without re-splitting fp32 values. This removes the per-load fp32-to-hi/lo split and uses wider vector loads in the consumer. The cost is extra split work and range checks in the producer epilogue, and it is restricted to one-segment, K-group-free launches, which may change the kernel geometry for those layers.

```diff
diff --git a/include/lama_hip.h b/include/lama_hip.h
--- a/include/lama_hip.h
+++ b/include/lama_hip.h
@@ -29,6 +29,7 @@
 
 #define LAMA_DT_F32 0
 #define LAMA_DT_F16 1
+#define LAMA_DT_SPLIT16 2
 
 typedef struct lama_tensor {
     void* ptr;
diff --git a/lama_amd/_lib.py b/lama_amd/_lib.py
--- a/lama_amd/_lib.py
+++ b/lama_amd/_lib.py
@@ -12,7 +12,7 @@
 CONV_COOPERATIVE = 1
 CONV_DEFER_OUT = 2
 CONV_SIBLINGS_SHIFT = 8
-DT_F32, DT_F16 = 0, 1
+DT_F32, DT_F16, DT_SPLIT16 = 0, 1, 2
 POOL_MAX, POOL_AVG_EXCLUDE_PAD = 0, 1
 ABI_VERSION = 112
 PREC_NAMES = {'f32': PREC_F32, 'bf16x3': PREC_BF16X3, 'f16x3': PREC_F16X3, 'f16': PREC_F16}
@@ -71,6 +71,38 @@
     if c0 < 0 or c <= 0 or c0 + c > Ct:
         raise LamaError('channel slice out of range')
     return Tensor4(t.data_ptr() + t.element_size() * c0 * H * W, Ct * H * W, c, H, W, DT_F16 if t.dtype == torch.float16 else DT_F32)
+
+
+def view_split(t: torch.Tensor) -> Tensor4:
+    if t.dtype != torch.float32 or t.dim() != 4 or not t.is_contiguous() or t.shape[1] % 8 != 0:
+        raise LamaError(f'expected a contiguous fp32-sized NCHW buffer with C % 8 == 0, got {t.dtype} {tuple(t.shape)}')
+    B, Ct, H, W = t.shape
+    return Tensor4(t.data_ptr(), Ct * H * W, Ct, H, W, DT_SPLIT16)
+
+
+def _split16_part_dtype(precision: int) -> torch.dtype:
+    if precision not in (PREC_F16X3, PREC_BF16X3):
+        raise LamaError('LAMA_DT_SPLIT16 exists for PREC_F16X3 / PREC_BF16X3 only')
+    return torch.float16 if precision == PREC_F16X3 else torch.bfloat16
+
+
+def split16_pack(x: torch.Tensor, precision: int) -> torch.Tensor:
+    dt = _split16_part_dtype(precision)
+    B, Ct, H, W = x.shape
+    if Ct % 8 != 0:
+        raise LamaError('LAMA_DT_SPLIT16 needs C % 8 == 0')
+    x = x.float()
+    hi = x.to(dt)
+    lo = (x - hi.float()).to(dt)
+    parts = torch.stack((hi, lo), 0).view(torch.int16).view(2, B, Ct // 8, 8, H, W)
+    return parts.permute(1, 2, 0, 4, 5, 3).contiguous().view(torch.float32).view(B, Ct, H, W)
+
+
+def split16_unpack(buf: torch.Tensor, precision: int):
+    dt = _split16_part_dtype(precision)
+    B, Ct, H, W = buf.shape
+    parts = buf.contiguous().view(torch.int16).view(B, Ct // 8, 2, H, W, 8).permute(2, 0, 1, 5, 3, 4).contiguous().view(2, B, Ct, H, W)
+    return parts[0].view(dt), parts[1].view(dt)
 
 
 class LamaLib:
diff --git a/lama_amd/csrc/conv_mfma.hip b/lama_amd/csrc/conv_mfma.hip
--- a/lama_amd/csrc/conv_mfma.hip
+++ b/lama_amd/csrc/conv_mfma.hip
@@ -597,7 +597,16 @@
     if (!a || !tensor_ok(a->x) || !tensor_ok(a->y) || !a->w_packed || a->batch <= 0) return LAMA_ERR_BAD_ARG;
     if (a->precision != LAMA_PREC_F32 && a->precision != LAMA_PREC_BF16X3 && a->precision != LAMA_PREC_F16X3 && a->precision != LAMA_PREC_F16)
         return LAMA_ERR_UNSUPPORTED;
-    {
+    const bool xs = a->x.dtype == LAMA_DT_SPLIT16, ys = a->y.dtype == LAMA_DT_SPLIT16;
+    if ((a->x2.ptr && a->x2.dtype == LAMA_DT_SPLIT16) || (a->resid.ptr && a->resid.dtype == LAMA_DT_SPLIT16) ||
+        (a->fuse1_w && a->fuse1_y.dtype == LAMA_DT_SPLIT16))
+        return LAMA_ERR_UNSUPPORTED;
+    if (xs || ys) {
+        if (a->precision != LAMA_PREC_BF16X3 && a->precision != LAMA_PREC_F16X3) return LAMA_ERR_UNSUPPORTED;
+        if (tl || a->transposed || a->x2.ptr || a->resid.ptr || a->fuse1_w) return LAMA_ERR_UNSUPPORTED;
+        if ((xs && a->x.C % 8 != 0) || (ys && a->y.C % 8 != 0)) return LAMA_ERR_UNSUPPORTED;
+        if ((!xs && a->x.dtype != LAMA_DT_F32) || (!ys && a->y.dtype != LAMA_DT_F32)) return LAMA_ERR_UNSUPPORTED;
+    } else {
         const bool xh = a->x.dtype == LAMA_DT_F16, yh = a->y.dtype == LAMA_DT_F16;
         if ((a->x.dtype != LAMA_DT_F32 && !xh) || (a->y.dtype != LAMA_DT_F32 && !yh)) return LAMA_ERR_BAD_ARG;
         if (a->x2.ptr && a->x2.dtype != LAMA_DT_F32 && a->x2.dtype != LAMA_DT_F16) return LAMA_ERR_BAD_ARG;
diff --git a/lama_amd/csrc/conv_split3.inc b/lama_amd/csrc/conv_split3.inc
--- a/lama_amd/csrc/conv_split3.inc
+++ b/lama_amd/csrc/conv_split3.inc
@@ -25,13 +25,14 @@
 typedef cb_half_t bf16x2 __attribute__((ext_vector_type(2)));
 typedef cb_half_t bf16x8 __attribute__((ext_vector_type(8)));
 typedef unsigned u32x4 __attribute__((ext_vector_type(4)));
+typedef unsigned u32x2 __attribute__((ext_vector_type(2)));
 
 namespace CB_NAME(cbns) {
 
 #define CB_THREADS 512
 #define CB_MAX_TAPS 49
 
-enum { CB_IO_F32 = 0, CB_IO_F16_F32 = 1, CB_IO_F32_F16 = 2, CB_IO_F16 = 3, CB_IO_X2H = 4 };
+enum { CB_IO_F32 = 0, CB_IO_F16_F32 = 1, CB_IO_F32_F16 = 2, CB_IO_F16 = 3, CB_IO_X2H = 4, CB_IO_XS = 8, CB_IO_YS = 16 };
 
 struct CbSeg {
     const float* x;
@@ -950,6 +951,17 @@
     if (has2 && pl.mode) return LAMA_ERR_UNSUPPORTED;
     const int io = (a->x.dtype == LAMA_DT_F16 ? 1 : 0) | (a->y.dtype == LAMA_DT_F16 ? 2 : 0) | ((has2 && a->x2.dtype == LAMA_DT_F16) ? CB_IO_X2H : 0);
     if ((io != CB_IO_F32) != (CB_HALF != 0)) return LAMA_ERR_UNSUPPORTED;
+    {
+        const int ios = (a->x.dtype == LAMA_DT_SPLIT16 ? CB_IO_XS : 0) | (a->y.dtype == LAMA_DT_SPLIT16 ? CB_IO_YS : 0);
+        if (ios) {
+            if (CB_HALF || has2 || a->transposed) return LAMA_ERR_UNSUPPORTED;
+            if (ios == CB_IO_YS) {
+                const int rc = stem_try_launch(stream, a, pl, Ho, Wo, ios);
+                if (rc != LAMA_ERR_UNSUPPORTED) return rc;
+            }
+            return cw_try_launch(stream, a, pl, nullptr, Ho, Wo, ios);
+        }
+    }
     {
         int rc = cw_try_launch(stream, a, pl, has2 ? &pl2 : nullptr, Ho, Wo, io);
         if (rc != LAMA_ERR_UNSUPPORTED) return rc;
diff --git a/lama_amd/csrc/conv_stem_dev.inc b/lama_amd/csrc/conv_stem_dev.inc
--- a/lama_amd/csrc/conv_stem_dev.inc
+++ b/lama_amd/csrc/conv_stem_dev.inc
@@ -27,8 +27,9 @@
     pb = __builtin_amdgcn_perm(lo, hi, 0x07060302u);
 }
 
-template <bool HO = false>
+template <bool HO = false, bool YS = false>
 __global__ __launch_bounds__(256, 2) void CB_NAME(stem7_ws_kernel)(StemParams p) {
+    static_assert(!(HO && YS), "pre-split output: the 3-term split precisions only");
     constexpr int ESO = HO ? 2 : 4;
     const int tid = threadIdx.x, lane = tid & 63, wave = LAMA_WAVE_UNIFORM(tid >> 6);
     const int F = wave & 1, half = wave >> 1;
@@ -171,10 +172,28 @@
 #pragma unroll
                 for (int r = 0; r < 16; ++r) ov[r] = tanhf(ov[r]);
             }
-#pragma unroll
-            for (int r = 0; r < 16; ++r) {
-                if constexpr (HO) LAMA_BUF_STORE_B16(yres, __builtin_bit_cast(unsigned short, (_Float16)ov[r]), eoff, ((r & 3) + 8 * (r >> 2)) * HW * ESO);
-                else LAMA_BUF_STORE_B32(yres, __builtin_bit_cast(unsigned, ov[r]), eoff, ((r & 3) + 8 * (r >> 2)) * HW * ESO);
+            if constexpr (YS) {
+#pragma unroll
+                for (int g = 0; g < 4; ++g) {
+                    unsigned h0, h1, l0, l1;
+                    cb_split2(ov[4 * g], ov[4 * g + 1], h0, l0);
+                    cb_split2(ov[4 * g + 2], ov[4 * g + 3], h1, l1);
+                    const int oct = F * 4 + g;
+                    const bool stored = px < W && oct * 8 < p.M;
+                    if (stored) {
+                        cb_range_watch(h0, rw);
+                        cb_range_watch(h1, rw);
+                    }
+                    const int voff = stored ? (y * W + px) * 16 + 8 * khalf : 0x7ffffff0;
+                    LAMA_BUF_STORE_B64(yres, (u32x2{h0, h1}), voff, oct * 2 * HW * 16);
+                    LAMA_BUF_STORE_B64(yres, (u32x2{l0, l1}), voff, (oct * 2 + 1) * HW * 16);
+                }
+            } else {
+#pragma unroll
+                for (int r = 0; r < 16; ++r) {
+                    if constexpr (HO) LAMA_BUF_STORE_B16(yres, __builtin_bit_cast(unsigned short, (_Float16)ov[r]), eoff, ((r & 3) + 8 * (r >> 2)) * HW * ESO);
+                    else LAMA_BUF_STORE_B32(yres, __builtin_bit_cast(unsigned, ov[r]), eoff, ((r & 3) + 8 * (r >> 2)) * HW * ESO);
+                }
             }
         }
         LAMA_WAVE_SYNC();
diff --git a/lama_amd/csrc/conv_wreg_dev.inc b/lama_amd/csrc/conv_wreg_dev.inc
--- a/lama_amd/csrc/conv_wreg_dev.inc
+++ b/lama_amd/csrc/conv_wreg_dev.inc
@@ -21,7 +21,7 @@
     bf16x8 bh[4], bl[4];
 };
 
-template <int T, int KSC, int WMV, int KG, int ABL = 0, int SCH = 2, bool HF = false, bool HI = HF, bool ROLL = false, int NU = 2>
+template <int T, int KSC, int WMV, int KG, int ABL = 0, int SCH = 2, bool HF = false, bool HI = HF, bool ROLL = false, int NU = 2, bool XS = false>
 __device__ __forceinline__ void cw_segment(const CbSeg& s, int F, int b, int gy0, int gx0, int TWlog, char* pbuf0, int pbytes,
                                            f32x16 (&acc)[4], unsigned& rw, long long* trace = nullptr) {
     using S = CwShape<T, KSC, WMV, KG>;
@@ -29,6 +29,8 @@
     constexpr bool BDB = S::BDB;
     constexpr int BKC = 16 * KSC;
     constexpr int ES = HI ? 2 : 4;
+    static_assert(!XS || (!HF && !HI), "pre-split input: the 3-term split precisions only");
+    constexpr int NLD = XS ? 2 * NU : 8 * NU;
     const int tid = threadIdx.x, lane = tid & 63, wave = LAMA_WAVE_UNIFORM(tid >> 6);
     const int kg = KG == 1 ? 0 : wave / WMV;
     const int khalf = lane >> 5, l31 = lane & 31;
@@ -54,7 +56,7 @@
             if (iy >= 0 && ix >= 0) { so = iy * s.W + ix; ok = 1; }
             lo = (q * s.npix + py * s.PWs + (s.PWh ? (px & 1) * s.PWh + (px >> 1) : px)) * 16;
         }
-        ubase[i] = (q * 8 * HW + so) * ES;
+        ubase[i] = XS ? (q * 2 * HW + so) * 16 : (q * 8 * HW + so) * ES;
         lds_off[i] = lo;
         uvalid[i] = ok;
     }
@@ -62,6 +64,20 @@
     float preg[PFD][NU][8];
     auto load_units = [&](int ch, auto slot_tag) {
         constexpr int SL = decltype(slot_tag)::value;
+        if constexpr (XS) {
+#pragma unroll
+            for (int hl = 0; hl < 2; ++hl)
+#pragma unroll
+                for (int i = 0; i < NU; ++i) {
+                    const u32x4 v = __builtin_bit_cast(u32x4, LAMA_BUF_LOAD_B128(xres, ubase[i], ch * BKC * HW * 4 + hl * HW * 16));
+#pragma unroll
+                    for (int e = 0; e < 4; ++e) {
+                        const unsigned ve = v[e];
+                        preg[SL][i][4 * hl + e] = __builtin_bit_cast(float, ve);
+                    }
+                }
+            return;
+        }
 #pragma unroll
         for (int e = 0; e < 8; ++e) {
             const int so = (ch * BKC + e) * HW * ES;
@@ -79,7 +95,10 @@
             unsigned hh[4], ll[4];
 #pragma unroll
             for (int e = 0; e < 4; ++e) {
-                if constexpr (HI) {
+                if constexpr (XS) {
+                    hh[e] = __builtin_bit_cast(unsigned, preg[SL][i][e]);
+                    ll[e] = __builtin_bit_cast(unsigned, preg[SL][i][4 + e]);
+                } else if constexpr (HI) {
                     hh[e] = __builtin_bit_cast(unsigned, preg[SL][i][2 * e]) | (__builtin_bit_cast(unsigned, preg[SL][i][2 * e + 1]) << 16);
                     cb_range_watch(hh[e], rw);
                     ll[e] = 0u;
@@ -209,7 +228,7 @@
             }
             if constexpr (SCH == 1) __builtin_amdgcn_sched_barrier(0);
             if constexpr (SCH == 2 && !(ABL & 8) && !HF) {
-                constexpr int NVM = ((ABL & 1) ? 0 : 2) + (LDU ? 8 * NU : 0);
+                constexpr int NVM = ((ABL & 1) ? 0 : 2) + (LDU ? NLD : 0);
                 auto grp = [&](auto i_tag) {
                     constexpr int i = decltype(i_tag)::value;
                     __builtin_amdgcn_sched_group_barrier(0x008, 1, 0);
@@ -313,7 +332,7 @@
                 for (int j = 0; j < 4; ++j) acc[j] = CB_MFMA(a_lo, rows[slot(ky + j)].h, acc[j], 0, 0, 0);
             }
             if constexpr (SCH == 2 && !HF && !(ABL & 8)) {
-                constexpr int NVM = ((ABL & 1) ? 0 : 2) + (LDU ? 8 * NU : 0);
+                constexpr int NVM = ((ABL & 1) ? 0 : 2) + (LDU ? NLD : 0);
                 auto grp = [&](auto i_tag) {
                     constexpr int i = decltype(i_tag)::value;
                     __builtin_amdgcn_sched_group_barrier(0x008, 1, 0);
@@ -357,8 +376,9 @@
 }
 
 template <int T1, int KSC1, int T2, int KSC2, int WMV = 4, int KG = 2, int ABL = 0, int SCH = 2, bool HF = false, bool HI1 = HF, bool HI2 = HF,
-          bool HO = HF, bool ROLL = false, int NU = 2, bool FUSE1 = false>
+          bool HO = HF, bool ROLL = false, int NU = 2, bool FUSE1 = false, bool XS = false, bool YS = false>
 __global__ __launch_bounds__(64 * WMV * KG, (WMV * KG == 4) ? 2 : 1) void CB_NAME(conv_wr_kernel)(CbParams p) {
+    static_assert(!(XS || YS) || (KG == 1 && T2 == 0 && !HF && !HO && !FUSE1), "pre-split tensors: plain one-segment launches without K-groups");
     using AT = typename LamaAct<HO>::T;
     const int L = lama_xcd_remap(blockIdx.x, gridDim.x);
     const int mt = L % p.MT;
@@ -387,7 +407,7 @@
 
     unsigned rw = 0;
     const int Fw = (ABL & 256) ? Fc % 6 : Fc;
-    cw_segment<T1, KSC1, WMV, KG, (ABL & 255), SCH, HF, HI1, ROLL && T1 == 9, NU>(p.s1, Fw, b, gy0, gx0, p.TWlog, lama_smem, p.pbytes, acc, rw, trace);
+    cw_segment<T1, KSC1, WMV, KG, (ABL & 255), SCH, HF, HI1, ROLL && T1 == 9, NU, XS>(p.s1, Fw, b, gy0, gx0, p.TWlog, lama_smem, p.pbytes, acc, rw, trace);
     if constexpr (T2 > 0) cw_segment<T2, KSC2, WMV, KG, (ABL & 65), SCH, HF, HI2>(p.s2, Fw, b, gy0, gx0, p.TWlog, lama_smem, p.pbytes, acc, rw, (ABL & 64) ? trace + 7 : nullptr);
     cb_range_report(rw, p.range_flag);
 
@@ -417,7 +437,9 @@
     };
     auto store_frag = [&](int j, const f32x16& v16, int slot) {
         bool pv;
-        const unsigned lo = (unsigned)(frag_off(j, pv) + kplane);
+        const int po = frag_off(j, pv);
+        const unsigned lo = (unsigned)(po + kplane);
+        [[maybe_unused]] float vs[16];
 #pragma unroll
         for (int r = 0; r < 16; ++r) {
             const int mu = row_u(r);
@@ -426,7 +448,25 @@
             else if (p.act == LAMA_ACT_SIGMOID) v = 1.0f / (1.0f + expf(-v));
             else if (p.act == LAMA_ACT_TANH) v = tanhf(v);
             v += rv[slot][r];
-            if (pv && mu + khalf4 < p.M) (reinterpret_cast<AT*>(p.y) + (long long)b * p.y_bstride + (long long)mu * plane)[lo] = (AT)v;
+            if constexpr (YS) vs[r] = v;
+            else if (pv && mu + khalf4 < p.M) (reinterpret_cast<AT*>(p.y) + (long long)b * p.y_bstride + (long long)mu * plane)[lo] = (AT)v;
+        }
+        if constexpr (YS) {
+            char* const yb = reinterpret_cast<char*>(p.y) + (long long)b * p.y_bstride * 4;
+#pragma unroll
+            for (int g = 0; g < 4; ++g) {
+                unsigned h0, h1, l0, l1;
+                cb_split2(vs[4 * g], vs[4 * g + 1], h0, l0);
+                cb_split2(vs[4 * g + 2], vs[4 * g + 3], h1, l1);
+                const int oct = F * 4 + g;
+                if (pv && oct * 8 < p.M) {
+                    cb_range_watch(h0, rw);
+                    cb_range_watch(h1, rw);
+                    char* const d = yb + ((long long)oct * 2 * plane + po) * 16 + 2 * khalf4;
+                    *reinterpret_cast<u32x2*>(d) = u32x2{h0, h1};
+                    *reinterpret_cast<u32x2*>(d + plane * 16) = u32x2{l0, l1};
+                }
+            }
         }
     };
     if constexpr (FUSE1) {
@@ -544,6 +584,7 @@
             else if (j + 1 < 4) load_resid(j + 1, (j + 1) & 1);
             store_frag(j, acc[j], NRV == 1 ? 0 : (j & 1));
         }
+        if constexpr (YS) cb_range_report(rw, p.range_flag);
     } else {
         if (kg == 1) {
 #pragma unroll
diff --git a/lama_amd/csrc/conv_wreg_host.inc b/lama_amd/csrc/conv_wreg_host.inc
--- a/lama_amd/csrc/conv_wreg_host.inc
+++ b/lama_amd/csrc/conv_wreg_host.inc
@@ -269,8 +269,27 @@
     if (io == CB_IO_F16) hipLaunchKernelGGL((CB_NAME(conv_wr_kernel)<9, 1, 0, 0, 4, 1, 0, 0, true, true, true, true, false, 5>), dim3(grid), dim3(256), shmem, st, p);
     else hipLaunchKernelGGL((CB_NAME(conv_wr_kernel)<9, 1, 0, 0, 4, 1, 0, 0, true, true, true, false, false, 5>), dim3(grid), dim3(256), shmem, st, p);
 #else
+    if (io & (CB_IO_XS | CB_IO_YS)) {
+        if (io & ~(CB_IO_XS | CB_IO_YS)) return LAMA_ERR_UNSUPPORTED;
+#define CW_S2_SPLIT(xs, ys) hipLaunchKernelGGL((CB_NAME(conv_wr_kernel)<9, 1, 0, 0, 4, 1, 0, 2, false, false, false, false, false, 5, false, xs, ys>), dim3(grid), dim3(256), shmem, st, p)
+        if (io == (CB_IO_XS | CB_IO_YS)) CW_S2_SPLIT(true, true);
+        else if (io == CB_IO_XS) CW_S2_SPLIT(true, false);
+        else CW_S2_SPLIT(false, true);
+#undef CW_S2_SPLIT
+        LAMA_CHECK_LAUNCH();
+        return LAMA_OK;
+    }
     if (io != CB_IO_F32) return LAMA_ERR_UNSUPPORTED;
     static const int geo = lama_env_int("LAMA_CW_S2", 1);
+#if defined(LAMA_PROFILING)
+    if (CB_F16 && geo != 2) {
+        static const int abl = lama_env_int("LAMA_CW_ABLATE", 0);
+#define CW_ABL_S2(v) \
+    if (abl == v) { hipLaunchKernelGGL((CB_NAME(conv_wr_kernel)<9, 1, 0, 0, 4, 1, v, 2, false, false, false, false, false, 5>), dim3(grid), dim3(256), shmem, st, p); LAMA_CHECK_LAUNCH(); return LAMA_OK; }
+        CW_ABL_S2(4) CW_ABL_S2(16) CW_ABL_S2(32)
+#undef CW_ABL_S2
+    }
+#endif
     if (geo == 2) hipLaunchKernelGGL((CB_NAME(conv_wr_kernel)<9, 2, 0, 0, 4, 2, 0, 2, false, false, false, false, false, 5>), dim3(grid), dim3(512), shmem, st, p);
     else hipLaunchKernelGGL((CB_NAME(conv_wr_kernel)<9, 1, 0, 0, 4, 1, 0, 2, false, false, false, false, false, 5>), dim3(grid), dim3(256), shmem, st, p);
 #endif
@@ -307,6 +326,9 @@
     if (!cw_enabled() || a->transposed || (a->stride != 1 && a->stride != 2) || pl.mode != 0 || pl.nseg != 1) return LAMA_ERR_UNSUPPORTED;
     const bool s2 = a->stride == 2;
     if (s2 && (pl.T[0] != 9 || pl2 || a->pad != 1)) return LAMA_ERR_UNSUPPORTED;
+    const bool split_io = (io & (CB_IO_XS | CB_IO_YS)) != 0;
+    if (split_io && (!s2 || CB_HALF || a->resid.ptr || a->x.C % 8 != 0 || pl.rows % 8 != 0 || pl.rows != a->y.C)) return LAMA_ERR_UNSUPPORTED;
+    if (split_io && ((long long)a->x.C * a->x.H * a->x.W >= (1ll << 29) || (long long)a->y.C * Ho * Wo >= (1ll << 29))) return LAMA_ERR_UNSUPPORTED;
     const int T1 = pl.T[0];
     int twlog3 = 5;
     const long long tiles_img = (T1 == 9 && !s2) ? cw_pick_tile(Wo, Ho, a->batch, a->flags, &twlog3) : lama_ceil_div64((long long)Ho * Wo, 128);
@@ -319,7 +341,7 @@
 #else
     static const int s2geo = lama_env_int("LAMA_CW_S2", 1);
 #endif
-    if (s2 && s2geo != 2) KG = 1;
+    if (s2 && (s2geo != 2 || split_io)) KG = 1;
     const int g41 = lama_env_int("LAMA_CW_41", 0);
     bool geo41 = false, coop41 = false;
     if (pl.T[0] == 9 && !pl2 && !s2 && pl.mft % 4 == 0) {
@@ -521,7 +543,8 @@
 }
 
 int stem_try_launch(hipStream_t stream, const lama_conv2d_args* a, const CbPlan& pl, int Ho, int Wo, int io) {
-    if (io != CB_IO_F32 && io != CB_IO_F32_F16) return LAMA_ERR_UNSUPPORTED;
+    if (io != CB_IO_F32 && io != CB_IO_F32_F16 && io != CB_IO_YS) return LAMA_ERR_UNSUPPORTED;
+    if (io == CB_IO_YS && pl.rows % 8 != 0) return LAMA_ERR_UNSUPPORTED;
     static const int mode = lama_env_int("LAMA_STEM_WS", 1);
     if (mode == 0 || pl.mode != 1 || pl.mft != 2 || a->transposed || a->stride != 1 || a->pad != 3 || a->pad_mode != LAMA_PAD_REFLECT ||
         a->resid.ptr || a->x.H < 4 || a->x.W < 4)
@@ -558,8 +581,9 @@
     if (io != CB_IO_F32_F16) return LAMA_ERR_UNSUPPORTED;
     hipLaunchKernelGGL(CB_NAME(stem7_ws_kernel)<true>, dim3(grid), dim3(256), STEM_LDS_BYTES, stream, p);
 #else
-    if (io != CB_IO_F32) return LAMA_ERR_UNSUPPORTED;
-    hipLaunchKernelGGL(CB_NAME(stem7_ws_kernel)<false>, dim3(grid), dim3(256), STEM_LDS_BYTES, stream, p);
+    if (io == CB_IO_YS) hipLaunchKernelGGL((CB_NAME(stem7_ws_kernel)<false, true>), dim3(grid), dim3(256), STEM_LDS_BYTES, stream, p);
+    else if (io != CB_IO_F32) return LAMA_ERR_UNSUPPORTED;
+    else hipLaunchKernelGGL(CB_NAME(stem7_ws_kernel)<false>, dim3(grid), dim3(256), STEM_LDS_BYTES, stream, p);
 #endif
     LAMA_CHECK_LAUNCH();
     return LAMA_OK;
diff --git a/lama_amd/ffc.py b/lama_amd/ffc.py
--- a/lama_amd/ffc.py
+++ b/lama_amd/ffc.py
@@ -95,6 +95,7 @@
         self.winograd = True
         self.local_first = True
         self.cooperative_serial = False
+        self.presplit_stem_min_tiles = 4096
 
     @property
     def lib(self) -> L.LamaLib:
@@ -306,8 +307,8 @@
 
     def drop_plan(self, shape, device) -> None:
         key = self._plan_key(shape, device)
-        self._plans.pop(key, None)
-        self._plans.pop(key + ('sparse_tail',), None)
+        for k in [k for k in self._plans if k[:len(key)] == key]:
+            del self._plans[k]
 
     def input_buffer(self, shape, device) -> torch.Tensor:
         device = torch.device(device)
@@ -580,15 +581,18 @@
 
     def launch(self, pk: dict, act: int, src: torch.Tensor, dst: torch.Tensor, scratch: Optional[dict],
                resid: Optional[torch.Tensor] = None, extra_pad: int = 0, side: Optional['torch.cuda.Stream'] = None,
-               x1_ready: bool = False, fuse_next: Optional['SpectralTransform'] = None) -> bool:
+               x1_ready: bool = False, fuse_next: Optional['SpectralTransform'] = None, split=(False, False)) -> bool:
         f, ex, prec = self, self._exec, self.precision
         B = src.shape[0]
         st = ex.stream(src)
         pad = f.padding + extra_pad
         if f.in_cg == 0:
-            ex.conv2d(L.view(src), pk['w_all'], L.view(dst), B, f.kernel_size, f.stride, pad, L.PAD_REFLECT, False, pk['b_all'],
+            ex.conv2d(L.view_split(src) if split[0] else L.view(src), pk['w_all'], L.view_split(dst) if split[1] else L.view(dst), B,
+                      f.kernel_size, f.stride, pad, L.PAD_REFLECT, False, pk['b_all'],
                       act, None if resid is None else L.view(resid), precision=prec, stream=st)
             return False
+        if split[0] or split[1]:
+            raise LamaError('LAMA_DT_SPLIT16 tensors: layers without a global input only')
         cl, cg, ocl, ocg = f.in_cl, f.in_cg, f.out_cl, f.out_cg
         spec = f.convg2g
         wino = (ex.winograd and pad == 1 and 'w_lout_wino' in pk and scratch is not None and scratch.get('wino') is not None
@@ -717,7 +721,7 @@
 
     def run(self, src: torch.Tensor, dst: torch.Tensor, scratch: Optional[dict], resid: Optional[torch.Tensor] = None,
             extra_pad: int = 0, side: Optional['torch.cuda.Stream'] = None, x1_ready: bool = False,
-            fuse_next: Optional['FFC_BN_ACT'] = None) -> bool:
+            fuse_next: Optional['FFC_BN_ACT'] = None, split=(False, False)) -> bool:
         f = self.ffc
         if f.in_cg and self._packed is not None and (f.convg2g._packed or {}).get('fused_scale') != id(self._packed.get('_sg')):
             self._packed = None
@@ -725,7 +729,7 @@
         if fuse_next is not None and fuse_next.ffc.in_cg:
             fuse_next._pack()
             nxt = fuse_next.ffc.convg2g
-        return f.launch(self._pack(), self._act, src, dst, scratch, resid, extra_pad, side, x1_ready, nxt)
+        return f.launch(self._pack(), self._act, src, dst, scratch, resid, extra_pad, side, x1_ready, nxt, split=split)
 
     def out_shape(self, src_shape, extra_pad: int = 0):
         return self.ffc.out_shape(src_shape, extra_pad)
@@ -985,6 +989,7 @@
         self.split_margin = 0.02
         self.split_replays = 9
         self.tail_head_rs = 16
+        self.presplit_outer = True
         super().train(False)
 
     def _precision_hook(self, precision: int):
@@ -1074,11 +1079,45 @@
             else:
                 scratch['ws'] = wn[:ws.numel()]
         side = torch.cuda.Stream(device=device) if (self.overlap_streams and not serial and not one_stream and torch.device(device).type == 'cuda') else None
-        return dict(steps=steps, bufs=bufs, scratch=scratch, out=cur, graph=None, static_in=None, side=side,
+        return dict(steps=steps, bufs=bufs, scratch=scratch, out=cur, graph=None, static_in=None, side=side, split=self._presplit_edges(steps, bufs, shape),
                     tail=self._plan_tail(steps, bufs, tuple(shape), device) if self._sparse() else None,
                     fuse=self.fuse_conv1 or (serial and self.fuse_conv1 is not False and self.fuse_conv1_serial))
 
     has_sparse_tail = True
+
+    def _cache_key(self, shape, device):
+        key = super()._cache_key(shape, device)
+        return key if self.presplit_outer else key + ('fp32_outer',)
+
+    def _presplit_edges(self, steps, bufs, shape) -> frozenset:
+        if not self.presplit_outer or self.precision not in (L.PREC_F16X3, L.PREC_BF16X3):
+            return frozenset()
+        ex = self._exec
+
+        def s2_conv(st, src_shape):
+            f, (_, C, H, W) = st[1].ffc, src_shape
+            return (f.in_cg == 0 and f.kernel_size == 3 and f.stride == 2 and f.padding + st[4] == 1 and C % 32 == 0
+                    and f.out_cl + f.out_cg >= 96 and (f.out_cl + f.out_cg) % 8 == 0 and C * H * W < (1 << 29))
+
+        def stem(st, src_shape, dst_shape):
+            f, (B, C, _, _), (_, M, Ho, Wo) = st[1].ffc, src_shape, dst_shape
+            return (f.in_cg == 0 and f.kernel_size == 7 and f.stride == 1 and f.padding + st[4] == 3 and C <= 4 and 33 <= M <= 64 and M % 8 == 0
+                    and Ho >= 4 and Wo >= 4 and 64 * Ho * Wo < (1 << 29) and B * Ho * ((Wo + 31) // 32) >= ex.presplit_stem_min_tiles)
+
+        def shape_of(name):
+            return tuple(shape) if name == 'in' else tuple(bufs[name].shape)
+
+        split = set()
+        for i in range(len(steps) - 1):
+            p, c = steps[i], steps[i + 1]
+            if p[0] != 'ffc' or c[0] != 'ffc' or c[2] != p[3] or p[1].ffc.out_cg or sum(1 for st in steps if st[2] == p[3]) != 1:
+                continue
+            ps, ds = shape_of(p[2]), shape_of(p[3])
+            if ds[1] * ds[2] * ds[3] >= (1 << 29) or not s2_conv(c, ds):
+                continue
+            if stem(p, ps, ds) or s2_conv(p, ps):
+                split.add(p[3])
+        return frozenset(split)
 
     def _plan_tail(self, steps, bufs, shape, device) -> Optional[dict]:
         _, C, H, W = shape
@@ -1128,7 +1167,8 @@
             kind = st[0]
             if kind == 'ffc':
                 _, lay, s, d, pad = st
-                lay.run(B(s), B(d), plan['scratch'] if lay.ffc.in_cg else None, None, pad, side=plan['side'])
+                sp = plan.get('split') or ()
+                lay.run(B(s), B(d), plan['scratch'] if lay.ffc.in_cg else None, None, pad, side=plan['side'], split=(s in sp, d in sp))
                 x1_ready = False
             elif kind == 'res':
                 _, lay, s, t, d = st
```

Result: faster. 870.0 images/s, median of 6 (+1.2%).
